# strukturag/libde265

Measured on AMD Instinct MI355X. Metric: decoded CTBs/s, higher is better.
Workload: dtype u16; 1 GPU; c5_8k10_8tiles; width=7680, height=4320, bit_depth=10, tiles=4x2, ctbs_per_picture=8160, stages=inter+residual+intra+deblock+sao, parallelism=pictures/1

## Files before the change

### libde265_amd/csrc/k_common.h

```cpp
#ifndef M355_K_COMMON_H
#define M355_K_COMMON_H

#include <hip/hip_runtime.h>
#include <stdint.h>

#include "de265_mi355x.h"
#include <k_asm.h>

struct DevRef {
  const void* plane[3];
  int stride[3];
  int valid;
  int pad;
};

struct DevIntraWork {
  uint32_t ctb;
  uint32_t ib_start, ib_count;
  uint16_t nb_same;
  uint16_t nb_earlier;
  uint8_t waves_code;
  uint8_t pad[3];
  uint32_t plan_base;
  uint32_t plan_count;
  uint32_t reserved;
};
#ifndef M355_INTRA_SHARE_MIN_LOG2
#define M355_INTRA_SHARE_MIN_LOG2 5
#endif
#define M355_IBX_HAS_RES 0x02000000u
#define M355_IBX_PCM     0x04000000u
#define M355_IBX_FILT    0x08000000u
#define M355_IBX_STRONG  0x10000000u
#define M355_IBX_BFILT   0x20000000u
#define M355_IBX_PUB_COL 0x40000000u
#define M355_IBX_PUB_ROW 0x80000000u
#define M355_INTRA_PLAN_CAP(cf) ((cf) == 0 ? 4608 : ((cf) == 1 ? 6912 : ((cf) == 2 ? 9216 : 13824)))
#define M355_INTRA_PLAN_BATCH(cf) ((cf) == 0 ? 2304 : ((cf) == 1 ? 2560 : ((cf) == 2 ? 3072 : 3584)))

struct DevPicParams {
  int32_t  width, height;
  int32_t  chroma_format_idc, bit_depth_luma, bit_depth_chroma, log2_ctb_size, log2_min_tb_size, log2_min_cb_size;
  int32_t  pic_cb_qp_offset, pic_cr_qp_offset;
  uint32_t flags;
  int32_t  num_tile_cols, num_tile_rows;
  uint16_t col_bd[M355_MAX_TILE_COLS + 1];
  uint16_t row_bd[M355_MAX_TILE_ROWS + 1];
};
static inline DevPicParams dev_pic_params(const m355_pic_params& q)
{
  DevPicParams d;
  d.width = q.width; d.height = q.height;
  d.chroma_format_idc = q.chroma_format_idc; d.bit_depth_luma = q.bit_depth_luma; d.bit_depth_chroma = q.bit_depth_chroma;
  d.log2_ctb_size = q.log2_ctb_size; d.log2_min_tb_size = q.log2_min_tb_size; d.log2_min_cb_size = q.log2_min_cb_size;
  d.pic_cb_qp_offset = q.pic_cb_qp_offset; d.pic_cr_qp_offset = q.pic_cr_qp_offset;
  d.flags = q.flags; d.num_tile_cols = q.num_tile_cols; d.num_tile_rows = q.num_tile_rows;
  for (int i = 0; i <= M355_MAX_TILE_COLS; i++) d.col_bd[i] = q.col_bd[i];
  for (int i = 0; i <= M355_MAX_TILE_ROWS; i++) d.row_bd[i] = q.row_bd[i];
  return d;
}

struct DevPic {
  DevPicParams pp;
  int sw, sh;
  int ctbW, ctbH, nCtb, w4, h4, wcb, hcb;
  int pw[3], ph[3];
  void* plane[3];
  int stride[3];
  void* out_plane[3];
  int out_stride[3];
  const DevRef* refs;
  const uint32_t* inter_tabs;
  const m355_slice* slices;
  const m355_ctb* ctbs;
  const m355_cu* cus;
  const m355_tu* tus;
  const m355_pb* pbs;
  const m355_wt* wts;
  const m355_rb* rb_bin[4];
  const m355_ib* ibs;
  const uint32_t* ib_aux;
  uint16_t* iplan;
  int intra_dense;
  const uint32_t* coeffs;
  const uint16_t* pcm;
  const uint8_t* scaling;
  int n_cus, n_tus, n_pbs, n_ibs;
  int rb_count[4];
  const uint32_t* ctb_ts;
  const uint32_t* ts2rs;
  const uint16_t* tile_id;
  uint32_t* cb_cu;
  uint8_t* cuf;
  uint8_t* edge_tu;
  uint8_t* edge_pb;
  uint32_t* pb_of;
  int16_t* resbuf;
  int16_t* res_tiles;
  uint32_t res_tile_base[4];
  int res_front;
  uint16_t* sao_nb;
  uint32_t* jobs;
  uint32_t* job_base;
  uint32_t* job_tot;
  uint32_t jobs_cap;
  int fill_pb_of_in_meta;
  unsigned long long* edge;
  uint32_t edge_col_ofs[3], edge_row_ofs[3];
  uint32_t* ticket;
  uint32_t* timeout;
  int device_validate;
  int n_wts;
  uint32_t n_coeffs, n_pcm, res_len, ref_valid;
  uint32_t epoch;
  const DevIntraWork* intra_work;
  int n_intra_work, n_intra_ticket;
  int intra_grid;
  int intra_keeper;
  int test_halo_late;
  const uint8_t* ctb_dep;
  const uint8_t* ctb_owner;
  int halo_cu_base, halo_pb_base;
  int n_pb_records;
};

struct HaloLayout {
  int n_vb, n_hb;
  int hw[3], hh[3];
  int xb[3][M355_MAX_TILE_COLS];
  int yb[3][M355_MAX_TILE_ROWS];
  int col_ofs[4], row_ofs[4];
  int n_units;
};

__host__ __device__ inline bool m355_pb_is_edge(const m355_pb& pb, int width, int height, int chroma_format_idc)
{
  const int h8 = (pb.h + 7) & ~7;
  for (int l = 0; l < 2; l++) {
    if (!(pb.flags & (M355_PBF_MC_L0 << l)) || (pb.flags & (M355_PBF_FILL_L0 << l))) continue;
    const int xl = pb.x + (pb.mv[l][0] >> 2), yl = pb.y + (pb.mv[l][1] >> 2);
    if (xl - 3 < 0 || xl + pb.w + 3 > width - 1) return true;
    if (yl - 3 < 0 || yl + h8 + 3 > height - 1) return true;
    if (chroma_format_idc == 1) {
      const int xc = (pb.x >> 1) + (pb.mv[l][0] >> 3), yc = (pb.y >> 1) + (pb.mv[l][1] >> 3);
      if (xc - 1 < 0 || xc + (pb.w >> 1) + 1 > (width >> 1) - 1) return true;
      if (yc - 1 < 0 || yc + (h8 >> 1) + 1 > (height >> 1) - 1) return true;
    }
  }
  return false;
}

__host__ __device__ inline void m355_intra_used_entries(int mode, int log2, int cidx, int chroma_format_idc, uint32_t pic_flags, uint32_t ib_flags, int* top_e, int* left_e)
{
  const int nT = 1 << log2;
  *top_e = 2 * nT; *left_e = 2 * nT;
  if (cidx == 0 && log2 == 5 && (pic_flags & M355_PF_STRONG_INTRA_SMOOTHING)) return;
  bool filt = false;
  if (!(pic_flags & M355_PF_INTRA_SMOOTHING_DISABLED) && (cidx == 0 || chroma_format_idc == 3) && mode != 1 && log2 != 2) {
    const int d26 = mode > 26 ? mode - 26 : 26 - mode, d10 = mode > 10 ? mode - 10 : 10 - mode, minDist = d26 < d10 ? d26 : d10;
    filt = log2 == 3 ? minDist > 7 : (log2 == 4 ? minDist > 1 : (log2 == 5 ? minDist > 0 : false));
  }
  const bool bf = cidx == 0 && log2 < 5 && (mode == 1 || !(ib_flags & M355_IBF_DISABLE_BOUNDARY_FILTER));
  const int mag[9] = {0, 2, 5, 9, 13, 17, 21, 26, 32};
  int te, le;
  if (mode == 0) { te = nT + 1; le = nT + 1; }
  else if (mode == 1) { te = nT; le = nT; }
  else if (mode > 10 && mode < 26) { te = nT; le = nT; }
  else if (mode == 26) { te = nT; le = bf ? nT : 0; }
  else if (mode == 10) { le = nT; te = bf ? nT : 0; }
  else if (mode > 26 && mode <= 34) { te = nT + 1 + ((nT * mag[mode - 26]) >> 5); le = 0; }
  else if (mode >= 2 && mode < 10) { le = nT + 1 + ((nT * mag[10 - mode]) >> 5); te = 0; }
  else return;
  if (filt) { if (te) te++; if (le) le++; }
  *top_e = te < 2 * nT ? te : 2 * nT; *left_e = le < 2 * nT ? le : 2 * nT;
}

struct TileCopyRect { uint32_t plane, xb, y, wb, h, pad; uint64_t ofs; };
static inline bool m355_inter_uses_jobs(const DevPic& p)
{
  const int bdmax = p.pp.bit_depth_luma > p.pp.bit_depth_chroma ? p.pp.bit_depth_luma : p.pp.bit_depth_chroma;
  return p.pp.chroma_format_idc <= 1 && bdmax <= 12 && p.pw[0] >= 16 && (p.pp.chroma_format_idc == 0 || p.pw[1] >= 8);
}

template <class PP> __host__ __device__ static inline bool m355_res32(const PP& pp) { return pp.bit_depth_luma >= 16 || pp.bit_depth_chroma >= 16; }

#define M355_TILE_COPY_RECTS 48
struct TileCopyArgs { char* plane[3]; size_t pitch[3]; TileCopyRect r[M355_TILE_COPY_RECTS]; };
void m355_launch_tiles_copy(const TileCopyArgs& a, int n, void* xbuf, bool to_slot, hipStream_t st);

struct ExportArgs {
  const uint8_t* src[3];
  uint8_t* dst[3];
  long long src_pitch[3], dst_pitch[3];
  uint32_t row_bytes[3], chunks[3], unit_end[3];
  int32_t shift[3];
  const uint32_t* timeout;
  uint32_t epoch;
};
void m355_launch_export(const ExportArgs& a, int src_bytes, int dst_bytes, bool semiplanar, hipStream_t st);

struct ExportScaledArgs {
  const uint8_t* src[3];
  uint8_t* dst[3];
  long long src_pitch[3], dst_pitch[3];
  uint32_t out_w[3], chunks[3], unit_end[3];
  int32_t rshift[3], lshift[3];
  const uint32_t* timeout;
  uint32_t epoch;
};
void m355_launch_export_scaled(const ExportScaledArgs& a, int src_bytes, int dst_bytes, bool semiplanar, int log2_scale, hipStream_t st);

struct ExportRgbArgs {
  const uint8_t* src[3];
  uint8_t* dst[3];
  long long src_pitch[2], dst_pitch[3];
  uint32_t x0, y0, width, height, cw, ch;
  uint32_t chunks, units;
  m355_rgb_coeffs k;
  const uint32_t* timeout;
  uint32_t epoch;
};
void m355_launch_export_rgb(const ExportRgbArgs& a, int src_bytes, int dst_bytes, bool planar, int chroma_format, hipStream_t st);

#define M355_RESIZE_TILE_W 256
#define M355_RESIZE_TILE_H 16
struct ExportResizedArgs {
  const uint8_t* src[3];
  uint8_t* dst[3];
  long long src_pitch[3], dst_pitch[3];
  uint32_t sn_x[3], sn_y[3], dn_x[3], dn_y[3], cosited[3];
  uint32_t tile_w[3], tiles_x[3], unit_end[3];
  int32_t tshift[3], oshift[3], lshift[3];
  const uint32_t* timeout;
  uint32_t epoch;
};
void m355_launch_export_resized(const ExportResizedArgs& a, int src_bytes, int dst_bytes, bool semiplanar, hipStream_t st);

struct ExportResizedRgbArgs {
  const uint8_t* src[3];
  uint8_t* dst[3];
  long long src_pitch[2], dst_pitch[3];
  uint32_t sn_x[2], sn_y[2], dn_x[2], dn_y[2];
  uint32_t tile_w, tiles_x, units;
  int32_t cf, planar, bdl, bdc;
  m355_rgb_coeffs k;
  const uint32_t* timeout;
  uint32_t epoch;
};
void m355_launch_export_resized_rgb(const ExportResizedRgbArgs& a, int src_bytes, int dst_bytes, hipStream_t st);

struct ExportTensorFrame {
  const uint8_t* src[3];
  long long src_pitch[2];
  const uint32_t* timeout;
  uint32_t epoch, pad;
};
struct ExportTensorArgs {
  uint8_t* dst;
  long long stride_n, stride_c, stride_h;
  uint32_t sn_x[2], sn_y[2], dn_x[2], dn_y[2];
  uint32_t tile_w, tiles_x, units, n;
  int32_t cf, nhwc, bf16, u16, bdl, bdc;
  float scale[3], bias[3];
  m355_rgb_coeffs k;
  ExportTensorFrame fr[M355_TENSOR_MAX_FRAMES];
};
void m355_launch_export_tensor(const ExportTensorArgs& a, int src_bytes, int elem_bytes, hipStream_t st);

template <class T> __device__ __forceinline__ T d_sel3(int c, T a0, T a1, T a2)
{
  M355_PIN_V(a0); M355_PIN_V(a1); M355_PIN_V(a2);
  return c == 0 ? a0 : (c == 1 ? a1 : a2);
}
#define M355_SEL3(arr, c) d_sel3((c), (arr)[0], (arr)[1], (arr)[2])

#define M355_GATE(p) do { if ((p).timeout[1] == (p).epoch) return; } while (0)

enum { E_TU_V = 1, E_TU_H = 2, E_PB_V = 4, E_PB_H = 8, E_NONZERO = 16 };

struct DevBatch { const DevPic* pics; uint32_t on; };
#define M355_BATCH_PIC_AT(b, k) if (!(((b).on >> (k)) & 1u)) return; const DevPic& p = (b).pics[(k)]
#define M355_BATCH_PIC(b) M355_BATCH_PIC_AT(b, blockIdx.z)
struct HostBatch { const DevPic* host; const DevPic* dev; int n; uint32_t on; };

void m355_launch_validate(const DevPic& p, hipStream_t st);
void m355_launch_meta(const DevPic& p, hipStream_t st);
void m355_launch_clear_gated(const DevPic& p, void* ptr, size_t bytes, hipStream_t st);
void m355_launch_meta_jobs(const DevPic& p, hipStream_t st);
void m355_launch_job_count(const DevPic& p, bool clear_planes, hipStream_t st);
void m355_launch_job_list(const DevPic& p, hipStream_t st);
void m355_launch_meta_planes(const DevPic& p, hipStream_t st, bool cleared, bool with_tu = true);
void m355_launch_meta_planes_jobs(const DevPic& p, hipStream_t st);
void m355_launch_tu_plan(const DevPic& p, hipStream_t st);
void m355_launch_inter(const DevPic& p, bool hbd, hipStream_t st);
#define M355_INTER_TAB_WORDS 300
void m355_inter_tables(bool bytes, int bd_luma, int bd_chroma, uint32_t* out);
void m355_launch_residual(const DevPic& p, bool hbd, bool big, hipStream_t st);
void m355_launch_residual_both(const DevPic& p, bool hbd, hipStream_t st);
void m355_launch_residual_add(const DevPic& p, bool hbd, hipStream_t st);
void m355_launch_residual_tu_plan(const DevPic& p, bool hbd, hipStream_t st);
void m355_launch_intra_plan(const DevPic& p, hipStream_t st);
void m355_launch_intra(const DevPic& p, bool hbd, hipStream_t st, bool ticket_zero = false);
void m355_launch_meta_planes_batch(const HostBatch& b, hipStream_t st);
void m355_launch_residual_batch(const HostBatch& b, bool hbd, bool big, hipStream_t st);
void m355_launch_intra_plan_batch(const HostBatch& b, hipStream_t st);
void m355_launch_deblock_batch(const HostBatch& b, bool hbd, hipStream_t st);
void m355_launch_sao_batch(const HostBatch& b, bool hbd, hipStream_t st);
void m355_launch_intra_batch(const DevPic& first, bool hbd, bool res32, const DevPic* dev_pics, int n, int max_work, uint32_t* ticket, int grid, hipStream_t st);
void m355_launch_deblock(const DevPic& p, bool hbd, hipStream_t st);
void m355_launch_deblock_pass(const DevPic& p, bool hbd, bool vertical, hipStream_t st);
void m355_launch_sao(const DevPic& p, bool hbd, hipStream_t st);
void m355_launch_halo_pack(const DevPic& p, const HaloLayout& h, bool hbd, int which, void* samples, uint32_t* meta, hipStream_t st);
void m355_launch_halo_add(uint32_t* buf, const uint32_t* scratch, uint32_t pitch_words, int n, uint32_t words, hipStream_t st);
void m355_launch_halo_unpack(const DevPic& p, const HaloLayout& h, bool hbd, int which, const void* samples, const uint32_t* meta, hipStream_t st);

__device__ __forceinline__ int d_clip3(int lo, int hi, int v) { return min(max(v, lo), hi); }
__device__ __forceinline__ int d_clip_bd(int v, int bd) { return d_clip3(0, (1 << bd) - 1, v); }
__device__ __forceinline__ int d_abs(int v) { return v < 0 ? -v : v; }
__device__ __forceinline__ int d_sign(int v) { return (v > 0) - (v < 0); }

__device__ __forceinline__ void wave_sync()
{
  __builtin_amdgcn_fence(__ATOMIC_RELEASE, "wavefront");
  __builtin_amdgcn_wave_barrier();
  __builtin_amdgcn_fence(__ATOMIC_ACQUIRE, "wavefront");
}

__device__ __forceinline__ int d_ctb_of(const DevPic& p, int xl, int yl)
{
  return (yl >> p.pp.log2_ctb_size) * p.ctbW + (xl >> p.pp.log2_ctb_size);
}
__device__ __forceinline__ const m355_slice& d_slice_at(const DevPic& p, int xl, int yl)
{
  return p.slices[p.ctbs[d_ctb_of(p, xl, yl)].slice_idx];
}
__device__ __forceinline__ uint32_t d_cu_index_at(const DevPic& p, int xl, int yl)
{
  return p.cb_cu[(yl >> p.pp.log2_min_cb_size) * p.wcb + (xl >> p.pp.log2_min_cb_size)];
}

#endif
```

### libde265_amd/csrc/k_intra.hip

```cpp
#include <stdlib.h>
#include <type_traits>
#include "k_common.h"
#include "k_meta_tu.h"

#include "k_intra_plan.h"
typedef unsigned long long m355_granule;

__device__ __forceinline__ m355_granule* d_edge_col(const DevPic& p, int c, int col, int y) { return p.edge + p.edge_col_ofs[c] + (size_t)col * (size_t)(p.ph[c] >> 1) + (size_t)(y >> 1); }
__device__ __forceinline__ m355_granule* d_edge_row(const DevPic& p, int c, int row, int x) { return p.edge + p.edge_row_ofs[c] + (size_t)row * (size_t)(p.pw[c] >> 1) + (size_t)(x >> 1); }

__device__ __forceinline__ uint32_t d_poll_halo(const m355_granule* top_row, const m355_granule* left_col, uint32_t* timeout, uint16_t* halo, int hi, uint32_t val, bool pending, int x0c, int y0c, uint32_t epoch)
{
  const int lane = threadIdx.x & 63;
  const bool is_top = hi < HALO_TOP_N;
  const int pos = is_top ? x0c - 1 + hi : y0c + hi - HALO_TOP_N;
  const m355_granule* gsrc = pending ? (is_top ? top_row : left_col) + (pos >> 1) : nullptr;
  unsigned spins = 0;
  for (;;) {
    if (pending) {
      const m355_granule gr = __hip_atomic_load(gsrc, __ATOMIC_RELAXED, __HIP_MEMORY_SCOPE_AGENT);
      if ((uint32_t)(gr >> 32) == epoch) { val = (uint32_t)((gr >> (16 * (pos & 1))) & 0xFFFFu); halo[hi] = (uint16_t)val; pending = false; }
    }
    if (!__any(pending)) break;
    __builtin_amdgcn_s_sleep(1);
    if ((++spins & 1023u) == 0 && (spins > SPIN_LIMIT || __hip_atomic_load(timeout, __ATOMIC_RELAXED, __HIP_MEMORY_SCOPE_AGENT) != 0u)) {
      if (lane == 0) atomicExch(timeout, 1u);
      break;
    }
  }
  return val;
}

template <int CF> __global__ void __launch_bounds__(256) k_intra_plan(DevPic p, int work_n) { k_intra_plan_body<CF>(p, work_n, (int)blockIdx.x, (int)blockIdx.y, (int)gridDim.y); }
template <int CF> __global__ void __launch_bounds__(256) k_intra_plan_batch(DevBatch b) { M355_BATCH_PIC(b); k_intra_plan_body<CF>(p, p.n_intra_work, (int)blockIdx.x, (int)blockIdx.y, (int)gridDim.y); }
template <int CF> __global__ void __launch_bounds__(256) k_tu_plan(DevPic p, int nb_tu, int work_n, int n_parts)
{
  const int b = (int)blockIdx.x;
  if (b < nb_tu) { k_meta_tu_body(p, b); return; }
  const int q = b - nb_tu;
  k_intra_plan_body<CF>(p, work_n, q / n_parts, q % n_parts, n_parts);
}

#ifdef __clang__
#define M355_WAVES_PER_EU(n) __attribute__((amdgpu_waves_per_eu(n)))
#else
#define M355_WAVES_PER_EU(n)
#endif
#ifndef M355_INTRA_SPARSE_WAVES_PER_EU
#define M355_INTRA_SPARSE_WAVES_PER_EU 6
#endif
template <class PIX, int CF, int NW, bool DENSE, bool BATCH, bool W16>
__global__ void __launch_bounds__(64 * NW) M355_WAVES_PER_EU((DENSE || CF >= 2) ? 4 : M355_INTRA_SPARSE_WAVES_PER_EU) k_intra(DevPic p0, int work_n, const DevPic* __restrict__ pics, int n_pics, uint32_t* batch_ticket)
{
  if (!BATCH) M355_GATE(p0);
  constexpr int CW_C = IntraGeo<CF>::CW_C;
  constexpr int BODY_L = IntraGeo<CF>::BODY_L, BODY_C = IntraGeo<CF>::BODY_C;
  constexpr int SAMP_L = IntraGeo<CF>::SAMP_L, SAMP_C = IntraGeo<CF>::SAMP_C;
  __shared__ __attribute__((aligned(16))) uint16_t s_body[SAMP_L + 2 * SAMP_C];
  constexpr int PLAN_LDS = DENSE ? M355_INTRA_PLAN_CAP(CF) : M355_INTRA_PLAN_BATCH(CF);
  constexpr bool PLAN_HERE = DENSE && NW == M355_INTRA_KEEPER_NW;
  __shared__ __attribute__((aligned(16))) uint16_t s_plan[PLAN_LDS];
  __shared__ uint16_t s_raw[NW][4 * 32 + 8];
  __shared__ uint16_t s_f[NW][4 * 32 + 8];
  __shared__ uint32_t s_ticket;
  __shared__ uint32_t s_need[3][MAXCTB];
  __shared__ uint32_t s_cover[3][MAXCTB / 4];
  __shared__ uint32_t s_hneed[3][8];
  __shared__ uint32_t s_hfinal[W16 ? 3 : 1][W16 ? (HALO_N + 31) / 32 : 1];
  __shared__ uint32_t s_kp_idx[(DENSE && NW == M355_INTRA_KEEPER_NW) ? 5 * 64 : 1];
  __shared__ uint16_t s_kp_h1[(DENSE && NW == M355_INTRA_KEEPER_NW) ? 5 * 64 : 1];

  const int wv = __builtin_amdgcn_readfirstlane((int)(threadIdx.x >> 6)), lane = threadIdx.x & 63;

  for (;;) {
  int item = (int)blockIdx.x, pk = 0;
  if (BATCH) {
    if (threadIdx.x == 0) s_ticket = atomicAdd(batch_ticket, 1u);
    __syncthreads();
    const uint32_t t = (uint32_t)__builtin_amdgcn_readfirstlane((int)s_ticket);
    if (t >= (uint32_t)work_n * (uint32_t)n_pics) return;
    pk = (int)(t % (uint32_t)n_pics); item = (int)(t / (uint32_t)n_pics);
  } else if (DENSE || item < p0.n_intra_ticket) {
    if (threadIdx.x == 0) s_ticket = atomicAdd(p0.ticket, 1u);
    __syncthreads();
    item = __builtin_amdgcn_readfirstlane((int)s_ticket);
  }
  item = __builtin_amdgcn_readfirstlane(item);
  const DevPic& p = *(BATCH ? pics + pk : &p0);
  if (BATCH) {
    if (item >= p.n_intra_work || p.timeout[1] == p.epoch) { __syncthreads(); continue; }
  } else if (item >= work_n) return;
  const DevIntraWork* wp = p.intra_work + item;
  const uint4 wd0 = *(const uint4*)wp;
  const uint4 wd1 = ((const uint4*)wp)[1];
  const int ctb = __builtin_amdgcn_readfirstlane((int)wd0.x);
  struct { uint32_t ib_start, ib_count; } ctbinfo = {(uint32_t)__builtin_amdgcn_readfirstlane((int)wd0.y), (uint32_t)__builtin_amdgcn_readfirstlane((int)wd0.z)};
  const uint32_t plan_base = (uint32_t)__builtin_amdgcn_readfirstlane((int)wd1.y), plan_count = (uint32_t)__builtin_amdgcn_readfirstlane((int)wd1.z);
  int GL, GC;
  {
    const int code = __builtin_amdgcn_readfirstlane((int)(wd1.x & 3u));
    constexpr int GLMAX = NW >= 12 ? 8 : (NW >= 6 ? 4 : 2), GCMAX = (NW - GLMAX) / 2 >= 4 ? 4 : ((NW - GLMAX) / 2 >= 2 ? 2 : 1);
    GL = min(GLMAX, code == 0 ? 1 : (code == 1 ? 2 : (code == 2 ? 4 : 8)));
    GC = code == 3 ? GCMAX : 1;
    if (DENSE) { GL = max(GL, 2); GC = GCMAX; }
  }
  const bool spare = wv >= GL + 2 * GC;
  if (spare && !DENSE) return;
  const int c = spare ? 3 : (wv < GL ? 0 : (wv < GL + GC ? 1 : 2));
  const int G = spare ? 1 : (c == 0 ? GL : GC), g = spare ? 0 : (c == 0 ? wv : (wv - GL - (c - 1) * GC));
  const int NWV = DENSE ? NW : GL + 2 * GC;
  const bool multi = GL + GC > 2;
  const int ctbX = ctb % p.ctbW, ctbY = ctb / p.ctbW;
  const int l2c = p.pp.log2_ctb_size;

  const int nc = p.pp.chroma_format_idc ? 3 : 1;
  const bool comp = c < nc;
  const int csw = (c && comp) ? (p.sw == 2) : 0, csh = (c && comp) ? (p.sh == 2) : 0;
  const int cw = (1 << l2c) >> csw, ch = (1 << l2c) >> csh;
  const int x0c = (ctbX << l2c) >> csw, y0c = (ctbY << l2c) >> csh;
  const int bd = (c && comp) ? p.pp.bit_depth_chroma : p.pp.bit_depth_luma;
  const bool res32 = W16 && m355_res32(p.pp);
  const int32_t* res32buf = (const int32_t*)p.resbuf;
  const int cs = comp ? c : 0;
  PIX* plane = (PIX*)p.plane[cs];
  const int stride = p.stride[cs], pw = p.pw[cs], ph = p.ph[cs];
  uint16_t* body = s_body + (cs == 0 ? 0 : SAMP_L + (cs - 1) * SAMP_C);
  const int HALO_BASE = cs == 0 ? BODY_L : BODY_C;
  uint16_t* halo = body + HALO_BASE;
  const int BODY_PITCH = cs == 0 ? BODY_PITCH_OF(MAXCTB) : BODY_PITCH_OF(CW_C);
  uint16_t* raw = s_raw[wv];
  uint16_t* pf = s_f[wv];
  const uint32_t epoch = p.epoch;
#define SYNC_CTB() do { if (multi) __syncthreads(); else wave_sync(); } while (0)

  constexpr bool EARLY = !DENSE;
  constexpr int HU = 4;
  static_assert(3 * MAXCTB + 1 <= 64 * HU, "a component's halo is staged in one pass");
  const int nhalo = (2 * cw + 1) + ch;
  uint4 ex_first = make_uint4(0, 0, 0, 0);
  uint32_t rf0 = 0, rf1 = 0xFFu, rf2 = 0;
  if (EARLY && lane < (int)min(ctbinfo.ib_count, 64u)) {
    ex_first = ((const uint4*)p.ib_aux)[ctbinfo.ib_start + lane];
    const uint32_t* r = (const uint32_t*)&p.ibs[ctbinfo.ib_start + lane];
    rf0 = r[0]; rf1 = r[1]; rf2 = r[2];
  }
  int hx[HU], hy[HU];
  bool hin[HU], htop[HU], hintra[HU];
  uint32_t hci[HU], hpm[HU];
  auto halo_where = [&]() {
#pragma unroll
    for (int u = 0; u < HU; u++) {
      const int h = lane + 64 * g + u * 64 * G;
      htop[u] = h < 2 * cw + 1;
      hx[u] = htop[u] ? x0c - 1 + h : x0c - 1; hy[u] = htop[u] ? y0c - 1 : y0c + (h - (2 * cw + 1));
      hin[u] = comp && h < nhalo && hx[u] >= 0 && hy[u] >= 0 && hx[u] < pw && hy[u] < ph;
      hci[u] = d_cu_index_at(p, hin[u] ? hx[u] << csw : 0, hin[u] ? hy[u] << csh : 0);
    }
  };
  auto halo_who = [&]() {
#pragma unroll
    for (int u = 0; u < HU; u++) hpm[u] = p.cus[hci[u] ? hci[u] - 1 : 0u].pred_mode;
  };
  auto halo_is_intra = [&]() {
#pragma unroll
    for (int u = 0; u < HU; u++) hintra[u] = hin[u] && hci[u] != 0 && hpm[u] == 0;
  };
  if (EARLY) halo_where();

  uint32_t plan_lo = 0;
  if (PLAN_HERE) {
    const uint32_t nbs = (uint32_t)__builtin_amdgcn_readfirstlane((int)(wd0.w & 0xFFFFu)), nbe = (uint32_t)__builtin_amdgcn_readfirstlane((int)(wd0.w >> 16));
    for (uint32_t k = (uint32_t)wv; k < ctbinfo.ib_count; k += (uint32_t)NW)
      d_intra_plan_block<CF>(p, ctbinfo.ib_start + k, ctbX, ctbY, nbs, nbe, s_raw[wv], s_plan);
  } else {
    const uint32_t n = min(plan_count, (uint32_t)PLAN_LDS);
    const uint4* src = (const uint4*)(p.iplan + plan_base);
    for (uint32_t o = (uint32_t)(wv * 64 + lane) * 8u; o < n; o += (uint32_t)NWV * 512u) *(uint4*)(s_plan + o) = src[o >> 3];
  }
  if (EARLY) halo_who();

  if (!res32) {
    int taken = 0;
    for (uint32_t kbase = 0; kbase < ctbinfo.ib_count; kbase += 64) {
      uint32_t rw0 = rf0, rw1 = rf1, rw2 = rf2;
      if (!(EARLY && kbase == 0)) {
        rw0 = 0; rw1 = 0xFFu; rw2 = 0;
        if (kbase + lane < ctbinfo.ib_count) {
          const uint32_t* r = (const uint32_t*)&p.ibs[ctbinfo.ib_start + kbase + lane];
          rw0 = r[0]; rw1 = r[1]; rw2 = r[2];
        }
      }
      unsigned long long mine = __ballot((int)(comp && (rw1 & 0xFFu) == (uint32_t)c));
      auto next_block = [&](int& b_ofs, int& b_log2, uint32_t& b_res) -> bool {
        while (mine) {
          const int src = __ffsll(mine) - 1;
          mine &= mine - 1;
          if ((taken++ & (G - 1)) != g) continue;
          const uint32_t w0 = __builtin_amdgcn_readlane(rw0, src), w1 = __builtin_amdgcn_readlane(rw1, src);
          const int flags = (int)(w1 >> 24);
          if (!(flags & M355_IBF_HAS_RESIDUAL) || (flags & M355_IBF_PCM)) continue;
          b_log2 = (int)((w1 >> 8) & 0xFFu); b_res = __builtin_amdgcn_readlane(rw2, src);
          b_ofs = ((int)(w0 >> 16) - y0c) * BODY_PITCH + BODY_X0 + (int)(w0 & 0xFFFFu) - x0c;
          return true;
        }
        return false;
      };
      auto load_block = [&](uint2* v, int b_log2, uint32_t b_res) {
#pragma unroll
        for (int u = 0; u < 4; u++) {
          const int o = lane * 4 + 256 * u;
          v[u] = make_uint2(0, 0);
          if (o < (1 << (2 * b_log2))) v[u] = *(const uint2*)(p.resbuf + b_res + o);
        }
      };
      auto store_block = [&](const uint2* v, int b_ofs, int b_log2) {
#pragma unroll
        for (int u = 0; u < 4; u++) {
          const int o = lane * 4 + 256 * u;
          if (o < (1 << (2 * b_log2))) *(uint2*)(body + b_ofs + (o >> b_log2) * BODY_PITCH + (o & ((1 << b_log2) - 1))) = v[u];
        }
      };
      for (;;) {
        int ofs_a = 0, log2_a = 2, ofs_b = 0, log2_b = 2;
        uint32_t res_a = 0, res_b = 0;
        if (!next_block(ofs_a, log2_a, res_a)) break;
        const bool two = next_block(ofs_b, log2_b, res_b);
        uint2 va[4], vb[4];
        load_block(va, log2_a, res_a);
        if (two) load_block(vb, log2_b, res_b);
        store_block(va, ofs_a, log2_a);
        if (two) store_block(vb, ofs_b, log2_b);
      }
    }
  }
  if (comp && g == 0) {
    for (int y = lane; y < ch; y += 64) s_need[cs][y] = 0;
    if (lane < 8) s_hneed[cs][lane] = 0;
    if (W16 && lane < (HALO_N + 31) / 32) s_hfinal[W16 ? cs : 0][lane] = 0;
    if (lane == 0) halo[HALO_N] = (uint16_t)(1u << (bd - 1));
    if (lane < MAXCTB / 4) s_cover[cs][lane] = 0;
    wave_sync();
    const int nvr = cw >> 3;
    for (uint32_t kbase = 0; kbase < ctbinfo.ib_count; kbase += 64) {
      uint32_t w0 = rf0, w1 = rf1;
      if (!(EARLY && kbase == 0)) {
        w1 = 0xFFu;
        if (kbase + lane < ctbinfo.ib_count) {
          const uint32_t* r = (const uint32_t*)&p.ibs[ctbinfo.ib_start + kbase + lane];
          w0 = r[0]; w1 = r[1];
        }
      }
      if ((w1 & 0xFFu) != (uint32_t)c) continue;
      const int nT = 1 << ((w1 >> 8) & 0xFFu);
      const int lx = (int)(w0 & 0xFFFFu) - x0c, ly = (int)(w0 >> 16) - y0c;
      {
        const uint32_t um = ((1u << (nT >> 2)) - 1u) << (lx >> 2);
        for (int uy = ly >> 2; uy < (ly + nT) >> 2; uy++) atomicOr(&s_cover[cs][uy], um);
      }
      if ((w1 >> 24) & M355_IBF_PCM) continue;
      if (ly >= 1) {
        const int v0 = max(lx - 1, 0) >> 3, v1 = min((lx + 2 * nT - 1) >> 3, nvr - 1);
        if (v1 >= v0) atomicOr(&s_need[cs][ly - 1], ((2u << v1) - 1u) & ~((1u << v0) - 1u));
      }
      if (lx >= 1) {
        const uint32_t bit = 1u << ((lx - 1) >> 3);
        const int y1 = min(ly + 2 * nT, ch);
        for (int y = max(ly, 0); y < y1; y++) atomicOr(&s_need[cs][y], bit);
      }
      auto need_range = [&](int h0, int h1) {
        for (int w = h0 >> 5; w <= (h1 >> 5); w++) {
          const int a = max(h0 - 32 * w, 0), b = min(h1 - 32 * w, 31);
          atomicOr(&s_hneed[cs][w], (b >= 31 ? ~0u : ((2u << b) - 1u)) & ~((1u << a) - 1u));
        }
      };
      if (ly == 0) need_range(lx, min(lx + 2 * nT, 2 * cw));
      if (lx == 0) need_range(2 * cw + 1 + max(ly - 1, 0), 2 * cw + 1 + min(ly + 2 * nT - 1, ch - 1));
    }
  }
  SYNC_CTB();
  if (comp) {
    if (!EARLY) { halo_where(); halo_who(); }
    halo_is_intra();
    m355_granule hgr[HU];
    uint32_t hpl[HU];
    const size_t g_row = p.edge_row_ofs[cs] + (size_t)max(ctbY - 1, 0) * (size_t)(pw >> 1), g_col = p.edge_col_ofs[cs] + (size_t)max(ctbX - 1, 0) * (size_t)(ph >> 1);
#pragma unroll
    for (int u = 0; u < HU; u++) {
      const int h = lane + 64 * g + u * 64 * G;
      const bool want = hin[u] && ((s_hneed[cs][min(h, nhalo - 1) >> 5] >> (h & 31)) & 1u);
      hintra[u] = hintra[u] && want;
      const size_t gi = htop[u] ? g_row + (size_t)(hx[u] >> 1) : g_col + (size_t)(hy[u] >> 1);
      hgr[u] = __hip_atomic_load(p.edge + (hintra[u] ? gi : (size_t)0), __ATOMIC_RELAXED, __HIP_MEMORY_SCOPE_AGENT);
      hpl[u] = plane[(want && !hintra[u]) ? (size_t)hy[u] * stride + hx[u] : (size_t)0];
      if (!want || hintra[u]) hpl[u] = 0;
    }
    {
      const int l2v = (l2c - csw) - 3;
      const int nvec = ch << l2v;
      constexpr int U = 4;
      auto stage_pass = [&](const int idx0) {
        uint4 v[U];
        bool take[U];
#pragma unroll
        for (int u = 0; u < U; u++) {
          const int idx = idx0 + u * 64 * G;
          const int y = idx >> l2v, xv = (idx & ((1 << l2v) - 1)) * 8;
          const int yc = min(y, ch - 1);
          take[u] = idx < nvec && ((s_need[cs][yc] >> (xv >> 3)) & 1u) && ((s_cover[cs][yc >> 2] >> (xv >> 2)) & 3u) != 3u && x0c + xv < pw && y0c + y < ph;
          v[u] = make_uint4(0, 0, 0, 0);
          if (take[u]) {
            const PIX* src = plane + (size_t)(y0c + y) * stride + x0c + xv;
            if (sizeof(PIX) == 2) v[u] = *(const uint4*)src;
            else { const uint2 b = *(const uint2*)src; v[u].x = b.x; v[u].y = b.y; }
          }
        }
#pragma unroll
        for (int u = 0; u < U; u++) {
          if (!take[u]) continue;
          const int idx = idx0 + u * 64 * G;
          const int y = idx >> l2v, xv = (idx & ((1 << l2v) - 1)) * 8;
          uint4 o = v[u];
          if (sizeof(PIX) == 1) {
            const uint32_t bx = v[u].x, by = v[u].y;
            o.x = (bx & 0xFFu) | ((bx & 0xFF00u) << 8); o.y = ((bx >> 16) & 0xFFu) | ((bx >> 8) & 0xFF0000u);
            o.z = (by & 0xFFu) | ((by & 0xFF00u) << 8); o.w = ((by >> 16) & 0xFFu) | ((by >> 8) & 0xFF0000u);
          }
          const uint32_t cov = (s_cover[cs][y >> 2] >> (xv >> 2)) & 3u;
          uint16_t* dst = body + y * BODY_PITCH + BODY_X0 + xv;
          if (cov == 0u) *(uint4*)dst = o;
          else if (cov == 2u) *(uint2*)dst = make_uint2(o.x, o.y);
          else *(uint2*)(dst + 4) = make_uint2(o.z, o.w);
        }
      };
      stage_pass(lane + 64 * g);
      for (int idx0 = lane + 64 * g + 64 * G * U; idx0 < nvec; idx0 += 64 * G * U) stage_pass(idx0);
    }
#pragma unroll
    for (int u = 0; u < HU; u++) {
      const int h = lane + 64 * g + u * 64 * G;
      if (h >= nhalo) continue;
      uint32_t val = hpl[u];
      if (hintra[u]) val = ((uint32_t)(hgr[u] >> 32) == epoch && !p.test_halo_late) ? (uint32_t)((hgr[u] >> (16 * ((htop[u] ? hx[u] : hy[u]) & 1))) & 0xFFFFu) : HALO_NOT_READY;
      if (htop[u]) halo[h] = (uint16_t)val; else halo[HALO_TOP_N + h - (2 * cw + 1)] = (uint16_t)val;
      if (W16 && !hintra[u] && val == HALO_NOT_READY) {
        const int hi = htop[u] ? h : HALO_TOP_N + h - (2 * cw + 1);
        atomicOr(&s_hfinal[W16 ? cs : 0][hi >> 5], 1u << (hi & 31));
      }
    }
  }
  __syncthreads();
  constexpr bool KEEPER = DENSE && NW == M355_INTRA_KEEPER_NW;
  constexpr int KSLOTS = CF == 3 ? 5 : 4;
  const bool keeper = KEEPER && wv == NW - 1;
  uint32_t kp_pend = 0, kp_fly = 0;
  m355_granule kp_gr[KSLOTS];
  if (keeper) {
    const int cwl = 1 << l2c;
#pragma unroll
    for (int k = 0; k < KSLOTS; k++) kp_gr[k] = 0;
#pragma unroll 1
    for (int k = 0; k < KSLOTS; k++) {
      int q = lane + 64 * k, cq = -1, cwq = 0;
      for (int cc = 0; cc < nc; cc++) {
        const int cw_ = cc ? cwl >> (p.sw == 2) : cwl, ch_ = cc ? cwl >> (p.sh == 2) : cwl, n_ = cw_ + 1 + (ch_ >> 1);
        if (cq < 0) { if (q < n_) { cq = cc; cwq = cw_; } else q -= n_; }
      }
      if (cq < 0) continue;
      const int cswq = cq ? (p.sw == 2) : 0, cshq = cq ? (p.sh == 2) : 0;
      const int x0q = (ctbX << l2c) >> cswq, y0q = (ctbY << l2c) >> cshq;
      const int hbase = (cq == 0 ? 0 : SAMP_L + (cq - 1) * SAMP_C) + (cq == 0 ? BODY_L : BODY_C);
      const bool top = q <= cwq;
      const int t = top ? q : q - (cwq + 1);
      const int h1 = top ? 2 * t : HALO_TOP_N + 2 * t + 1;
      const bool lo = !(top && t == 0);
      const bool miss = s_body[hbase + h1] == HALO_NOT_READY || (lo && s_body[hbase + h1 - 1] == HALO_NOT_READY);
      if (!miss) continue;
      const size_t eofs = top ? (cq == 0 ? p.edge_row_ofs[0] : (cq == 1 ? p.edge_row_ofs[1] : p.edge_row_ofs[2]))
                              : (cq == 0 ? p.edge_col_ofs[0] : (cq == 1 ? p.edge_col_ofs[1] : p.edge_col_ofs[2]));
      const int pwq = cq == 0 ? p.pw[0] : (cq == 1 ? p.pw[1] : p.pw[2]), phq = cq == 0 ? p.ph[0] : (cq == 1 ? p.ph[1] : p.ph[2]);
      s_kp_idx[k * 64 + lane] = (uint32_t)(top ? eofs + (size_t)(ctbY - 1) * (size_t)(pwq >> 1) + (size_t)((x0q - 2 + 2 * t) >> 1)
                                               : eofs + (size_t)(ctbX - 1) * (size_t)(phq >> 1) + (size_t)((y0q + 2 * t) >> 1));
      s_kp_h1[k * 64 + lane] = (uint16_t)((hbase + h1) | (lo ? 0x8000 : 0));
      kp_pend |= 1u << k;
    }
  }
  auto keeper_step = [&]() {
    if (!__any((int)(kp_pend != 0u))) return;
    uint32_t gi[KSLOTS], hh[KSLOTS];
#pragma unroll
    for (int k = 0; k < KSLOTS; k++) { gi[k] = s_kp_idx[k * 64 + lane]; hh[k] = s_kp_h1[k * 64 + lane]; }
#pragma unroll
    for (int k = 0; k < KSLOTS; k++) {
      if (!((kp_fly >> k) & 1u)) continue;
      const m355_granule gr = kp_gr[k];
      if ((uint32_t)(gr >> 32) != epoch) continue;
      s_body[hh[k] & 0x7FFFu] = (uint16_t)(gr >> 16);
      if (hh[k] & 0x8000u) s_body[(hh[k] & 0x7FFFu) - 1] = (uint16_t)gr;
      kp_pend &= ~(1u << k);
    }
    kp_fly = kp_pend;
#pragma unroll
    for (int k = 0; k < KSLOTS; k++)
      if ((kp_pend >> k) & 1u) kp_gr[k] = __hip_atomic_load(p.edge + gi[k], __ATOMIC_RELAXED, __HIP_MEMORY_SCOPE_AGENT);
  };
  const int thr_strong = 1 << (p.pp.bit_depth_luma - 5);
  const int pix_max = (1 << bd) - 1;
  const int lofs_b4 = ((lane & 15) >> 2) * BODY_PITCH + (lane & 3), lofs_b8 = (lane >> 3) * BODY_PITCH + (lane & 7);
  int taken = 0;
  if (KEEPER && keeper) {
    for (uint32_t kbase = 0; kbase < ctbinfo.ib_count; kbase += 64) {
      const int nvalid = min(64, (int)(ctbinfo.ib_count - kbase));
      const int lv = lane < nvalid ? (int)((p.ib_aux[4 * (size_t)(ctbinfo.ib_start + kbase + lane) + 3] >> 16) & 0x3FFFu) : -1;
      const int lv_first = __builtin_amdgcn_readlane(lv, 0), lv_last = __builtin_amdgcn_readlane(lv, nvalid - 1);
      for (int L = lv_first; L <= lv_last; L++) {
        keeper_step();
        d_drain_lds(); __builtin_amdgcn_s_barrier();
      }
    }
  } else
  for (uint32_t kbase = 0; kbase < ctbinfo.ib_count; kbase += 64) {
    uint4 ex = make_uint4(0, 0, 0, 0);
    int lv = -1;
    const int nvalid = min(64, (int)(ctbinfo.ib_count - kbase));
    if (lane < nvalid) {
      ex = (EARLY && kbase == 0) ? ex_first : ((const uint4*)p.ib_aux)[ctbinfo.ib_start + kbase + lane];
      lv = (int)((ex.w >> 16) & 0x3FFFu);
    }
    if (!DENSE) {
      const uint32_t lo = (uint32_t)__builtin_amdgcn_readlane((int)ex.w, 0) & 0xFFFFu;
      const uint32_t last = (uint32_t)__builtin_amdgcn_readlane((int)ex.w, nvalid - 1) & 0xFFFFu;
      if (last + 130u > plan_lo + (uint32_t)PLAN_LDS && plan_count > (uint32_t)PLAN_LDS) {
        __syncthreads();
        const uint32_t lo8 = lo & ~7u;
        const uint32_t n = min(plan_count - lo8, (uint32_t)PLAN_LDS);
        const uint4* src = (const uint4*)(p.iplan + plan_base + lo8);
        for (uint32_t o = (uint32_t)(wv * 64 + lane) * 8u; o < n; o += (uint32_t)NWV * 512u) *(uint4*)(s_plan + o) = src[o >> 3];
        plan_lo = lo8;
        __syncthreads();
      }
    }
    const int lv_first = __builtin_amdgcn_readlane(lv, 0), lv_last = __builtin_amdgcn_readlane(lv, nvalid - 1);
    unsigned long long mine;
    {
      const unsigned long long same = __ballot((int)(comp && lane < nvalid && ((ex.x >> 17) & 3u) == (uint32_t)c));
      const unsigned long long big = same & __ballot((int)(((ex.x >> 14) & 7u) >= (uint32_t)M355_INTRA_SHARE_MIN_LOG2 && !(ex.x & M355_IBX_PCM)));
      const unsigned long long few = same & ~big;
      const int rank = taken + __popcll(few & ((1ull << lane) - 1ull));
      mine = (few & __ballot((int)((rank & (G - 1)) == g))) | big;
      taken += __popcll(few);
    }
    int nsrc = -1, nlevel = -1;
    uint32_t e0 = 0, e1 = 0, e3 = 0, ncode = 0;
    int d_bofs = 0, d_angle = 0, d_inv = 0, d_cls = 0, d_log2 = 0, d_small = 0;
    int d_baddr = 0;
    auto fetch_next = [&]() {
      nsrc = mine ? __ffsll(mine) - 1 : -1;
      mine &= mine - 1;
      if (nsrc < 0) return;
      e0 = (uint32_t)__builtin_amdgcn_readlane((int)ex.x, nsrc); e1 = (uint32_t)__builtin_amdgcn_readlane((int)ex.y, nsrc);
      const uint32_t e2 = (uint32_t)__builtin_amdgcn_readlane((int)ex.z, nsrc);
      e3 = (uint32_t)__builtin_amdgcn_readlane((int)ex.w, nsrc);
      nlevel = (int)((e3 >> 16) & 0x3FFFu);
      d_log2 = (int)((e0 >> 14) & 7u);
      const int lx = (int)(e0 & 127u), ly = (int)((e0 >> 7) & 127u);
      d_bofs = ly * BODY_PITCH + lx + BODY_X0;
      d_cls = (int)((e2 >> 8) & 7u); d_angle = (int)(int8_t)(e2 & 0xFFu); d_inv = (int)(int16_t)(e2 >> 16);
      d_small = (d_log2 <= 3 && !(e0 & M355_IBX_PCM)) ? 1 : 0;
      if (d_small) {
        ncode = s_plan[((e3 & 0xFFFFu) - plan_lo) + (uint32_t)min(lane, 4 << d_log2)];
        d_baddr = d_bofs + (d_log2 == 2 ? lofs_b4 : lofs_b8);
      }
      M355_PIN_S(d_small); M355_PIN_S(d_bofs); M355_PIN_S(d_cls); M355_PIN_S(d_angle); M355_PIN_S(d_inv); M355_PIN_S(d_log2); M355_PIN_S(nlevel);
    };
    fetch_next();
    bool pend = false;
#define PROF_T(k) do { } while (0)
    for (int L = lv_first; L <= lv_last; L++) {
    PROF_T(0);
    if (pend) { fetch_next(); pend = false; }
    while (nsrc >= 0 && nlevel == L) {
      const uint32_t code0 = ncode;
      uint32_t bv0 = 0;
      int rs0 = 0;
      if (__builtin_expect(d_small, 1)) { bv0 = body[code0]; rs0 = (int)(int16_t)body[d_baddr]; }
      if (res32 && d_small && (e0 & M355_IBX_HAS_RES)) rs0 = lane < (1 << (2 * d_log2)) ? res32buf[e1 + lane] : 0;
      const int log2 = d_log2, nT = 1 << log2, cls = d_cls, angle = d_angle, inv = d_inv;
      const int mode = (int)((e0 >> 19) & 63u);
      const bool vert = mode >= 18;
      const bool has_res = (e0 & M355_IBX_HAS_RES) != 0, bfilt = (e0 & M355_IBX_BFILT) != 0;
      const bool pub_col = (e0 & M355_IBX_PUB_COL) != 0, pub_row = (e0 & M355_IBX_PUB_ROW) != 0;
      const int lx = (int)(e0 & 127u), ly = (int)((e0 >> 7) & 127u);

      auto small_block = [&](auto l2_) {
        constexpr int LOG2 = decltype(l2_)::value, NT = 1 << LOG2, Z = 2 * NT, NENT = 4 * NT + 1;
        const int x = lane & (NT - 1), y = lane >> LOG2;
        const bool inb = lane < NT * NT;
        uint32_t bv = bv0;
        int rs = 0;
        rs = rs0 & (has_res ? -1 : 0);
        if (__builtin_expect(__any((int)(bv == HALO_NOT_READY)), 0)) {
          bool pending = bv == HALO_NOT_READY && code0 >= (uint32_t)HALO_BASE && code0 < (uint32_t)(HALO_BASE + HALO_N);
          if (W16 && pending) pending = !((s_hfinal[W16 ? cs : 0][(code0 - HALO_BASE) >> 5] >> ((code0 - HALO_BASE) & 31)) & 1u);
          if (__any((int)pending))
            bv = d_poll_halo(d_edge_row(p, cs, ctbY - 1, 0), d_edge_col(p, cs, ctbX - 1, 0), p.timeout, halo, (int)code0 - HALO_BASE, bv, pending, x0c, y0c, epoch);
        }
        PROF_T(1);
        {
          const uint32_t nb = (uint32_t)__builtin_amdgcn_update_dpp(0, (int)bv, 0x138, 0xF, 0xF, false) + (uint32_t)__builtin_amdgcn_update_dpp(0, (int)bv, 0x130, 0xF, 0xF, false);
          const uint32_t fbv = (nb + 2u * bv + 2u) >> 2;
          if ((e0 & M355_IBX_FILT) && lane > 0 && lane < NENT - 1) bv = fbv;
        }
#define BRL(i) ((int)__builtin_amdgcn_readlane((int)bv, (i) + Z))
#define BRP(i) ((int)__builtin_amdgcn_ds_bpermute(((i) + Z) << 2, (int)bv))
        int v;
        if (__builtin_expect(cls >= 3, 1)) {
          const int a_ = vert ? y : x, b_ = vert ? x : y;
          const int tt = __mul24(a_ + 1, angle), iIdx = tt >> 5, iFact = tt & 31;
          const int x1 = b_ + iIdx + 1, x2 = x1 + 1;
          const int p1 = (__mul24(x1, inv) + 128) >> 8, p2 = (__mul24(x2, inv) + 128) >> 8;
          int i1 = x1 >= 0 ? x1 : -p1, i2 = x2 >= 0 ? x2 : -p2;
          if (!vert) { i1 = -i1; i2 = -i2; }
          const int r1 = BRP(i1), r2 = BRP(i2);
          v = (32 * r1 + __mul24(iFact, r2 - r1) + 16) >> 5;
        } else if (cls == 0) {
          const int l = BRP(-1 - y), t = BRP(1 + x), tr = BRL(1 + NT), bl = BRL(-1 - NT);
          v = (__mul24(NT - 1 - x, l) + __mul24(x + 1, tr) + __mul24(NT - 1 - y, t) + __mul24(y + 1, bl) + NT) >> (LOG2 + 1);
        } else if (cls == 1) {
          int s_ = (lane >= Z - NT && lane <= Z + NT && lane != Z) ? (int)bv : 0;
          s_ += __builtin_amdgcn_update_dpp(0, s_, 0xB1, 0xF, 0xF, false);
          s_ += __builtin_amdgcn_update_dpp(0, s_, 0x4E, 0xF, 0xF, false);
          s_ += __builtin_amdgcn_update_dpp(0, s_, 0x141, 0xF, 0xF, false);
          s_ += __builtin_amdgcn_update_dpp(0, s_, 0x140, 0xF, 0xF, false);
          int sum = __builtin_amdgcn_readlane(s_, 0) + __builtin_amdgcn_readlane(s_, 16);
          const int dc = (sum + NT) >> (LOG2 + 1);
          v = dc;
          if (bfilt) {
            const int eb = BRP(y == 0 ? x + 1 : -y - 1), e2c = BRL(-1) + BRL(1);
            if (x == 0 || y == 0) v = (eb + 3 * dc + 2) >> 2;
            if (lane == 0) v = (e2c + 2 * dc + 2) >> 2;
          }
        } else {
          const int l = BRP(-1 - y), t = BRP(1 + x), corner = BRL(0), first = vert ? BRL(1) : BRL(-1);
          v = vert ? t : l;
          if (bfilt && (vert ? x == 0 : y == 0)) v = d_clip3(0, pix_max, first + (((vert ? l : t) - corner) >> 1));
        }
#undef BRL
#undef BRP
        v = d_clip3(0, pix_max, v + rs);
        if (inb) body[d_baddr] = (uint16_t)v;
        if (__builtin_expect((e0 & (M355_IBX_PUB_COL | M355_IBX_PUB_ROW)) != 0, 0)) {
        if (pub_col) {
          const uint32_t v2 = (uint32_t)__builtin_amdgcn_ds_bpermute((lane + NT) << 2, v);
          if (inb && x == NT - 1 && !(y & 1))
            __hip_atomic_store(d_edge_col(p, cs, ctbX, y0c + ly + y), ((m355_granule)epoch << 32) | (v2 << 16) | (uint32_t)v, __ATOMIC_RELAXED, __HIP_MEMORY_SCOPE_AGENT);
        }
        if (pub_row) {
          const uint32_t v2 = (uint32_t)__builtin_amdgcn_ds_bpermute((lane + 1) << 2, v);
          if (inb && y == NT - 1 && !(x & 1))
            __hip_atomic_store(d_edge_row(p, cs, ctbY, x0c + lx + x), ((m355_granule)epoch << 32) | (v2 << 16) | (uint32_t)v, __ATOMIC_RELAXED, __HIP_MEMORY_SCOPE_AGENT);
        }
        }
      };

      if (__builtin_expect(d_small, 1)) {
        if (log2 == 2) small_block(std::integral_constant<int, 2>()); else small_block(std::integral_constant<int, 3>());
      } else {
      const int nPass = (nT * nT) >> 6;
      const bool shared = log2 >= M355_INTRA_SHARE_MIN_LOG2;
      const int it_lo = shared ? (nPass * g) / G : 0, it_hi = shared ? (nPass * (g + 1)) / G : nPass;
      if (!(e0 & M355_IBX_PCM)) {
        if (it_lo < it_hi) {
        const int nEnt = 4 * nT + 1, Z = 2 * nT;
        const uint16_t* pl = s_plan + ((e3 & 0xFFFFu) - plan_lo);
        uint32_t cd[3] = {0, 0, 0}, val[3] = {0, 0, 0};
#pragma unroll
        for (int q = 0; q < 3; q++) {
          if (64 * q >= nEnt) continue;
          const int e = lane + 64 * q;
          if (e < nEnt) cd[q] = (uint32_t)pl[e];
        }
#pragma unroll
        for (int q = 0; q < 3; q++) {
          if (64 * q >= nEnt) continue;
          if (lane + 64 * q < nEnt) val[q] = body[cd[q]];
        }
        if (__any((int)(val[0] == HALO_NOT_READY || val[1] == HALO_NOT_READY || val[2] == HALO_NOT_READY))) {
#pragma unroll
          for (int q = 0; q < 3; q++) {
            if (64 * q >= nEnt) continue;
            bool pending = lane + 64 * q < nEnt && val[q] == HALO_NOT_READY && cd[q] >= (uint32_t)HALO_BASE && cd[q] < (uint32_t)(HALO_BASE + HALO_N);
            if (W16 && pending) pending = !((s_hfinal[W16 ? cs : 0][(cd[q] - HALO_BASE) >> 5] >> ((cd[q] - HALO_BASE) & 31)) & 1u);
            if (__any((int)pending))
              val[q] = d_poll_halo(d_edge_row(p, cs, ctbY - 1, 0), d_edge_col(p, cs, ctbX - 1, 0), p.timeout, halo, (int)cd[q] - HALO_BASE, val[q], pending, x0c, y0c, epoch);
          }
        }
#pragma unroll
        for (int q = 0; q < 3; q++) {
          if (64 * q >= nEnt) continue;
          if (lane + 64 * q < nEnt) raw[lane + 64 * q] = (uint16_t)val[q];
        }
        wave_sync();
        PROF_T(1);
        uint16_t* P = raw;
        if (e0 & M355_IBX_FILT) {
          const bool bi = (e0 & M355_IBX_STRONG) && d_abs((int)raw[Z] + raw[Z + 64] - 2 * raw[Z + 32]) < thr_strong && d_abs((int)raw[Z] + raw[Z - 64] - 2 * raw[Z - 32]) < thr_strong;
#pragma unroll
          for (int q = 0; q < 3; q++) {
            if (64 * q >= nEnt) continue;
            const int e = lane + 64 * q;
            if (e < nEnt) {
              const int i = e - Z;
              int v;
              if (i == -Z || i == Z) v = raw[e];
              else if (bi) {
                if (i == 0) v = raw[Z];
                else if (i < 0) v = raw[Z] + (((-i) * ((int)raw[Z - 64] - raw[Z]) + 32) >> 6);
                else v = raw[Z] + ((i * ((int)raw[Z + 64] - raw[Z]) + 32) >> 6);
              } else v = (raw[e + 1] + 2 * raw[e] + raw[e - 1] + 2) >> 2;
              pf[e] = (uint16_t)v;
            }
          }
          wave_sync();
          P = pf;
        }
#define BRD(i) ((int)P[(i) + Z])
        int dcVal = 0;
        if (mode == 1) {
          int s_ = 0;
          if (lane < nT) s_ = BRD(lane + 1) + BRD(-lane - 1);
          s_ += __builtin_amdgcn_update_dpp(0, s_, 0xB1, 0xF, 0xF, false);
          s_ += __builtin_amdgcn_update_dpp(0, s_, 0x4E, 0xF, 0xF, false);
          s_ += __builtin_amdgcn_update_dpp(0, s_, 0x141, 0xF, 0xF, false);
          s_ += __builtin_amdgcn_update_dpp(0, s_, 0x140, 0xF, 0xF, false);
          dcVal = (__builtin_amdgcn_readlane(s_, 0) + __builtin_amdgcn_readlane(s_, 16) + nT) >> (log2 + 1);
        }
        {
          const int xb = lane & (nT - 1), yb = lane >> log2, ystep = 64 >> log2, nIt = (nT * nT) >> 6;
          const int res_on = has_res ? -1 : 0;
          auto big_loop = [&](auto cls_) {
            constexpr int CLS = decltype(cls_)::value;
            const int x = xb;
            const int t_x = (CLS == 0 || CLS == 2) ? BRD(1 + x) : 0;
            const int u_tr = CLS == 0 ? BRD(1 + nT) : 0, u_bl = CLS == 0 ? BRD(-1 - nT) : 0;
            const int u_c = CLS == 2 ? BRD(0) : 0, u_f = CLS == 2 ? (vert ? BRD(1) : BRD(-1)) : 0;
            const int u_e2 = CLS == 1 ? BRD(-1) + BRD(1) : 0;
            (void)nIt;
            for (int it0 = it_lo; it0 < it_hi; it0 += 4) {
              int ta[4], tb[4], fa[4], rs[4];
#pragma unroll
              for (int u = 0; u < 4; u++) {
                const int y = yb + min(it0 + u, it_hi - 1) * ystep;
                fa[u] = 0; tb[u] = 0;
                if (CLS == 0 || CLS == 2) ta[u] = BRD(-1 - y);
                else if (CLS == 1) ta[u] = BRD(y == 0 ? x + 1 : -y - 1);
                else {
                  const int a_ = vert ? y : x, b_ = vert ? x : y;
                  const int tt = __mul24(a_ + 1, angle), iIdx = tt >> 5;
                  fa[u] = tt & 31;
                  const int x1 = b_ + iIdx + 1, x2 = x1 + 1;
                  int i1, i2;
                  if (CLS == 3) { i1 = vert ? x1 : -x1; i2 = vert ? x2 : -x2; }
                  else {
                    const int p1 = (__mul24(x1, inv) + 128) >> 8, p2 = (__mul24(x2, inv) + 128) >> 8;
                    i1 = x1 >= 0 ? x1 : -p1; i2 = x2 >= 0 ? x2 : -p2;
                    if (!vert) { i1 = -i1; i2 = -i2; }
                  }
                  ta[u] = BRD(i1); tb[u] = BRD(fa[u] ? i2 : i1);
                }
                rs[u] = (int)(int16_t)body[d_bofs + y * BODY_PITCH + x] & res_on;
                if (res32) rs[u] = has_res ? res32buf[e1 + y * nT + x] : 0;
              }
#pragma unroll
              for (int u = 0; u < 4; u++) {
                const int y = yb + min(it0 + u, it_hi - 1) * ystep;
                int v;
                if (CLS == 0) v = (__mul24(nT - 1 - x, ta[u]) + __mul24(x + 1, u_tr) + __mul24(nT - 1 - y, t_x) + __mul24(y + 1, u_bl) + nT) >> (log2 + 1);
                else if (CLS == 1) {
                  v = dcVal;
                  if (bfilt) {
                    if (x == 0 || y == 0) v = (ta[u] + 3 * dcVal + 2) >> 2;
                    if (x == 0 && y == 0) v = (u_e2 + 2 * dcVal + 2) >> 2;
                  }
                } else if (CLS == 2) {
                  v = vert ? t_x : ta[u];
                  if (bfilt && (vert ? x == 0 : y == 0)) v = d_clip3(0, pix_max, u_f + (((vert ? ta[u] : t_x) - u_c) >> 1));
                } else v = (32 * ta[u] + __mul24(fa[u], tb[u] - ta[u]) + 16) >> 5;
                v = d_clip3(0, pix_max, v + rs[u]);
                body[d_bofs + y * BODY_PITCH + x] = (uint16_t)v;
              }
            }
          };
          if (cls == 0) big_loop(std::integral_constant<int, 0>());
          else if (cls == 1) big_loop(std::integral_constant<int, 1>());
          else if (cls == 2) big_loop(std::integral_constant<int, 2>());
          else if (cls == 3) big_loop(std::integral_constant<int, 3>());
          else big_loop(std::integral_constant<int, 4>());
        }
#undef BRD
        }
      } else {
        for (int o = lane; o < nT * nT; o += 64) {
          const int y = o >> log2, x = o & (nT - 1);
          body[(ly + y) * BODY_PITCH + lx + x + BODY_X0] = p.pcm[e1 + o];
        }
      }
      const int pr_lo = (e0 & M355_IBX_PCM) ? 0 : it_lo * (64 >> log2), pr_hi = (e0 & M355_IBX_PCM) ? nT : it_hi * (64 >> log2);
      if (pub_col || (pub_row && pr_hi == nT)) {
        wave_sync();
        if (pub_col && lane < (nT >> 1) && 2 * lane >= pr_lo && 2 * lane < pr_hi) {
          const int y = ly + 2 * lane;
          const uint32_t s0 = body[y * BODY_PITCH + lx + nT - 1 + BODY_X0], s1 = body[(y + 1) * BODY_PITCH + lx + nT - 1 + BODY_X0];
          __hip_atomic_store(d_edge_col(p, cs, ctbX, y0c + y), ((m355_granule)epoch << 32) | (s1 << 16) | s0, __ATOMIC_RELAXED, __HIP_MEMORY_SCOPE_AGENT);
        }
        if (pub_row && pr_hi == nT && lane >= 32 && lane < 32 + (nT >> 1)) {
          const int x = lx + 2 * (lane - 32);
          const uint32_t s0 = body[(ly + nT - 1) * BODY_PITCH + x + BODY_X0], s1 = body[(ly + nT - 1) * BODY_PITCH + x + 1 + BODY_X0];
          __hip_atomic_store(d_edge_row(p, cs, ctbY, x0c + x), ((m355_granule)epoch << 32) | (s1 << 16) | s0, __ATOMIC_RELAXED, __HIP_MEMORY_SCOPE_AGENT);
        }
      }
      }
      PROF_T(2);
      const int peek = mine ? __builtin_amdgcn_readlane(lv, __ffsll(mine) - 1) : -1;
      if (peek != L) { pend = true; break; }
      fetch_next();
    }
    PROF_T(3);
    SYNC_CTB();
    PROF_T(4);
    }
  }
  if (comp) {
    const int l2u = (l2c - csw) - 2;
    const int npieces = ch << l2u;
    for (int idx = lane + 64 * g; idx < npieces; idx += 64 * G) {
      const int y = idx >> l2u, u = idx & ((1 << l2u) - 1);
      if (!((s_cover[cs][y >> 2] >> u) & 1u)) continue;
      const uint2 v = *(const uint2*)(body + y * BODY_PITCH + BODY_X0 + 4 * u);
      PIX* dst = plane + (size_t)(y0c + y) * stride + x0c + 4 * u;
      if (sizeof(PIX) == 2) *(uint2*)dst = v;
      else *(uint32_t*)dst = (v.x & 0xFFu) | ((v.x >> 8) & 0xFF00u) | ((v.y & 0xFFu) << 16) | ((v.y & 0xFF0000u) << 8);
    }
  }
  if (!DENSE) return;
  __syncthreads();
  }
#undef SYNC_CTB
}

#ifndef M355_INTRA_DENSE_NW
#define M355_INTRA_DENSE_NW 12
#endif
#ifndef M355_INTRA_SPARSE_NW
#define M355_INTRA_SPARSE_NW 4
#endif

template <class PIX, int CF, bool W16>
static void launch_intra_cf(const DevPic& p, bool ticket_zero, hipStream_t st)
{
  if (!ticket_zero) hipMemsetAsync(p.ticket, 0, 4, st);
  const dim3 dense_grid(p.intra_grid > 0 && p.intra_grid < p.n_intra_work ? p.intra_grid : p.n_intra_work);
  if (p.intra_dense && p.intra_keeper) hipLaunchKernelGGL(HIP_KERNEL_NAME(k_intra<PIX, CF, M355_INTRA_KEEPER_NW, true, false, W16>), dense_grid, dim3(64 * M355_INTRA_KEEPER_NW), 0, st, p, p.n_intra_work, (const DevPic*)nullptr, 1, (uint32_t*)nullptr);
  else if (p.intra_dense) hipLaunchKernelGGL(HIP_KERNEL_NAME(k_intra<PIX, CF, M355_INTRA_DENSE_NW, true, false, W16>), dense_grid, dim3(64 * M355_INTRA_DENSE_NW), 0, st, p, p.n_intra_work, (const DevPic*)nullptr, 1, (uint32_t*)nullptr);
  else hipLaunchKernelGGL(HIP_KERNEL_NAME(k_intra<PIX, CF, M355_INTRA_SPARSE_NW, false, false, W16>), dim3(p.n_intra_work), dim3(64 * M355_INTRA_SPARSE_NW), 0, st, p, p.n_intra_work, (const DevPic*)nullptr, 1, (uint32_t*)nullptr);
}

void m355_launch_intra(const DevPic& p, bool hbd, hipStream_t st, bool ticket_zero)
{
  if (!p.n_intra_work) return;
  if (hbd && m355_res32(p.pp)) {
    switch (p.pp.chroma_format_idc) {
      case 0: launch_intra_cf<uint16_t, 0, true>(p, ticket_zero, st); break;
      case 1: launch_intra_cf<uint16_t, 1, true>(p, ticket_zero, st); break;
      case 2: launch_intra_cf<uint16_t, 2, true>(p, ticket_zero, st); break;
      default: launch_intra_cf<uint16_t, 3, true>(p, ticket_zero, st); break;
    }
    return;
  }
  switch (p.pp.chroma_format_idc) {
    case 0: if (hbd) launch_intra_cf<uint16_t, 0, false>(p, ticket_zero, st); else launch_intra_cf<uint8_t, 0, false>(p, ticket_zero, st); break;
    case 1: if (hbd) launch_intra_cf<uint16_t, 1, false>(p, ticket_zero, st); else launch_intra_cf<uint8_t, 1, false>(p, ticket_zero, st); break;
    case 2: if (hbd) launch_intra_cf<uint16_t, 2, false>(p, ticket_zero, st); else launch_intra_cf<uint8_t, 2, false>(p, ticket_zero, st); break;
    default: if (hbd) launch_intra_cf<uint16_t, 3, false>(p, ticket_zero, st); else launch_intra_cf<uint8_t, 3, false>(p, ticket_zero, st); break;
  }
}

template <class PIX, int CF, bool W16 = false>
static void launch_intra_batch_cf(const DevPic& first, const DevPic* dev_pics, int n, int max_work, uint32_t* ticket, int grid, hipStream_t st)
{
  hipLaunchKernelGGL(HIP_KERNEL_NAME(k_intra<PIX, CF, M355_INTRA_DENSE_NW, true, true, W16>), dim3(grid), dim3(64 * M355_INTRA_DENSE_NW), 0, st, first, max_work, dev_pics, n, ticket);
}
void m355_launch_intra_batch(const DevPic& first, bool hbd, bool res32, const DevPic* dev_pics, int n, int max_work, uint32_t* ticket, int grid, hipStream_t st)
{
  if (max_work <= 0 || n <= 0) return;
  if (hbd && res32) {
    switch (first.pp.chroma_format_idc) {
      case 0: launch_intra_batch_cf<uint16_t, 0, true>(first, dev_pics, n, max_work, ticket, grid, st); break;
      case 1: launch_intra_batch_cf<uint16_t, 1, true>(first, dev_pics, n, max_work, ticket, grid, st); break;
      case 2: launch_intra_batch_cf<uint16_t, 2, true>(first, dev_pics, n, max_work, ticket, grid, st); break;
      default: launch_intra_batch_cf<uint16_t, 3, true>(first, dev_pics, n, max_work, ticket, grid, st); break;
    }
    return;
  }
  switch (first.pp.chroma_format_idc) {
    case 0: if (hbd) launch_intra_batch_cf<uint16_t, 0>(first, dev_pics, n, max_work, ticket, grid, st); else launch_intra_batch_cf<uint8_t, 0>(first, dev_pics, n, max_work, ticket, grid, st); break;
    case 1: if (hbd) launch_intra_batch_cf<uint16_t, 1>(first, dev_pics, n, max_work, ticket, grid, st); else launch_intra_batch_cf<uint8_t, 1>(first, dev_pics, n, max_work, ticket, grid, st); break;
    case 2: if (hbd) launch_intra_batch_cf<uint16_t, 2>(first, dev_pics, n, max_work, ticket, grid, st); else launch_intra_batch_cf<uint8_t, 2>(first, dev_pics, n, max_work, ticket, grid, st); break;
    default: if (hbd) launch_intra_batch_cf<uint16_t, 3>(first, dev_pics, n, max_work, ticket, grid, st); else launch_intra_batch_cf<uint8_t, 3>(first, dev_pics, n, max_work, ticket, grid, st); break;
  }
}

void m355_launch_intra_plan_batch(const HostBatch& b, hipStream_t st)
{
  int work = 0, cf = 1;
  for (int k = 0; k < b.n; k++) if ((b.on >> k) & 1u) { work = std::max(work, b.host[k].n_intra_work); cf = b.host[k].pp.chroma_format_idc; }
  if (!work) return;
  const DevBatch d{b.dev, b.on};
  const dim3 grid(work, PLAN_SPLIT, b.n);
  switch (cf) {
    case 0: hipLaunchKernelGGL(HIP_KERNEL_NAME(k_intra_plan_batch<0>), grid, dim3(256), 0, st, d); break;
    case 1: hipLaunchKernelGGL(HIP_KERNEL_NAME(k_intra_plan_batch<1>), grid, dim3(256), 0, st, d); break;
    case 2: hipLaunchKernelGGL(HIP_KERNEL_NAME(k_intra_plan_batch<2>), grid, dim3(256), 0, st, d); break;
    default: hipLaunchKernelGGL(HIP_KERNEL_NAME(k_intra_plan_batch<3>), grid, dim3(256), 0, st, d); break;
  }
}

void m355_launch_tu_plan(const DevPic& p, hipStream_t st)
{
  const int n_plan = (p.intra_dense && p.intra_keeper) ? 0 : p.n_intra_work, split = p.intra_dense ? PLAN_SPLIT : 1;
  const int nb_tu = (p.n_tus + 255) / 256, nb = nb_tu + n_plan * split;
  if (!nb) return;
  switch (p.pp.chroma_format_idc) {
    case 0: hipLaunchKernelGGL(HIP_KERNEL_NAME(k_tu_plan<0>), dim3(nb), dim3(256), 0, st, p, nb_tu, n_plan, split); break;
    case 1: hipLaunchKernelGGL(HIP_KERNEL_NAME(k_tu_plan<1>), dim3(nb), dim3(256), 0, st, p, nb_tu, n_plan, split); break;
    case 2: hipLaunchKernelGGL(HIP_KERNEL_NAME(k_tu_plan<2>), dim3(nb), dim3(256), 0, st, p, nb_tu, n_plan, split); break;
    default: hipLaunchKernelGGL(HIP_KERNEL_NAME(k_tu_plan<3>), dim3(nb), dim3(256), 0, st, p, nb_tu, n_plan, split); break;
  }
}

void m355_launch_intra_plan(const DevPic& p, hipStream_t st)
{
  if (!p.n_intra_work) return;
  if (p.intra_dense && p.intra_keeper) return;
  const int split = p.intra_dense ? PLAN_SPLIT : 1;
  switch (p.pp.chroma_format_idc) {
    case 0: hipLaunchKernelGGL(HIP_KERNEL_NAME(k_intra_plan<0>), dim3(p.n_intra_work, split), dim3(256), 0, st, p, p.n_intra_work); break;
    case 1: hipLaunchKernelGGL(HIP_KERNEL_NAME(k_intra_plan<1>), dim3(p.n_intra_work, split), dim3(256), 0, st, p, p.n_intra_work); break;
    case 2: hipLaunchKernelGGL(HIP_KERNEL_NAME(k_intra_plan<2>), dim3(p.n_intra_work, split), dim3(256), 0, st, p, p.n_intra_work); break;
    default: hipLaunchKernelGGL(HIP_KERNEL_NAME(k_intra_plan<3>), dim3(p.n_intra_work, split), dim3(256), 0, st, p, p.n_intra_work); break;
  }
}
```

### libde265_amd/csrc/runtime_decode.hip

```cpp
#include "runtime_internal.h"

extern "C" {

bool chain_residuals_forced();

int prepare(m355_ctx* c, Resident& r, DevPic& d_out, bool& want_sao_out, hipStream_t st) {
  hipSetDevice(c->device);
  const m355_picture& pic = r.hdr;
  const m355_pic_params& pp = pic.pp;
  Frame* dst = get_frame(c, pic.dst_frame);
  if (!dst) return fail(M355_ERR_INVALID, "dst_frame %d is not a live frame", pic.dst_frame);
  if (dst->w != pp.width || dst->h != pp.height || dst->cf != pp.chroma_format_idc || dst->bdl != pp.bit_depth_luma || dst->bdc != pp.bit_depth_chroma)
    return fail(M355_ERR_INVALID, "dst frame geometry does not match the picture parameters");
  DevPic d = r.dp;
  d.ref_valid = 0;
  DevRef refs[M355_MAX_REF_FRAMES];
  memset(refs, 0, sizeof(refs));
  for (int i = 0; i < M355_MAX_REF_FRAMES; i++) {
    if (pic.ref_frames[i] < 0) continue;
    Frame* f = get_frame(c, pic.ref_frames[i]);
    if (!f) return fail(M355_ERR_INVALID, "ref_frames[%d]=%d is not a live frame", i, pic.ref_frames[i]);
    if (f->w != dst->w || f->h != dst->h || f->cf != dst->cf || f->bdl != dst->bdl || f->bdc != dst->bdc)
      return fail(M355_ERR_INVALID, "reference frame %d geometry differs (motion.cc:377-398 would conceal; record FILL instead)", i);
    if (f == dst) return fail(M355_ERR_INVALID, "a picture cannot reference itself");
    for (int cc = 0; cc < 3; cc++) { refs[i].plane[cc] = f->plane[cc]; refs[i].stride[cc] = f->stride[cc]; }
    refs[i].valid = 1;
    d.ref_valid |= 1u << i;
  }
  if (!r.refs_dev) {
    HIPCHK(hipMalloc(&r.refs_dev, sizeof(refs)));
    HIPCHK(hipHostMalloc(&r.refs_host, sizeof(refs), hipHostMallocDefault));
    r.refs_valid = false;
  }
  if (!r.refs_valid || memcmp(r.refs_host, refs, sizeof(refs)) != 0) {
    if (!r.fresh) HIPCHK(sync_all(c));
    memcpy(r.refs_host, refs, sizeof(refs));
    HIPCHK(hipMemcpyAsync(r.refs_dev, r.refs_host, sizeof(refs), hipMemcpyHostToDevice, st));
    r.refs_valid = true;
  }
  d.refs = r.refs_dev;
  {
    const uint32_t key = (uint32_t)(dst->bpp[0] == 1) | ((uint32_t)pp.bit_depth_luma << 8) | ((uint32_t)pp.bit_depth_chroma << 16);
    const uint32_t* tab = nullptr;
    for (auto& e : c->inter_tabs) if (e.first == key) tab = e.second;
    if (!tab) {
      uint32_t host[M355_INTER_TAB_WORDS];
      m355_inter_tables(dst->bpp[0] == 1, std::min((int)pp.bit_depth_luma, 16), std::min((int)pp.bit_depth_chroma, 16), host);
      uint32_t* dev = nullptr;
      HIPCHK(hipMalloc(&dev, sizeof(host)));
      HIPCHK(hipMemcpy(dev, host, sizeof(host), hipMemcpyHostToDevice));
      c->inter_tabs.emplace_back(key, dev);
      tab = dev;
    }
    d.inter_tabs = tab;
  }
  Lane& L = lane(c);
  int rc;
  {
    const size_t u4 = (size_t)d.w4 * d.h4, ncb = (size_t)d.wcb * d.hcb;
    const size_t need = ((2 * u4 + 63) & ~(size_t)63) + ncb * 4 + 64;
    if ((rc = grow(&L.edge_tu, &L.cap_u4, need, st, false))) return rc;
    if ((rc = grow(&L.pb_of, &L.cap_cb, u4, st, true))) return rc;
  }
  {
    size_t n = 0;
    for (int cc = 0; cc < 3; cc++) {
      d.edge_col_ofs[cc] = (uint32_t)n; n += (size_t)d.ctbW * (size_t)(dst->ph[cc] >> 1);
      d.edge_row_ofs[cc] = (uint32_t)n; n += (size_t)d.ctbH * (size_t)(dst->pw[cc] >> 1);
    }
    if ((rc = grow(&L.edge, &L.cap_edge, n + 1, st, true))) return rc;
  }
  if ((rc = grow(&L.cuf, &L.cap_cuf, (size_t)pic.n_cus + (size_t)r.halo.n_units + 1, st, false))) return rc;
  const size_t res_intra = (((size_t)pic.res_len + 64) & ~(size_t)63) * (m355_res32(pp) ? 2 : 1);
  size_t res_tiles = 0;
  for (int s = 0; s < 4; s++) { d.res_tile_base[s] = (uint32_t)res_tiles; res_tiles += (size_t)pic.rb_count[s] << (2 * (s + 2)); }
  const bool tiles = (c->depth >= sched::chain_residual_tiles_min_depth || chain_residuals_forced()) && (long long)pic.pp.width * pic.pp.height <= sched::one_stream_max_samples;
  const size_t res_need = res_intra + (tiles ? res_tiles : 0) + 1;
  if ((rc = grow(&L.resbuf, &L.cap_res, res_need, st, false))) return rc;
  d.res_tiles = tiles ? L.resbuf + res_intra : nullptr;
  d.res_front = 0;
  if ((rc = grow(&L.sao_nb, &L.cap_sao, (size_t)d.nCtb * 3, st, false))) return rc;
  {
    const size_t area = (size_t)pp.width * pp.height;
    const size_t cap = pic.n_pbs > 0 ? std::min(area / 16, area / 32 + 8 * (size_t)pic.n_pbs) + 256 : 1;
    const size_t n_chunks = ((size_t)(pic.n_pbs > 0 ? pic.n_pbs : 0) + 255) / 256;
    if ((rc = grow(&L.jobs, &L.cap_jobs, cap, st, false))) return rc;
    if ((rc = grow(&L.job_base, &L.cap_jobbase, n_chunks * 4 + 8, st, true))) return rc;
    d.jobs_cap = (uint32_t)cap; d.job_base = L.job_base; d.job_tot = L.job_base + n_chunks * 4;
  }
  if ((rc = grow(&L.iplan, &L.cap_iplan, (size_t)r.n_iplan + 8, st, false))) return rc;

  const bool want_sao = (c->stages & M355_STAGE_SAO) && (pp.flags & M355_PF_SAO_ENABLED);
  Frame* target = dst;
  if (want_sao) {
    if (!L.work.used || L.work.w != dst->w || L.work.h != dst->h || L.work.cf != dst->cf || L.work.bdl != dst->bdl || L.work.bdc != dst->bdc) {
      HIPCHK(sync_all(c));
      if (L.work.used) frame_free(L.work);
      frame_geometry(L.work, dst->w, dst->h, dst->cf, dst->bdl, dst->bdc);
      if ((rc = frame_alloc(L.work, st))) return rc;
    }
    target = &L.work;
  }
  for (int cc = 0; cc < 3; cc++) {
    d.pw[cc] = dst->pw[cc]; d.ph[cc] = dst->ph[cc];
    d.plane[cc] = target->plane[cc]; d.stride[cc] = target->stride[cc];
    d.out_plane[cc] = dst->plane[cc]; d.out_stride[cc] = dst->stride[cc];
  }
  d.edge_tu = L.edge_tu; d.edge_pb = L.edge_tu + (size_t)d.w4 * d.h4;
  d.cb_cu = (uint32_t*)(L.edge_tu + (((size_t)2 * d.w4 * d.h4 + 63) & ~(size_t)63));
  d.cuf = L.cuf; d.pb_of = L.pb_of;
  d.fill_pb_of_in_meta = ((c->stages & M355_STAGE_INTER) && m355_inter_uses_jobs(d)) ? 0 : 1;
  d.jobs = L.jobs; d.sao_nb = L.sao_nb; d.iplan = L.iplan;
  d.resbuf = L.resbuf; d.edge = L.edge; d.ticket = L.ticket; d.timeout = L.timeout;
  {
    static const int grid_env = getenv("M355_INTRA_GRID") ? atoi(getenv("M355_INTRA_GRID")) : 0;
    static int slots = 0;
    if (!slots) { hipDeviceProp_t prop; slots = (hipGetDeviceProperties(&prop, c->device) == hipSuccess && prop.multiProcessorCount > 0) ? 2 * prop.multiProcessorCount : 512; }
    d.intra_grid = grid_env > 0 ? grid_env : std::max(64, slots / std::max(1, c->depth));
    d.intra_keeper = c->depth <= sched::intra_keeper_max_depth;
    if (!d.intra_keeper && r.dp.intra_dense) {
      bool idle = true;
      for (int i = 0; i < c->depth && idle; i++) if (&c->lanes[i] != &L && ev_query(c, c->lanes[i].last) != hipSuccess) idle = false;
      d.intra_keeper = idle;
    }
    static const bool no_keeper = getenv("M355_TEST_NO_KEEPER") != nullptr;
    if (no_keeper) d.intra_keeper = 0;
    static const int halo_late = getenv("M355_TEST_HALO_LATE") ? atoi(getenv("M355_TEST_HALO_LATE")) : 0;
    d.test_halo_late = halo_late;
  }
  d.epoch = ++c->epoch;
  if (d.epoch == 0) d.epoch = ++c->epoch;
  d_out = d; want_sao_out = want_sao;
  return M355_OK;
}

void clear_target(m355_ctx* c, const DevPic& d, Frame* tgt, bool gated, hipStream_t st) {
  for (int cc = 0; cc < 3; cc++) {
    if (!tgt->pw[cc]) continue;
    const size_t bytes = (size_t)tgt->stride[cc] * tgt->ph[cc] * tgt->bpp[cc];
    if (gated) m355_launch_clear_gated(d, tgt->plane[cc], bytes, st);
    else hipMemsetAsync(tgt->plane[cc], 0, bytes, st);
  }
}

bool chain_residuals_forced() { static const bool on = getenv("M355_TEST_CHAIN_RESIDUALS") != nullptr; return on; }

hipStream_t launch_prediction(m355_ctx* c, const Resident& r, const DevPic& d, bool hbd, hipStream_t st, hipEvent_t* ev, bool with_intra, hipStream_t chain, Frame* hazard_dst) {
  Lane& L = lane(c);
  const bool single = d.intra_dense || (long long)d.pp.width * d.pp.height <= sched::one_stream_max_samples;
  hipStream_t s2 = single ? st : L.stream2;
  static const int clear_min = getenv("M355_CLEAR_IN_COUNT_MIN") ? atoi(getenv("M355_CLEAR_IN_COUNT_MIN")) : sched::clear_in_count_min_pbs;
  const bool clear_in_count = d.n_pbs >= std::max(1, clear_min);
  bool tu_plan_with_residuals = false;
  const bool res_front = (chain || chain_residuals_forced()) && d.res_tiles && (c->stages & M355_STAGE_RESIDUAL) && d.pp.bit_depth_luma <= 15 && d.pp.bit_depth_chroma <= 15 &&
                         d.rb_count[0] + d.rb_count[1] + d.rb_count[2] + d.rb_count[3] > 0;
  if (clear_in_count) m355_launch_job_count(d, true, st);
  if (!single) { hipEventRecord(L.ev_fork, st); hipStreamWaitEvent(s2, L.ev_fork, 0); }
  if (single && clear_in_count && (c->stages & M355_STAGE_INTRA)) {
    m355_launch_meta_planes_jobs(d, st);
    if (c->depth <= sched::tu_plan_in_residuals_max_depth && (c->stages & M355_STAGE_RESIDUAL) && !res_front) tu_plan_with_residuals = true; else m355_launch_tu_plan(d, st);
  } else {
    if (c->stages & M355_STAGE_INTRA) {
      m355_launch_meta_planes(d, s2, clear_in_count, false);
      m355_launch_tu_plan(d, s2);
    } else m355_launch_meta_planes(d, s2, clear_in_count);
    if (clear_in_count) m355_launch_job_list(d, st); else m355_launch_meta_jobs(d, st);
  }
  auto launch_residuals = [&](const DevPic& dd) {
    hipStream_t sr = !single ? s2 : st;
    if (sr != st) { hipEventRecord(L.ev_fork2, st); hipStreamWaitEvent(s2, L.ev_fork2, 0); }
    if (tu_plan_with_residuals) m355_launch_residual_tu_plan(dd, hbd, st);
    else if (sr == st) m355_launch_residual_both(dd, hbd, st);
    else {
      m355_launch_residual(dd, hbd, false, sr);
      m355_launch_residual(dd, hbd, true, st);
    }
  };
  if (res_front) { DevPic dq = d; dq.res_front = 1; launch_residuals(dq); }
  if (ev) hipEventRecord(ev[1], st);
  if (chain && chain != st) {
    EvRef front;
    if (ev_mark(c, st, &front) == M355_OK) {
      st = chain; ev_wait(c, st, front);
      if (ev) hipEventRecord(ev[1], st);
    }
  }
  if (hazard_dst) dst_hazards(c, hazard_dst, true, st);
  if (c->depth >= 2)
    for (int i = 0; i < M355_MAX_REF_FRAMES; i++) {
      Frame* f = r.hdr.ref_frames[i] >= 0 ? get_frame(c, r.hdr.ref_frames[i]) : nullptr;
      if (f) ev_wait(c, st, f->wr);
    }
  if (c->stages & M355_STAGE_INTER) m355_launch_inter(d, hbd, st);
  if (ev) hipEventRecord(ev[2], st);
  if ((c->stages & M355_STAGE_RESIDUAL) && !res_front) launch_residuals(d);
  else if (res_front) m355_launch_residual_add(d, hbd, st);
  if (!single) { hipEventRecord(L.ev_join, s2); hipStreamWaitEvent(st, L.ev_join, 0); }
  if (ev) hipEventRecord(ev[3], st);
  if (with_intra && (c->stages & M355_STAGE_INTRA)) m355_launch_intra(d, hbd, st, clear_in_count);
  if (ev) hipEventRecord(ev[4], st);
  return st;
}

void dst_hazards(m355_ctx* c, Frame* dstf, bool piped, hipStream_t st) {
  readers_wait(c, st, dstf);
  if (!piped) return;
  ev_wait(c, st, dstf->wr);
  for (int k = 0; k < M355_MAX_LANES; k++) ev_wait(c, st, dstf->rd[k]);
}

int mark_done(m355_ctx* c, Resident& r, Frame* dstf, hipStream_t st, const DevPic* d) {
  const int rc = ev_mark(c, st, &r.done);
  if (rc) return rc;
  r.fresh = false;
  dstf->wr_stream = st; dstf->wr = r.done;
  dstf->wr_gate = d ? d->timeout : nullptr; dstf->wr_epoch = d ? d->epoch : 0;
  lane(c).last = r.done; lane(c).last_stream = st;
  return M355_OK;
}

struct DecodeState {
  DevPic d; bool want_sao = false; hipEvent_t* ev = nullptr;
  hipStream_t st = nullptr;
};

enum { PRE_ALL = 0, PRE_NO_INTRA = 1, PRE_HAZARDS = 2 };
static int decode_pre(m355_ctx* c, Resident& r, bool rotate, DecodeState& S, int mode, hipStream_t on_stream = nullptr)
{
  const bool with_intra = mode == PRE_ALL;
  if (r.sharded) return fail(M355_ERR_INVALID, "a sharded picture is decoded by phases (m355_decode_phase)");
  hipStream_t chain = nullptr;
  if (rotate && c->depth >= 2) {
    unsigned long long newest = 0;
    for (int i = 0; i < M355_MAX_REF_FRAMES; i++) {
      Frame* f = r.hdr.ref_frames[i] >= 0 ? get_frame(c, r.hdr.ref_frames[i]) : nullptr;
      static const bool always = getenv("M355_TEST_CHAIN_LANES") != nullptr;
      if (!f || f->wr.ticket <= newest || (!always && ev_query(c, f->wr) == hipSuccess)) continue;
      newest = f->wr.ticket; chain = f->wr.stream;
    }
    int lane = (c->active + 1) % c->depth;
    if (chain) {
      const bool split = c->depth >= sched::chain_split_min_depth;
      for (int k = 0; k < c->depth; k++) {
        const int l = (c->active + 1 + k) % c->depth;
        if ((c->lanes[l].stream != chain) == split) { lane = l; break; }
      }
    }
    select_lane(c, lane);
  }
  Lane& L = lane(c);
  hipStream_t st = on_stream ? on_stream : L.stream;
  if (!on_stream && with_intra && r.dp.intra_dense && c->active >= sched::intra_class_first_lane && lane_priorities_mode() == 2 && lane_class_priority(c->active) != 0) {
    if (!L.stream_hi) HIPCHK(hipStreamCreateWithPriority(&L.stream_hi, hipStreamNonBlocking, lane_class_priority(c->active)));
    st = L.stream_hi;
  }
  ev_wait(c, st, L.last);
  DevPic& d = S.d;
  int rc = prepare(c, r, d, S.want_sao, st);
  if (rc) return rc;
  const bool want_sao = S.want_sao;
  const m355_pic_params& pp = r.hdr.pp;
  const bool hbd = pp.bit_depth_luma > 8;
  const bool piped = c->depth >= 2;
  Frame* dstf = get_frame(c, r.hdr.dst_frame);
  if (piped) {
    ev_wait(c, st, r.up);
  }
  hipEvent_t* ev = nullptr;
  if (with_intra && c->timing_on) {
    if (c->ev_used >= 4096) c->ev_used = 0;
    while ((int)c->evs.size() < (c->ev_used + 1) * 7) { hipEvent_t e; HIPCHK(hipEventCreate(&e)); c->evs.push_back(e); }
    ev = &c->evs[c->ev_used * 7];
    c->ev_used++;
    hipEventRecord(ev[0], st);
  }
  S.ev = ev;
  if (r.device_validate) m355_launch_validate(d, st);
  const bool hazards_late = !want_sao && piped && mode != PRE_HAZARDS && !(pp.flags & M355_PF_CLEAR_DST);
  if (!want_sao && !hazards_late) dst_hazards(c, dstf, piped, st);
  if (pp.flags & M355_PF_CLEAR_DST) clear_target(c, d, want_sao ? &L.work : dstf, r.device_validate && !want_sao, st);
  if (!with_intra) d.intra_keeper = 0;
  if (mode != PRE_HAZARDS) st = launch_prediction(c, r, d, hbd, st, ev, with_intra, with_intra && chain != st ? chain : nullptr, hazards_late ? dstf : nullptr);
  S.st = st;
  return M355_OK;
}

static int decode_post(m355_ctx* c, Resident& r, DecodeState& S, bool filters = true)
{
  const DevPic& d = S.d;
  const bool want_sao = S.want_sao;
  hipEvent_t* ev = S.ev;
  const m355_pic_params& pp = r.hdr.pp;
  const bool hbd = pp.bit_depth_luma > 8;
  const bool piped = c->depth >= 2;
  Frame* dstf = get_frame(c, r.hdr.dst_frame);
  const hipStream_t st = S.st;
  const bool deblock = filters && (c->stages & M355_STAGE_DEBLOCK) && (pp.flags & M355_PF_DEBLOCK_ENABLED);
  if (deblock) m355_launch_deblock(d, hbd, st);
  if (ev) hipEventRecord(ev[5], st);
  if (filters && want_sao) { dst_hazards(c, dstf, piped, st); m355_launch_sao(d, hbd, st); }
  if (ev) hipEventRecord(ev[6], st);
  {
    const int rcm = mark_done(c, r, dstf, st, &d);
    if (rcm) return rcm;
  }
  const EvRef done = r.done;
  for (int i = 0; i < M355_MAX_REF_FRAMES; i++) {
    Frame* f = r.hdr.ref_frames[i] >= 0 ? get_frame(c, r.hdr.ref_frames[i]) : nullptr;
    if (f) f->rd[c->active] = done;
  }
  {
    m355_ctx::Status& s = c->status[++c->serial % M355_STATUS_RING];
    if (s.serial && s.validated && !s.reported) {
      ev_sync(c, s.done);
      if (c->status_words[4 * (s.serial % M355_STATUS_RING) + 1] == s.epoch) { if (!c->lost_count++) c->lost_first = s.serial; }
    }
    s.serial = c->serial; s.epoch = d.epoch; s.validated = r.device_validate; s.reported = false;
    s.done = done;
    if (r.device_validate) {
      if (!c->status_words) HIPCHK(hipHostMalloc(&c->status_words, 16 * M355_STATUS_RING, hipHostMallocDefault));
      hipMemcpyAsync(c->status_words + 4 * (c->serial % M355_STATUS_RING), lane(c).timeout, 16, hipMemcpyDeviceToHost, st);
      const int rcm = ev_mark(c, st, &s.done);
      if (rcm) return rcm;
    }
  }
  hipError_t e = hipGetLastError();
  if (e != hipSuccess) return fail(M355_ERR_HIP, "kernel launch failed: %s", hipGetErrorString(e));
  {
    static const bool dbg = getenv("M355_DEBUG_TIMEOUT") && atoi(getenv("M355_DEBUG_TIMEOUT"));
    if (dbg) {
      hipStreamSynchronize(st);
      uint32_t t = 0;
      hipMemcpy(&t, lane(c).timeout, 4, hipMemcpyDeviceToHost);
      if (t) fprintf(stderr, "m355: decode %llu (epoch %u, %d pbs, %d ibs, %d cus, lane %d): intra wait gave up\n", c->serial, d.epoch, d.n_pbs, d.n_ibs, d.n_cus, c->active);
    }
  }
  return M355_OK;
}

int decode(m355_ctx* c, Resident& r, bool rotate) {
  DecodeState S;
  const int rc = decode_pre(c, r, rotate, S, PRE_ALL);
  return rc ? rc : decode_post(c, r, S);
}

int status_of(m355_ctx* c, m355_ctx::Status& s) {
  if (!s.validated) return M355_OK;
  const uint32_t* w = c->status_words + 4 * (s.serial % M355_STATUS_RING);
  if (w[1] != s.epoch) return M355_OK;
  const unsigned long long key = (unsigned long long)w[2] | ((unsigned long long)w[3] << 32);
  uint32_t bad = (uint32_t)key;
  if ((uint32_t)(key >> 32) != ~s.epoch) bad = 0;
  static const char* const names[8] = {"?", "cu", "tu", "pb", "weight", "rb", "ib", "?"};
  s.reported = true;
  return fail(M355_ERR_INVALID, "picture %llu: %s %u rejected by the device-side list validation (the picture was not decoded)", s.serial, names[(bad >> 28) & 7], bad & 0x0FFFFFFFu);
}

unsigned long long m355_last_serial(m355_ctx* c) { return c->serial; }

int m355_decode_status(m355_ctx* c, unsigned long long serial)
{
  if (serial == 0 || serial > c->serial) return fail(M355_ERR_INVALID, "no decode with serial %llu", serial);
  m355_ctx::Status& s = c->status[serial % M355_STATUS_RING];
  if (s.serial != serial) return fail(M355_ERR_STALE, "decode %llu is older than the last %d decodes: its status is no longer kept (m355_wait reports rejections)", serial, M355_STATUS_RING);
  hipSetDevice(c->device);
  const hipError_t q = ev_query(c, s.done);
  if (q == hipErrorNotReady) return M355_ERR_BUSY;
  if (q != hipSuccess) return fail(M355_ERR_HIP, "hipEventQuery failed: %s", hipGetErrorString(q));
  return status_of(c, s);
}

int m355_decode_batch(m355_ctx* c, const int* handles, int n)
{
  if (n < 1 || !handles) return fail(M355_ERR_INVALID, "m355_decode_batch: no pictures");
  if (n > std::max(1, c->depth)) return fail(M355_ERR_INVALID, "m355_decode_batch: %d pictures on %d lanes (m355_set_pipeline_depth)", n, c->depth);
  for (int k = 0; k < n; k++) {
    const int h = handles[k];
    if (h < 0 || h >= (int)c->resident.size() || !c->resident[h].used) return fail(M355_ERR_INVALID, "bad picture handle");
    for (int j = 0; j < k; j++) if (handles[j] == h) return fail(M355_ERR_INVALID, "m355_decode_batch: picture %d twice in one batch", h);
    const Resident& r = c->resident[h];
    const m355_pic_params &a = r.hdr.pp, &b = c->resident[handles[0]].hdr.pp;
    if (r.sharded) return fail(M355_ERR_INVALID, "a sharded picture is decoded by phases (m355_decode_phase)");
    if (!r.dp.intra_dense || r.dp.n_pbs > 0) return fail(M355_ERR_INVALID, "m355_decode_batch: picture %d is not an intra picture", h);
    if (a.chroma_format_idc != b.chroma_format_idc || (a.bit_depth_luma > 8) != (b.bit_depth_luma > 8))
      return fail(M355_ERR_INVALID, "m355_decode_batch: the pictures differ in chroma format or sample type");
    for (int j = 0; j < k; j++)
      if (c->resident[handles[j]].hdr.dst_frame == r.hdr.dst_frame) return fail(M355_ERR_INVALID, "m355_decode_batch: two pictures into frame %d", r.hdr.dst_frame);
  }
  hipSetDevice(c->device);
  if (n == 1 || !(c->stages & M355_STAGE_INTRA)) {
    for (int k = 0; k < n; k++) { int rc = decode(c, c->resident[handles[k]]); if (rc) return rc; }
    return M355_OK;
  }
  DecodeState S[M355_MAX_LANES];
  int lane[M355_MAX_LANES];
  int rc_late = M355_OK, n_ok = 0;
  static const int streams_env = getenv("M355_BATCH_STREAMS") ? std::min(4, std::max(0, atoi(getenv("M355_BATCH_STREAMS")))) : -1;
  const int n_streams = streams_env >= 0 ? streams_env : std::min(4, std::max(1, c->depth / n));
  hipStream_t bs = nullptr;
  if (n_streams > 0) {
    const int j = (int)(c->batch_count++ % (unsigned)n_streams);
    if (!c->batch_stream[j]) HIPCHK(hipStreamCreateWithFlags(&c->batch_stream[j], hipStreamNonBlocking));
    bs = c->batch_stream[j];
  }
  for (int k = 0; k < n; k++) {
    Resident& r = c->resident[handles[k]];
    const int rc = decode_pre(c, r, true, S[k], bs ? PRE_HAZARDS : PRE_NO_INTRA, bs);
    if (rc) { rc_late = rc; break; }
    lane[k] = c->active;
    if (!bs) {
      if (!c->batch_ev_pre[k] && hipEventCreateWithFlags(&c->batch_ev_pre[k], hipEventDisableTiming) != hipSuccess) return fail(M355_ERR_HIP, "hipEventCreate failed");
      hipEventRecord(c->batch_ev_pre[k], S[k].st);
    }
    n_ok++;
  }
  if (!n_ok) return rc_late;
  m355_ctx::BatchSlot& b = c->batch[c->batch_next];
  c->batch_next = (c->batch_next + 1) % M355_BATCH_RING;
  if (!b.dev) {
    HIPCHK(hipHostMalloc((void**)&b.host, sizeof(DevPic) * M355_MAX_LANES, hipHostMallocDefault));
    HIPCHK(hipMalloc((void**)&b.dev, sizeof(DevPic) * M355_MAX_LANES + 64));
    b.ticket = (uint32_t*)((uint8_t*)b.dev + sizeof(DevPic) * M355_MAX_LANES);
    HIPCHK(hipEventCreateWithFlags(&b.ev, hipEventDisableTiming));
  }
  if (b.pending) { hipEventSynchronize(b.ev); b.pending = false; }
  const hipStream_t st0 = S[0].st;
  int max_work = 0; long total = 0;
  bool res32 = false;
  for (int k = 0; k < n_ok; k++) {
    b.host[k] = S[k].d;
    max_work = std::max(max_work, S[k].d.n_intra_work); total += S[k].d.n_intra_work;
    res32 = res32 || m355_res32(S[k].d.pp);
    if (k && !bs) hipStreamWaitEvent(st0, c->batch_ev_pre[k], 0);
  }
  hipMemcpyAsync(b.dev, b.host, sizeof(DevPic) * n_ok, hipMemcpyHostToDevice, st0);
  hipMemsetAsync(b.ticket, 0, 4, st0);
  const bool hbd = c->resident[handles[0]].hdr.pp.bit_depth_luma > 8;
  const HostBatch hb{b.host, b.dev, n_ok, n_ok >= 32 ? 0xFFFFFFFFu : (1u << n_ok) - 1u};
  if (bs) {
    m355_launch_meta_planes_batch(hb, st0);
    if (c->stages & M355_STAGE_INTRA) m355_launch_intra_plan_batch(hb, st0);
    if (c->stages & M355_STAGE_RESIDUAL) { m355_launch_residual_batch(hb, hbd, false, st0); m355_launch_residual_batch(hb, hbd, true, st0); }
  }
  {
    static const int grid_env = getenv("M355_INTRA_GRID") ? atoi(getenv("M355_INTRA_GRID")) : 0;
    static int slots = 0;
    if (!slots) { hipDeviceProp_t prop; slots = (hipGetDeviceProperties(&prop, c->device) == hipSuccess && prop.multiProcessorCount > 0) ? 2 * prop.multiProcessorCount : 512; }
    int widest = 0;
    for (int k = 0; k < n_ok; k++) widest += std::min(S[k].d.ctbH, (S[k].d.ctbW + 1) / 2) + 1;
    const int grid = (int)std::min<long>(std::max<long>(total, 1), grid_env > 0 ? grid_env : std::min(slots, n_streams <= 1 ? slots : std::max(widest, slots / (2 * n_streams))));
    m355_launch_intra_batch(S[0].d, hbd, res32, b.dev, n_ok, max_work, b.ticket, grid, st0);
  }
  hipEventRecord(b.ev, st0); b.pending = true;
  if (bs) {
    uint32_t dbk = 0, sao = 0;
    for (int k = 0; k < n_ok; k++) {
      if ((c->stages & M355_STAGE_DEBLOCK) && (c->resident[handles[k]].hdr.pp.flags & M355_PF_DEBLOCK_ENABLED)) dbk |= 1u << k;
      if (S[k].want_sao) sao |= 1u << k;
    }
    if (dbk) m355_launch_deblock_batch(HostBatch{b.host, b.dev, n_ok, dbk}, hbd, st0);
    if (sao) {
      for (int k = 0; k < n_ok; k++) if ((sao >> k) & 1u) dst_hazards(c, get_frame(c, c->resident[handles[k]].hdr.dst_frame), c->depth >= 2, bs);
      m355_launch_sao_batch(HostBatch{b.host, b.dev, n_ok, sao}, hbd, st0);
    }
    hipEventRecord(b.ev, st0);
  }
  for (int k = 0; k < n_ok; k++) {
    select_lane(c, lane[k]);
    if (!bs && k) hipStreamWaitEvent(S[k].st, b.ev, 0);
    const int rc = decode_post(c, c->resident[handles[k]], S[k], !bs);
    if (rc && !rc_late) rc_late = rc;
  }
  return rc_late;
}
}
```

### libde265_amd/csrc/runtime_internal.h

```cpp
#ifndef M355_RUNTIME_INTERNAL_H
#define M355_RUNTIME_INTERNAL_H
#include <dlfcn.h>
#include <stdarg.h>
#include <stdio.h>
#include <stdlib.h>
#include <string.h>

#include <algorithm>
#include <array>
#include <atomic>
#include <chrono>
#include <condition_variable>
#include <functional>
#include <mutex>
#include <thread>
#include <string>
#include <utility>
#include <vector>

#include <pthread.h>
#include "k_common.h"
#include "k_hash.h"
#include "k_measure.h"


extern thread_local std::string g_err;
int fail(int code, const char* fmt, ...);
#define HIPCHK(call) do { hipError_t e_ = (call); if (e_ != hipSuccess) return fail(M355_ERR_HIP, "%s failed: %s", #call, hipGetErrorString(e_)); } while (0)

#define M355_STATUS_RING 64
#define M355_BATCH_RING 16
#define M355_MAX_LANES 32
#define M355_TRANSIENT_MAX 12

namespace sched {
constexpr long long one_stream_max_samples = 16ll << 20;
constexpr int clear_in_count_min_pbs = 64 * 256;
constexpr int tu_plan_in_residuals_max_depth = 1;
constexpr int intra_keeper_max_depth = 1;
constexpr int chain_split_min_depth = 3;
constexpr int chain_residual_tiles_min_depth = 3;
constexpr int intra_class_first_lane = 3;
}

struct EvRef { unsigned long long ticket = 0; hipStream_t stream = nullptr; };
#define M355_EV_RING 256

enum ReaderKind { RD_DOWNLOAD, RD_EXPORT, RD_HASH, RD_MEASURE, RD_KINDS };
struct Frame {
  bool used = false;
  int w = 0, h = 0, cf = 0, bdl = 0, bdc = 0;
  int pw[3] = {0, 0, 0}, ph[3] = {0, 0, 0}, stride[3] = {0, 0, 0}, bpp[3] = {1, 1, 1};
  void* plane[3] = {nullptr, nullptr, nullptr};
  EvRef wr, rd[M355_MAX_LANES];
  hipStream_t wr_stream = nullptr;
  const uint32_t* wr_gate = nullptr; uint32_t wr_epoch = 0;
  EvRef reader[RD_KINDS];
};

static void frame_geometry(Frame& f, int w, int h, int cf, int bdl, int bdc)
{
  f.w = w; f.h = h; f.cf = cf; f.bdl = bdl; f.bdc = bdc;
  const int sw = (cf == 1 || cf == 2) ? 2 : 1, sh = (cf == 1) ? 2 : 1;
  for (int c = 0; c < 3; c++) {
    f.bpp[c] = ((c ? bdc : bdl) <= 8) ? 1 : 2;
    if (c && cf == 0) { f.pw[c] = f.ph[c] = f.stride[c] = 0; continue; }
    f.pw[c] = c ? w / sw : w;
    f.ph[c] = c ? h / sh : h;
    const int pitch_bytes = (f.pw[c] * f.bpp[c] + 127) & ~127;
    f.stride[c] = pitch_bytes / f.bpp[c];
  }
}
static int frame_alloc(Frame& f, hipStream_t st)
{
  for (int c = 0; c < 3; c++) {
    if (!f.pw[c]) continue;
    const size_t bytes = (size_t)f.stride[c] * f.ph[c] * f.bpp[c] + 256;
    HIPCHK(hipMalloc(&f.plane[c], bytes));
    HIPCHK(hipMemsetAsync(f.plane[c], 0, bytes, st));
  }
  f.used = true;
  return M355_OK;
}
static void frame_free(Frame& f)
{
  for (int c = 0; c < 3; c++) { if (f.plane[c]) hipFree(f.plane[c]); f.plane[c] = nullptr; }
  f.wr = EvRef();
  for (int k = 0; k < M355_MAX_LANES; k++) f.rd[k] = EvRef();
  for (EvRef& m : f.reader) m = EvRef();
  f.wr_stream = nullptr; f.wr_gate = nullptr; f.wr_epoch = 0;
  f.used = false;
}

struct Resident {
  bool used = false;
  m355_picture hdr;
  char* dev = nullptr;
  char* host = nullptr;
  size_t cap = 0, bytes = 0;
  DevPic dp;
  DevRef* refs_dev = nullptr;
  DevRef* refs_host = nullptr;
  bool refs_valid = false;
  int n_intra_work = 0;
  uint32_t n_iplan = 0;
  bool sharded = false;
  int shard_rank = 0, shard_n = 1;
  HaloLayout halo;
  DevPic live;
  bool live_sao = false, live_valid = false;
  void* xprev = nullptr;
  int lane = 0;
  void* xb[4] = {nullptr, nullptr, nullptr, nullptr};
  size_t xb_bytes[4] = {0, 0, 0, 0};
  void* xscratch = nullptr;
  std::vector<hipEvent_t> x3_read;
  unsigned long long xb_epoch = 0;
  std::vector<int> peers;
  EvRef up;
  EvRef done;
  bool fresh = false;
  bool arena = false;
  m355_arena_caps caps;
  int arena_halo_units = 0;
  bool reserved = false;
  bool device_validate = false;
  size_t xscratch_pitch = 0;
  std::vector<uint8_t> sched_u8;
  std::vector<uint32_t> sched_u32;
  std::vector<uint32_t> sched_order, sched_cand, sched_bucket, sched_u32b;
};

struct Lane {
  hipStream_t stream = nullptr, stream2 = nullptr;
  hipEvent_t ev_fork = nullptr, ev_fork2 = nullptr, ev_join = nullptr;
  hipStream_t stream_hi = nullptr, last_stream = nullptr;
  EvRef last;
  Frame work;
  uint32_t *pb_of = nullptr, *ticket = nullptr, *timeout = nullptr;
  unsigned long long* edge = nullptr;
  uint8_t *edge_tu = nullptr, *cuf = nullptr;
  int16_t* resbuf = nullptr;
  uint32_t* jobs = nullptr;
  uint16_t* sao_nb = nullptr;
  uint16_t* iplan = nullptr;
  uint32_t* job_base = nullptr;
  size_t cap_cb = 0, cap_u4 = 0, cap_edge = 0, cap_cuf = 0, cap_res = 0, cap_jobs = 0, cap_sao = 0, cap_iplan = 0, cap_jobbase = 0;
};

struct m355_ctx {
  int device = 0;
  Lane lanes[M355_MAX_LANES];
  int depth = 1, active = 0;
  std::vector<std::pair<uint32_t, uint32_t*>> inter_tabs;
  struct EvSlot { hipEvent_t ev = nullptr; unsigned long long ticket = 0; };
  EvSlot evring[M355_EV_RING];
  unsigned long long ev_ticket = 0;
  std::vector<Frame> frames;
  std::vector<Resident> resident;
  Resident transient[M355_TRANSIENT_MAX];
  int next_transient = 0;
  int transient_ring() const { return 3; }
  uint32_t epoch = 0;
  struct Status { unsigned long long serial = 0; uint32_t epoch = 0; bool validated = false, reported = false; EvRef done; };
  Status status[M355_STATUS_RING];
  uint32_t* status_words = nullptr;
  unsigned long long serial = 0;
  unsigned long long lost_first = 0; int lost_count = 0;
  int stages = M355_STAGE_ALL;
  int shard_rank = 0, shard_n = 0;
  m355_comm comm = {nullptr, nullptr, nullptr};
  void* rccl = nullptr;
  void* ipc = nullptr;
  int xchg_h = -1, xchg_k = -1;
  std::vector<hipEvent_t> evs;
  int ev_used = 0;
  bool timing_on = false;
  uint32_t* hash_acc = nullptr;
  struct HashSlot {
    unsigned long long ticket = 0; int type = 0, np = 0;
    int row_bytes[3] = {0, 0, 0}, rows[3] = {0, 0, 0};
    EvRef mark; int frame = -1;
    uint8_t* planes = nullptr; size_t planes_cap = 0;
  };
  HashSlot hash_slot[M355_HASH_REQUESTS];
  unsigned long long hash_ticket = 0;
  uint32_t *hash_rec = nullptr, *hash_res = nullptr;
  std::vector<std::pair<uint8_t*, size_t>> hash_pool;
  struct MeasSlot {
    unsigned long long ticket = 0;
    int np = 0, pw[3] = {0, 0, 0}, ph[3] = {0, 0, 0}, row0[3] = {0, 0, 0};
    EvRef mark; int frame[2] = {-1, -1};
    unsigned long long* rows = nullptr; size_t rows_cap = 0;
  };
  MeasSlot meas_slot[M355_MEASURE_REQUESTS];
  unsigned long long meas_ticket = 0;
  unsigned long long *meas_rec = nullptr, *meas_res = nullptr;
  std::vector<std::pair<unsigned long long*, size_t>> meas_pool;
  void* stage = nullptr; size_t stage_bytes = 0;
  struct BatchSlot { DevPic* host = nullptr; DevPic* dev = nullptr; uint32_t* ticket = nullptr; hipEvent_t ev = nullptr; bool pending = false; };
  BatchSlot batch[M355_BATCH_RING];
  int batch_next = 0;
  hipStream_t batch_stream[4] = {nullptr, nullptr, nullptr, nullptr};
  unsigned batch_count = 0;
  hipEvent_t batch_ev_pre[M355_MAX_LANES] = {};
  struct ScanCache { int ctbW = 0, ctbH = 0, ntc = 0, ntr = 0; decltype(m355_pic_params::col_bd) col_bd; decltype(m355_pic_params::row_bd) row_bd;
                     std::vector<uint32_t> ctb_ts, ts2rs; std::vector<uint16_t> tile_id; } scan;
};
static inline Lane& lane(m355_ctx* c) { return c->lanes[c->active]; }
static inline void select_lane(m355_ctx* c, int index) { c->active = index; }

struct TileRect { int x0, y0, x1, y1; };
struct Seg { const void* src; size_t bytes; size_t ofs; };
struct Lay {
  Seg seg[32];
  int ns;
  size_t total;
  int i_sl, i_ct, i_cu, i_tu, i_pb, i_wt, i_rb[4], i_ibin, i_ib, i_il, i_co, i_pc, i_sc, i_ts, i_rs, i_ti, i_iw, i_dp, i_ow;
};
struct Id128 { char b[128]; };
struct Rccl {
  void* so = nullptr;
  void* comm = nullptr;
  int (*GetUniqueId)(void*) = nullptr;
  int (*CommInitRank)(void**, int,  Id128, int) = nullptr;
  int (*CommDestroy)(void*) = nullptr;
  int (*GroupStart)() = nullptr;
  int (*GroupEnd)() = nullptr;
  int (*Send)(const void*, size_t, int, int, void*, void*) = nullptr;
  int (*Recv)(void*, size_t, int, int, void*, void*) = nullptr;
  int (*AllGather)(const void*, void*, size_t, int, void*, void*) = nullptr;
};
extern Rccl g_rccl;
int ipc_before_repack(m355_ctx* c, int h, hipStream_t st);
int ipc_end_picture(m355_ctx* c, int rc_own);
int ipc_before_free(m355_ctx* c, int h);
extern "C" int m355_shard_ipc_close(m355_ctx* c);
template <class T> static int grow(T** p, size_t* cap, size_t need, hipStream_t st, bool zero)
{
  if (need <= *cap) return M355_OK;
  HIPCHK(hipStreamSynchronize(st));
  if (*p) hipFree(*p);
  *p = nullptr;
  const size_t n = need + need / 4 + 64;
  HIPCHK(hipMalloc(p, n * sizeof(T)));
  if (zero) HIPCHK(hipMemsetAsync(*p, 0, n * sizeof(T), st));
  *cap = n;
  return M355_OK;
}

extern "C" {
void clear_target(m355_ctx* c, const DevPic& d, Frame* tgt, bool gated, hipStream_t st);
int copy_tiles(m355_ctx* c, const m355_pic_params& pp, Frame* f, int k0, int k1, int skip, int nranks, char* xbuf, size_t slot, bool to_slot);
int decode(m355_ctx* c, Resident& r, bool rotate = true);
void dst_hazards(m355_ctx* c, Frame* dstf, bool piped, hipStream_t st);
int ev_mark(m355_ctx* c, hipStream_t st, EvRef* out);
hipError_t ev_query(m355_ctx* c, const EvRef& r);
hipError_t ev_sync(m355_ctx* c, const EvRef& r);
void ev_wait(m355_ctx* c, hipStream_t st, const EvRef& r);
Frame* get_frame(m355_ctx* c, int h);
hipStream_t reader_begin(m355_ctx* c, Frame* f, int kind, const uint32_t** gate = nullptr, uint32_t* epoch = nullptr);
int reader_end(m355_ctx* c, Frame* f, int kind, hipStream_t st);
void readers_wait(m355_ctx* c, hipStream_t st, const Frame* f);
void halo_layout(const m355_pic_params& pp, HaloLayout& h);
int lane_class_priority(int index);
int lane_priorities_mode();
hipStream_t launch_prediction(m355_ctx* c, const Resident& r, const DevPic& d, bool hbd, hipStream_t st, hipEvent_t* ev, bool with_intra = true, hipStream_t chain = nullptr, Frame* hazard_dst = nullptr);
void make_layout(const m355_arena_caps& k, int nCtb, int halo_units, bool sharded, bool with_ib_input, Lay& L);
int mark_done(m355_ctx* c, Resident& r, Frame* dstf, hipStream_t st, const DevPic* d = nullptr);
int prepare(m355_ctx* c, Resident& r, DevPic& d_out, bool& want_sao_out, hipStream_t st);
size_t slot_bytes(const m355_pic_params& pp, int nranks);
int status_of(m355_ctx* c, m355_ctx::Status& s);
hipError_t sync_all(m355_ctx* c);
int upload(m355_ctx* c, Resident& r, const m355_picture* pic);
}

#endif
```

### libde265_amd/csrc/runtime_upload.hip

```cpp
#include "runtime_internal.h"
#include "record_checks.h"

extern "C" {

extern "C++" {
static int host_threads()
{
  static int n = 0;
  if (!n) {
    const unsigned hc = std::thread::hardware_concurrency();
    n = hc >= 128 ? 32 : (hc >= 32 ? 16 : (hc >= 16 ? 8 : (hc >= 4 ? 4 : 1)));
    if (const char* e = getenv("M355_HOST_THREADS")) { const int v = atoi(e); if (v >= 1 && v <= 64) n = v; }
  }
  return n;
}
struct HostPool {
  std::vector<std::thread> th;
  std::mutex mu;
  std::condition_variable cv_go, cv_done;
  const std::function<void(int)>* job = nullptr;
  int n_parts = 0, next = 0, pending = 0;
  unsigned long long gen = 0;
  std::atomic<unsigned long long> gen_hint{0};
  std::atomic<int> pending_hint{0};
  bool stop = false;
  explicit HostPool(int workers)
  {
    for (int i = 0; i < workers; i++) th.emplace_back([this]() { work(); });
  }
  ~HostPool()
  {
    { std::lock_guard<std::mutex> g(mu); stop = true; }
    cv_go.notify_all();
    for (auto& t : th) t.join();
  }
  static void cpu_relax()
  {
#if defined(__x86_64__) || defined(__i386__)
    __builtin_ia32_pause();
#endif
  }
  void work()
  {
    unsigned long long seen = 0;
    bool warm = false;
    std::unique_lock<std::mutex> lk(mu);
    for (;;) {
      if (warm && !stop && !(gen != seen && next < n_parts)) {
        lk.unlock();
        for (int spin = 0; spin < 4000 && gen_hint.load(std::memory_order_acquire) == seen; spin++) cpu_relax();
        lk.lock();
      }
      warm = false;
      cv_go.wait(lk, [&]() { return stop || (gen != seen && next < n_parts); });
      if (stop) return;
      while (next < n_parts) {
        const int part = next++;
        const std::function<void(int)>* f = job;
        lk.unlock();
        (*f)(part);
        lk.lock();
        warm = true;
        pending_hint.store(--pending, std::memory_order_release);
        if (pending == 0) cv_done.notify_all();
      }
      seen = gen;
    }
  }
  void run(int parts, const std::function<void(int)>& f)
  {
    std::unique_lock<std::mutex> lk(mu);
    job = &f; n_parts = parts; next = 0; pending = parts; gen++;
    pending_hint.store(parts, std::memory_order_relaxed);
    gen_hint.store(gen, std::memory_order_release);
    cv_go.notify_all();
    while (next < n_parts) {
      const int part = next++;
      lk.unlock();
      f(part);
      lk.lock();
      pending_hint.store(--pending, std::memory_order_release);
    }
    if (pending) {
      lk.unlock();
      for (int spin = 0; spin < 4000 && pending_hint.load(std::memory_order_acquire) != 0; spin++) cpu_relax();
      lk.lock();
    }
    cv_done.wait(lk, [&]() { return pending == 0; });
    job = nullptr; n_parts = 0;
  }
};
static HostPool* g_pool = nullptr;
static HostPool& host_pool()
{
  static std::once_flag once;
  std::call_once(once, []() { pthread_atfork(nullptr, nullptr, []() { g_pool = nullptr; }); });
  if (!g_pool) g_pool = new HostPool(host_threads() - 1);
  return *g_pool;
}
static std::mutex g_pool_mu;
template <class F> static void parallel_ranges(size_t n, size_t min_per_thread, F f)
{
  int T = host_threads();
  if (n < 2 * min_per_thread) T = 1;
  else if (n / min_per_thread < (size_t)T) T = (int)(n / min_per_thread);
  if (T <= 1) { f((size_t)0, n); return; }
  const std::function<void(int)> part = [&](int t) { f(n * (size_t)t / T, n * ((size_t)t + 1) / T); };
  std::unique_lock<std::mutex> g(g_pool_mu, std::try_to_lock);
  if (!g.owns_lock()) { f((size_t)0, n); return; }
  host_pool().run(T, part);
}
static void parallel_memcpy(void* dst, const void* src, size_t bytes)
{
  parallel_ranges(bytes, (size_t)1 << 20, [=](size_t b, size_t e) { memcpy((char*)dst + b, (const char*)src + b, e - b); });
}
}

static int validate(const m355_picture* pic, const m355_rb* const* rb_bin_in, bool records_on_device, int* ctbW_out, int* ctbH_out)
{
  const m355_pic_params& pp = pic->pp;
  if (pp.width <= 0 || pp.height <= 0 || pp.chroma_format_idc > 3) return fail(M355_ERR_INVALID, "bad picture size / chroma format");
  if (pp.log2_ctb_size < 4 || pp.log2_ctb_size > 6 || pp.log2_min_tb_size < 2 || pp.log2_min_tb_size > pp.log2_ctb_size ||
      pp.log2_min_cb_size < 3 || pp.log2_min_cb_size > pp.log2_ctb_size)
    return fail(M355_ERR_INVALID, "bad block-size parameters");
  if (pp.bit_depth_luma < 8 || pp.bit_depth_luma > 16 || pp.bit_depth_chroma < 8 || pp.bit_depth_chroma > 16) return fail(M355_ERR_INVALID, "bad bit depth");
  if ((pp.width & ((1 << pp.log2_min_cb_size) - 1)) || (pp.height & ((1 << pp.log2_min_cb_size) - 1)))
    return fail(M355_ERR_INVALID, "picture size %dx%d is not a multiple of the minimum coding block size %d", pp.width, pp.height, 1 << pp.log2_min_cb_size);
  if (pp.width > 65535 - 64 || pp.height > 65535 - 64) return fail(M355_ERR_INVALID, "picture larger than the 16-bit block coordinates allow");
  if (pic->n_pbs >= (1 << 25)) return fail(M355_ERR_INVALID, "too many prediction blocks (job words hold 25 index bits)");
  const int cs = 1 << pp.log2_ctb_size;
  const int ctbW = (pp.width + cs - 1) / cs, ctbH = (pp.height + cs - 1) / cs;
  if (pic->n_ctbs != ctbW * ctbH) return fail(M355_ERR_INVALID, "n_ctbs %d != %dx%d", pic->n_ctbs, ctbW, ctbH);
  if (pp.num_tile_cols < 1 || pp.num_tile_cols > M355_MAX_TILE_COLS || pp.num_tile_rows < 1 || pp.num_tile_rows > M355_MAX_TILE_ROWS)
    return fail(M355_ERR_INVALID, "bad tile counts");
  if (pp.col_bd[0] != 0 || pp.row_bd[0] != 0 || pp.col_bd[pp.num_tile_cols] != ctbW || pp.row_bd[pp.num_tile_rows] != ctbH)
    return fail(M355_ERR_INVALID, "tile boundaries do not cover the picture");
  for (int i = 0; i < pp.num_tile_cols; i++) if (pp.col_bd[i + 1] <= pp.col_bd[i]) return fail(M355_ERR_INVALID, "tile columns not increasing");
  for (int i = 0; i < pp.num_tile_rows; i++) if (pp.row_bd[i + 1] <= pp.row_bd[i]) return fail(M355_ERR_INVALID, "tile rows not increasing");
  if (pic->n_slices < 1) return fail(M355_ERR_INVALID, "no slices");
  if ((pp.flags & M355_PF_SCALING_LIST) && !pic->scaling_factors) return fail(M355_ERR_INVALID, "scaling list enabled but no factors");
  if (pic->n_cus < 0 || pic->n_tus < 0 || pic->n_pbs < 0 || pic->n_wts < 0 || pic->n_ibs < 0) return fail(M355_ERR_INVALID, "negative list length");
  const int sw = (pp.chroma_format_idc == 1 || pp.chroma_format_idc == 2) ? 2 : 1, sh = pp.chroma_format_idc == 1 ? 2 : 1;
  uint32_t ibsum = 0;
  for (int i = 0; i < pic->n_ctbs; i++) {
    const m355_ctb& c = pic->ctbs[i];
    if (c.slice_idx >= pic->n_slices) return fail(M355_ERR_INVALID, "ctb %d: slice index out of range", i);
    if ((uint64_t)c.ib_start + c.ib_count > (uint64_t)pic->n_ibs) return fail(M355_ERR_INVALID, "ctb %d: intra block range out of bounds", i);
    ibsum += c.ib_count;
  }
  if ((int)ibsum != pic->n_ibs) return fail(M355_ERR_INVALID, "intra blocks not all owned by a CTB");
  size_t nrb = 0, bin_end[4];
  for (int s = 0; s < 4; s++) { if (pic->rb_count[s] < 0) return fail(M355_ERR_INVALID, "negative rb_count"); nrb += (size_t)pic->rb_count[s]; bin_end[s] = nrb; }
  auto chk_ctb = [&](size_t i) -> const char* {
    const m355_ctb& c = pic->ctbs[i];
    const int cx = (int)i % ctbW, cy = (int)i / ctbW;
    for (uint32_t k = 0; k < c.ib_count; k++) {
      const m355_ib& ib = pic->ibs[c.ib_start + k];
      if (ib.cidx > 2 || ib.log2_size < 2 || ib.log2_size > 5) return "an intra block is malformed";
      const int csw = ib.cidx ? (sw == 2) : 0, csh = ib.cidx ? (sh == 2) : 0, n = 1 << ib.log2_size;
      const int x0 = (cx << pp.log2_ctb_size) >> csw, y0 = (cy << pp.log2_ctb_size) >> csh;
      if (ib.x < x0 || ib.y < y0 || ib.x + n > x0 + (cs >> csw) || ib.y + n > y0 + (cs >> csh)) return "an intra block lies outside the CTB";
    }
    return nullptr;
  };
  M355RecLimits lim = {pp.width, pp.height, sw, sh, pp.chroma_format_idc, pp.log2_min_cb_size, pp.log2_ctb_size, pic->n_wts,
                       pp.flags, pic->n_coeffs, pic->res_len, pic->n_pcm, 0};
  for (int i = 0; i < M355_MAX_REF_FRAMES; i++) if (pic->ref_frames[i] >= 0) lim.ref_mask |= 1u << i;
  const m355_rb* rb_bin[4];
  for (int b = 0; b < 4; b++) rb_bin[b] = rb_bin_in ? rb_bin_in[b] : pic->rbs + (b ? bin_end[b - 1] : 0);
  auto chk_rb = [&](size_t k) {
    const int s = k < bin_end[0] ? 0 : (k < bin_end[1] ? 1 : (k < bin_end[2] ? 2 : 3));
    return m355_check_rb(rb_bin[s][k - (s ? bin_end[s - 1] : 0)], s, lim);
  };
  const char* const names[7] = {"ctb", "cu", "tu", "pb", "weight", "rb", "ib"};
  const size_t rec = records_on_device ? 0 : 1;
  const size_t cnts[7] = {(size_t)pic->n_ctbs, rec * pic->n_cus, rec * pic->n_tus, rec * pic->n_pbs, rec * pic->n_wts, rec * nrb, rec * pic->n_ibs};
  size_t ofs[8];
  ofs[0] = 0;
  for (int q = 0; q < 7; q++) ofs[q + 1] = ofs[q] + cnts[q];
  std::atomic<size_t> first(ofs[7]);
  std::atomic<const char*> first_msg(nullptr);
  std::mutex mu;
  parallel_ranges(ofs[7], records_on_device ? 512 : 8192, [&](size_t b, size_t e) {
    for (int q = 0; q < 7; q++) {
      const size_t lo = std::max(b, ofs[q]), hi = std::min(e, ofs[q + 1]);
      if (lo >= hi || lo >= first.load(std::memory_order_relaxed)) continue;
      size_t bad = hi;
      const char* m = nullptr;
      const size_t base = ofs[q];
#define SWEEP(check, text) for (size_t g = lo; g < hi; g++) { const size_t i = g - base; if (auto r = (check)) { bad = g; m = (text); break; } }
      switch (q) {
        case 0: SWEEP(chk_ctb(i), r) break;
        case 1: SWEEP(m355_check_cu(pic->cus[i], lim), m355_rc_text[r]) break;
        case 2: SWEEP(m355_check_tu(pic->tus[i], lim), m355_rc_text[r]) break;
        case 3: SWEEP(m355_check_pb(pic->pbs[i], lim), m355_rc_text[r]) break;
        case 4: SWEEP(m355_check_wt(pic->wts[i], lim), m355_rc_text[r]) break;
        case 5: SWEEP(chk_rb(i), m355_rc_text[r]) break;
        default: SWEEP(m355_check_ib(pic->ibs[i], lim), m355_rc_text[r]) break;
      }
#undef SWEEP
      if (bad < hi) { std::lock_guard<std::mutex> gd(mu); if (bad < first.load()) { first.store(bad); first_msg.store(m); } return; }
    }
  });
  if (first.load() < ofs[7]) {
    int q = 0;
    while (first.load() >= ofs[q + 1]) q++;
    return fail(M355_ERR_INVALID, "%s %zu: %s", names[q], first.load() - ofs[q], first_msg.load());
  }
  *ctbW_out = ctbW; *ctbH_out = ctbH;
  return M355_OK;
}


static void intra_dependencies(int ctbW, int ctbH, const uint16_t* tile_id, const uint8_t* touch, const uint8_t* need, uint8_t* dep)
{
  const int nCtb = ctbW * ctbH;
  memset(dep, 0, (size_t)nCtb);
  for (int c = 0; c < nCtb; c++) {
    if (!need[c]) continue;
    const int cx = c % ctbW, cy = c / ctbW;
    const int dx[4] = {-1, -1, 0, 1}, dy[4] = {0, -1, -1, -1};
    const uint8_t tbit[4] = {1, 4, 2, 2};
    for (int n = 0; n < 4; n++) {
      const int nx = cx + dx[n], ny = cy + dy[n];
      if (nx < 0 || ny < 0 || nx >= ctbW) continue;
      const int nb = ny * ctbW + nx;
      if (tile_id[nb] != tile_id[c]) continue;
      if (((need[c] >> n) & 1) && (touch[nb] & tbit[n])) {
        dep[c] |= (uint8_t)(1 << n);
        dep[nb] |= 16;
      }
    }
  }
}

static int intra_schedule(const m355_picture* pic, int ctbW, int ctbH, m355_ib* out, uint32_t* aux, uint32_t* plan_count, uint8_t* log2_waves, uint8_t* touch, uint8_t* need, int* dense)
{
  const m355_pic_params& pp = pic->pp;
  const int sw = (pp.chroma_format_idc == 1 || pp.chroma_format_idc == 2) ? 2 : 1, sh = pp.chroma_format_idc == 1 ? 2 : 1;
  std::atomic<long long> n_blocks(0), n_intra_ctbs(0), n_levels(0);
  std::atomic<int> overlap(-1);
  const bool one_sided = !(pp.flags & M355_PF_CONSTRAINED_INTRA_PRED);
  const bool timed = one_sided && (size_t)pic->n_ibs >= 8 * (size_t)pic->n_ctbs;
  static const bool level_stats = getenv("M355_INTRA_LEVEL_STATS") != nullptr;
  double span[4] = {0, 0, 0, 0};
  std::mutex span_mu;
  std::vector<int32_t> edge_t;
  std::vector<uint16_t> tcol, trow;
  if (timed) {
    edge_t.assign((size_t)pic->n_ctbs * 96, -1);
    tcol.resize((size_t)ctbW); trow.resize((size_t)ctbH);
    for (int i = 0; i < pp.num_tile_cols; i++) for (int x = pp.col_bd[i]; x < pp.col_bd[i + 1] && x < ctbW; x++) tcol[(size_t)x] = (uint16_t)i;
    for (int i = 0; i < pp.num_tile_rows; i++) for (int y = pp.row_bd[i]; y < pp.row_bd[i + 1] && y < ctbH; y++) trow[(size_t)y] = (uint16_t)i;
  }
  constexpr int T_HANDOFF = 6, T_16 = 2, T_32 = 2;
  struct Scratch {
    std::vector<std::pair<uint32_t, uint32_t>> key, sorted;
    std::vector<int32_t> tstart, tvals;
    std::vector<uint32_t> histv;
    long long my_blocks = 0, my_ctbs = 0, my_levels = 0;
    double my_span[4] = {0, 0, 0, 0};
  };
  auto schedule_ctb = [&](size_t c, Scratch& S) {
    auto& key = S.key; auto& sorted = S.sorted;
    long long& my_blocks = S.my_blocks; long long& my_ctbs = S.my_ctbs; long long& my_levels = S.my_levels; double* const my_span = S.my_span;
    {
      const m355_ctb& ctb = pic->ctbs[c];
      log2_waves[c] = 0; plan_count[c] = 0; touch[c] = 0; need[c] = 0;
      if (!ctb.ib_count) return;
      my_ctbs++; my_blocks += ctb.ib_count;
      const int cx = (int)c % ctbW, cy = (int)c / ctbW;
      int8_t grid[3][16][16];
      int32_t tgrid[3][16][16];
      memset(grid, 0xFF, sizeof(grid));
      if (timed) { memset(tgrid, 0xFF, sizeof(tgrid)); S.tstart.assign(ctb.ib_count, 0); }
      key.clear();
      bool clash = false;
      for (uint32_t k = 0; k < ctb.ib_count; k++) {
        const m355_ib& ib = pic->ibs[ctb.ib_start + k];
        const int csw = ib.cidx ? (sw == 2) : 0, csh = ib.cidx ? (sh == 2) : 0;
        const int ux = (ib.x - ((cx << pp.log2_ctb_size) >> csw)) >> 2, uy = (ib.y - ((cy << pp.log2_ctb_size) >> csh)) >> 2;
        const int n4 = (1 << ib.log2_size) >> 2;
        int level = 0;
        {
          const int cw = (1 << pp.log2_ctb_size) >> csw, ch = (1 << pp.log2_ctb_size) >> csh, n = 1 << ib.log2_size;
          const int lx = ib.x - ((cx << pp.log2_ctb_size) >> csw), ly = ib.y - ((cy << pp.log2_ctb_size) >> csh);
          uint8_t t = 0, n_ = 0;
          if (lx + n == cw) t |= 1;
          if (ly + n == ch) t |= 2;
          if (lx + n == cw && ly + n == ch) t |= 4;
          if (!(ib.flags & M355_IBF_PCM)) {
            if (lx == 0) n_ |= 1;
            if (lx == 0 && ly == 0) n_ |= 2;
            if (ly == 0) n_ |= 4;
            if (ly == 0 && lx + 2 * n > cw) n_ |= 8;
          }
          touch[c] |= t; need[c] |= n_;
        }
        if (ux < 0 || uy < 0 || ux >= 16 || uy >= 16) { key.push_back(std::make_pair((uint32_t)ib.cidx, k)); continue; }
        if (!(ib.flags & M355_IBF_PCM)) {
          const int nT = 1 << ib.log2_size;
          int top_e = 2 * nT, left_e = 2 * nT;
          if (one_sided && !(ib.cidx == 0 && ib.log2_size == 5 && (pp.flags & M355_PF_STRONG_INTRA_SMOOTHING))) {
            const int m = ib.mode;
            bool filt = false;
            if (!(pp.flags & M355_PF_INTRA_SMOOTHING_DISABLED) && (ib.cidx == 0 || pp.chroma_format_idc == 3) && m != 1 && ib.log2_size != 2) {
              const int minDist = std::min(abs(m - 26), abs(m - 10));
              filt = ib.log2_size == 3 ? minDist > 7 : (ib.log2_size == 4 ? minDist > 1 : (ib.log2_size == 5 ? minDist > 0 : false));
            }
            const bool bf = ib.cidx == 0 && ib.log2_size < 5 && (m == 1 || !(ib.flags & M355_IBF_DISABLE_BOUNDARY_FILTER));
            static const int8_t mag[9] = {0, 2, 5, 9, 13, 17, 21, 26, 32};
            int te = 2 * nT, le = 2 * nT;
            if (m == 0) { te = nT + 1; le = 2 * nT; }
            else if (m == 1) { te = nT; le = nT; }
            else if (m > 10 && m < 26) { te = nT; le = nT; }
            else if (m == 26) { te = nT; le = (bf || uy == 0) ? nT : 0; }
            else if (m == 10) { le = nT; te = (bf || ux == 0) ? nT : 0; }
            else if (m > 26 && m <= 34) { te = std::min(2 * nT, nT + ((nT * mag[m - 26]) >> 5) + 2); le = uy > 0 ? 0 : 2 * nT; }
            else if (m >= 2 && m <= 9) { le = 2 * nT; te = ux > 0 ? 0 : 2 * nT; }
            if (filt) { if (te) te = std::min(2 * nT, te + 1); if (le) le = 2 * nT; }
            top_e = te; left_e = le;
          }
          const int top_u = (top_e + 3) >> 2, left_u = (left_e + 3) >> 2;
          if (!timed) for (int t = -1; t < 2 * n4; t++) {
            if (t < left_u && ux - 1 >= 0 && uy + t >= 0 && uy + t < 16) level = std::max(level, grid[ib.cidx][uy + t][ux - 1] + 1);
            if (t < top_u && uy - 1 >= 0 && ux + t >= 0 && ux + t < 16) level = std::max(level, grid[ib.cidx][uy - 1][ux + t] + 1);
          }
          if (timed) {
            int ute, ule;
            m355_intra_used_entries(ib.mode, ib.log2_size, ib.cidx, pp.chroma_format_idc, pp.flags, ib.flags, &ute, &ule);
            const int utop = (ute + 3) >> 2, uleft = (ule + 3) >> 2;
            const int cu = ((1 << pp.log2_ctb_size) >> csw) >> 2, cv = ((1 << pp.log2_ctb_size) >> csh) >> 2;
            int32_t ts = 0;
            auto nb_edge = [&](int dx, int dy, int slot) -> int32_t {
              const int nx = cx + dx, ny = cy + dy;
              if (nx < 0 || ny < 0 || nx >= ctbW || tcol[(size_t)nx] != tcol[(size_t)cx] || trow[(size_t)ny] != trow[(size_t)cy]) return -1;
              return edge_t[((size_t)ny * ctbW + nx) * 96 + (size_t)ib.cidx * 32 + slot];
            };
            for (int t = -1; t < 2 * n4; t++) {
              const int ly_ = uy + t, lx_ = ux + t;
              if (ux - 1 >= 0) { if (t < left_u && ly_ >= 0 && ly_ < 16) ts = std::max(ts, tgrid[ib.cidx][ly_][ux - 1]); }
              else if ((t < uleft || t == -1) && ly_ < cv) {
                const int32_t e = ly_ >= 0 ? nb_edge(-1, 0, ly_) : nb_edge(-1, -1, 16 + cu - 1);
                if (e >= 0) ts = std::max(ts, e + T_HANDOFF);
              }
              if (uy - 1 >= 0) { if (t < top_u && lx_ >= 0 && lx_ < 16) ts = std::max(ts, tgrid[ib.cidx][uy - 1][lx_]); }
              else if (t < utop || t == -1) {
                const int32_t e = lx_ < 0 ? nb_edge(-1, -1, 16 + cu - 1) : (lx_ < cu ? nb_edge(0, -1, 16 + lx_) : (lx_ - cu < cu ? nb_edge(1, -1, 16 + lx_ - cu) : -1));
                if (e >= 0) ts = std::max(ts, e + T_HANDOFF);
              }
            }
            S.tstart[k] = ts;
          }
        }
        if (timed) {
          const int32_t td = S.tstart[k] + (ib.log2_size >= 5 ? T_32 : (ib.log2_size == 4 ? T_16 : 1));
          for (int y = uy; y < uy + n4 && y < 16; y++) for (int x = ux; x < ux + n4 && x < 16; x++) tgrid[ib.cidx][y][x] = td;
        }
        level = std::min(level, 126);
        for (int y = uy; y < uy + n4 && y < 16; y++)
          for (int x = ux; x < ux + n4 && x < 16; x++) { if (grid[ib.cidx][y][x] >= 0) clash = true; grid[ib.cidx][y][x] = (int8_t)level; }
        key.push_back(std::make_pair(((uint32_t)level << 2) | ib.cidx, k));
      }
      if (clash) { int e = -1; overlap.compare_exchange_strong(e, (int)c); }
      if (timed) {
        int32_t tmin = INT32_MAX, tmax = 0;
        for (uint32_t k = 0; k < ctb.ib_count; k++) { tmin = std::min(tmin, S.tstart[k]); tmax = std::max(tmax, S.tstart[k]); }
        const size_t span_t = (size_t)(tmax - tmin) + 1;
        if (span_t <= 8192) {
          S.tvals.assign(span_t + 1, 0);
          for (uint32_t k = 0; k < ctb.ib_count; k++) S.tvals[(size_t)(S.tstart[k] - tmin)] = 1;
          int32_t r = 0;
          for (size_t i = 0; i < span_t; i++) { const int32_t u = S.tvals[i]; S.tvals[i] = r; r += u; }
          for (auto& e : key) e.first = ((uint32_t)S.tvals[(size_t)(S.tstart[e.second] - tmin)] << 2) | (e.first & 3u);
        } else {
          S.tvals.assign(S.tstart.begin(), S.tstart.end());
          std::sort(S.tvals.begin(), S.tvals.end());
          S.tvals.erase(std::unique(S.tvals.begin(), S.tvals.end()), S.tvals.end());
          for (auto& e : key) e.first = ((uint32_t)(std::lower_bound(S.tvals.begin(), S.tvals.end(), S.tstart[e.second]) - S.tvals.begin()) << 2) | (e.first & 3u);
        }
        int32_t* const et = &edge_t[c * 96];
        for (int q = 0; q < 3; q++) {
          const int csw = q ? (sw == 2) : 0, csh = q ? (sh == 2) : 0;
          const int cu = ((1 << pp.log2_ctb_size) >> csw) >> 2, cv = ((1 << pp.log2_ctb_size) >> csh) >> 2;
          for (int i = 0; i < 16; i++) { et[q * 32 + i] = i < cv ? tgrid[q][i][cu - 1] : -1; et[q * 32 + 16 + i] = i < cu ? tgrid[q][cv - 1][i] : -1; }
        }
      }
      {
        uint32_t kmax = 0;
        for (const auto& e : key) kmax = std::max(kmax, e.first);
        if (S.histv.size() < (size_t)kmax + 2) S.histv.resize((size_t)kmax + 2);
        uint32_t* const hist = S.histv.data();
        for (uint32_t i = 0; i <= kmax + 1; i++) hist[i] = 0;
        for (const auto& e : key) hist[e.first + 1]++;
        for (uint32_t i = 1; i <= kmax; i++) hist[i] += hist[i - 1];
        sorted.resize(key.size());
        for (const auto& e : key) sorted[hist[e.first]++] = e;
        key.swap(sorted);
      }
      uint32_t widest = 1, run = 0, rel = 0;
      for (uint32_t k = 0; k < ctb.ib_count; k++) {
        const m355_ib& ib = pic->ibs[ctb.ib_start + key[k].second];
        out[ctb.ib_start + k] = ib;
        const int csw_ = ib.cidx ? (sw == 2) : 0, csh_ = ib.cidx ? (sh == 2) : 0;
        const int cwc = (1 << pp.log2_ctb_size) >> csw_, chc = (1 << pp.log2_ctb_size) >> csh_, nT_ = 1 << ib.log2_size;
        const int lx_ = ib.x - ((cx << pp.log2_ctb_size) >> csw_), ly_ = ib.y - ((cy << pp.log2_ctb_size) >> csh_);
        uint32_t e0 = (uint32_t)(lx_ & 127) | ((uint32_t)(ly_ & 127) << 7) | ((uint32_t)(ib.log2_size & 7) << 14) | ((uint32_t)(ib.cidx & 3) << 17) | ((uint32_t)(ib.mode & 63) << 19);
        if (ib.flags & M355_IBF_HAS_RESIDUAL) e0 |= M355_IBX_HAS_RES;
        if (ib.flags & M355_IBF_PCM) e0 |= M355_IBX_PCM;
        if (ib.cidx == 0 && ib.log2_size < 5 && (ib.mode == 1 || !(ib.flags & M355_IBF_DISABLE_BOUNDARY_FILTER))) e0 |= M355_IBX_BFILT;
        if (lx_ + nT_ == cwc && cx + 1 < ctbW) e0 |= M355_IBX_PUB_COL;
        if (ly_ + nT_ == chc && cy + 1 < ctbH) e0 |= M355_IBX_PUB_ROW;
        if (!(ib.flags & M355_IBF_PCM) && !(pp.flags & M355_PF_INTRA_SMOOTHING_DISABLED) && (ib.cidx == 0 || pp.chroma_format_idc == 3) && ib.mode != 1 && ib.log2_size != 2) {
          const int minDist = std::min(abs((int)ib.mode - 26), abs((int)ib.mode - 10));
          const bool filt = ib.log2_size == 3 ? minDist > 7 : (ib.log2_size == 4 ? minDist > 1 : (ib.log2_size == 5 ? minDist > 0 : false));
          if (filt) e0 |= M355_IBX_FILT | (((pp.flags & M355_PF_STRONG_INTRA_SMOOTHING) && ib.cidx == 0 && ib.log2_size == 5) ? M355_IBX_STRONG : 0u);
        }
        int angle = 0, inv = 0;
        if (ib.mode >= 2 && ib.mode <= 34) {
          static const int8_t mag[9] = {0, 2, 5, 9, 13, 17, 21, 26, 32};
          static const int16_t invm[9] = {0, 4096, 1638, 910, 630, 482, 390, 315, 256};
          const int d = ib.mode >= 18 ? abs((int)ib.mode - 26) : abs((int)ib.mode - 10);
          const bool neg = ib.mode >= 18 ? ib.mode < 26 : ib.mode > 10;
          angle = neg ? -mag[d] : mag[d];
          inv = angle < 0 ? -invm[d] : 0;
        }
        uint32_t* ex = aux + 4 * (size_t)(ctb.ib_start + k);
        const uint32_t cls = ib.mode == 0 ? 0u : (ib.mode == 1 ? 1u : (angle == 0 ? 2u : (angle > 0 ? 3u : 4u)));
        ex[0] = e0; ex[1] = ib.res_ofs; ex[2] = ((uint32_t)(uint16_t)(int16_t)inv << 16) | (cls << 8) | (uint32_t)(uint8_t)(int8_t)angle;
        ex[3] = (rel & 0xFFFFu) | (((key[k].first >> 2) & 0x3FFFu) << 16);
        if (!(ib.flags & M355_IBF_PCM) && ib.log2_size >= 2 && ib.log2_size <= 5) rel += (4u << ib.log2_size) + 1u;
        run = (k && key[k].first == key[k - 1].first) ? run + 1 : 1;
        if ((key[k].first & 3) == 0) widest = std::max(widest, run);
        if (ib.log2_size >= M355_INTRA_SHARE_MIN_LOG2 && !(ib.flags & M355_IBF_PCM)) widest = std::max(widest, 8u);
      }
      plan_count[c] = rel;
      log2_waves[c] = widest >= 5 ? 3 : (widest >= 3 ? 2 : (widest == 2 ? 1 : 0));
      if (level_stats) {
        static const int GW[4][3] = {{8, 2, 2}, {8, 4, 4}, {12, 0, 0}, {16, 16, 16}};
        double ms[4] = {0, 0, 0, 0};
        uint32_t k0 = 0;
        while (k0 < ctb.ib_count) {
          uint32_t k1 = k0;
          while (k1 < ctb.ib_count && (key[k1].first >> 2) == (key[k0].first >> 2)) k1++;
          for (int pol = 0; pol < 4; pol++) {
            double load[3][16]; memset(load, 0, sizeof(load));
            int cnt[3] = {0, 0, 0};
            for (uint32_t k = k0; k < k1; k++) {
              const m355_ib& ib = pic->ibs[ctb.ib_start + key[k].second];
              const double cost = ib.log2_size >= 5 ? 4.5 : (ib.log2_size == 4 ? 2.0 : 1.0);
              const int comp = GW[pol][1] ? ib.cidx : 0;
              load[comp][cnt[comp]++ % GW[pol][comp]] += cost;
            }
            double m = 0;
            for (int a = 0; a < 3; a++) for (int b = 0; b < 16; b++) m = std::max(m, load[a][b]);
            ms[pol] += m;
          }
          k0 = k1;
        }
        for (int pol = 0; pol < 4; pol++) my_span[pol] += ms[pol];
      }
      if (ctb.ib_count) my_levels += (key[ctb.ib_count - 1].first >> 2) + 1;
    }
  };
  auto fold_stats = [&](const Scratch& S) {
    n_blocks += S.my_blocks; n_intra_ctbs += S.my_ctbs; n_levels += S.my_levels;
    if (level_stats) { std::lock_guard<std::mutex> lk(span_mu); for (int q = 0; q < 4; q++) span[q] += S.my_span[q]; }
  };
  if (!timed) {
    parallel_ranges((size_t)pic->n_ctbs, (size_t)pic->n_ibs >= 8 * (size_t)pic->n_ctbs ? 16 : 256, [&](size_t cb, size_t ce) {
      Scratch S;
      for (size_t c = cb; c < ce; c++) schedule_ctb(c, S);
      fold_stats(S);
    });
  } else {
    const size_t n = (size_t)pic->n_ctbs;
    std::vector<uint32_t> order(n);
    {
      std::vector<uint32_t> cnt((size_t)ctbW + 2 * (size_t)ctbH + 2, 0);
      for (size_t c = 0; c < n; c++) cnt[(c % ctbW) + 2 * (c / ctbW) + 1]++;
      for (size_t i = 1; i < cnt.size(); i++) cnt[i] += cnt[i - 1];
      for (size_t c = 0; c < n; c++) order[cnt[(c % ctbW) + 2 * (c / ctbW)]++] = (uint32_t)c;
    }
    std::unique_ptr<std::atomic<uint8_t>[]> done(new std::atomic<uint8_t>[n]);
    for (size_t c = 0; c < n; c++) done[c].store(0, std::memory_order_relaxed);
    std::atomic<size_t> next(0);
    const size_t parts = std::min<size_t>((size_t)std::max(1, host_threads()), std::max<size_t>(1, (size_t)std::min(ctbW, ctbH)));
    parallel_ranges(parts, 1, [&](size_t, size_t) {
      Scratch S;
      for (;;) {
        const size_t i = next.fetch_add(1, std::memory_order_relaxed);
        if (i >= n) break;
        const size_t c = order[i];
        const int cx = (int)(c % ctbW), cy = (int)(c / ctbW);
        const size_t dep[2] = {cx > 0 ? c - 1 : n, cy > 0 ? (cx + 1 < ctbW ? c - ctbW + 1 : c - ctbW) : n};
        for (int d = 0; d < 2; d++)
          if (dep[d] < n) while (!done[dep[d]].load(std::memory_order_acquire)) std::this_thread::yield();
        schedule_ctb(c, S);
        done[c].store(1, std::memory_order_release);
      }
      fold_stats(S);
    });
  }
  {
    const bool stats = level_stats;
    if (stats) fprintf(stderr, "intra_schedule: level makespans in block units, waves 8+2+2: %.0f, 8+4+4: %.0f, 12 shared: %.0f, 16 shared: %.0f\n", span[0], span[1], span[2], span[3]);
    if (stats) fprintf(stderr, "intra_schedule: %lld blocks in %lld CTBs, %lld levels (one-sided %d)\n", n_blocks.load(), n_intra_ctbs.load(), n_levels.load(), (int)one_sided);
  }
  *dense = (n_intra_ctbs.load() && n_blocks.load() >= 8 * (long)ctbW * ctbH) ? 1 : 0;
  return overlap.load();
}

static size_t al(size_t v) { return (v + 255) & ~(size_t)255; }
void halo_layout(const m355_pic_params& pp, HaloLayout& h) {
  memset(&h, 0, sizeof(h));
  const int cf = pp.chroma_format_idc;
  const int sw = (cf == 1 || cf == 2) ? 2 : 1, sh = cf == 1 ? 2 : 1;
  const int cs = 1 << pp.log2_ctb_size;
  h.n_vb = pp.num_tile_cols - 1; h.n_hb = pp.num_tile_rows - 1;
  int col = 0, row = 0;
  for (int c = 0; c < 3; c++) {
    h.col_ofs[c] = col; h.row_ofs[c] = row;
    if (c && cf == 0) continue;
    const int pw = c ? pp.width / sw : pp.width, ph = c ? pp.height / sh : pp.height;
    h.hw[c] = c ? 4 / sw : 4; h.hh[c] = c ? 4 / sh : 4;
    for (int b = 0; b < h.n_vb; b++) h.xb[c][b] = (pp.col_bd[b + 1] * cs) / (c ? sw : 1);
    for (int b = 0; b < h.n_hb; b++) h.yb[c][b] = (pp.row_bd[b + 1] * cs) / (c ? sh : 1);
    col += h.n_vb * ph * 2 * h.hw[c];
    row += h.n_hb * 2 * h.hh[c] * pw;
  }
  h.col_ofs[3] = col; h.row_ofs[3] = row;
  const int w4 = (pp.width + 3) / 4, h4 = (pp.height + 3) / 4;
  h.n_units = 2 * h.n_vb * h4 + 2 * h.n_hb * w4;
}

static void caps_of(const m355_picture* pic, m355_arena_caps& k)
{
  memset(&k, 0, sizeof(k));
  k.n_slices = pic->n_slices; k.n_ctbs = pic->n_ctbs; k.n_cus = pic->n_cus; k.n_tus = pic->n_tus; k.n_pbs = pic->n_pbs; k.n_wts = pic->n_wts;
  for (int b = 0; b < 4; b++) k.n_rbs[b] = pic->rb_count[b];
  k.n_ibs = pic->n_ibs; k.n_coeffs = pic->n_coeffs; k.n_pcm = pic->n_pcm; k.scaling = pic->scaling_factors != nullptr;
}
void make_layout(const m355_arena_caps& k, int nCtb, int halo_units, bool sharded, bool with_ib_input, Lay& L) {
  L.ns = 0; L.total = 0;
  auto add = [&](size_t bytes) { L.seg[L.ns].src = nullptr; L.seg[L.ns].bytes = 0; L.seg[L.ns].ofs = L.total; L.total += al(bytes ? bytes : 1); return L.ns++; };
  L.i_sl = add(sizeof(m355_slice) * (size_t)k.n_slices);
  L.i_ct = add(sizeof(m355_ctb) * (size_t)k.n_ctbs);
  L.i_cu = add(sizeof(m355_cu) * ((size_t)k.n_cus + (size_t)halo_units));
  L.i_tu = add(sizeof(m355_tu) * (size_t)k.n_tus);
  L.i_pb = add(sizeof(m355_pb) * ((size_t)k.n_pbs + (size_t)halo_units));
  L.i_wt = add(sizeof(m355_wt) * (size_t)k.n_wts);
  for (int b = 0; b < 4; b++) L.i_rb[b] = add(sizeof(m355_rb) * (size_t)k.n_rbs[b]);
  L.i_ibin = add(with_ib_input ? sizeof(m355_ib) * (size_t)k.n_ibs : 0);
  L.i_ib = add(sizeof(m355_ib) * (size_t)k.n_ibs);
  L.i_il = add(16 * (size_t)k.n_ibs);
  L.i_co = add(4 * (size_t)k.n_coeffs);
  L.i_pc = add(2 * (size_t)k.n_pcm);
  L.i_sc = add(k.scaling ? 6 * (16 + 64 + 256 + 1024) : 0);
  L.i_ts = add(4 * (size_t)nCtb);
  L.i_rs = add(4 * (size_t)nCtb);
  L.i_ti = add(2 * (size_t)nCtb);
  L.i_iw = add(sizeof(DevIntraWork) * (size_t)nCtb);
  L.i_dp = add((size_t)nCtb);
  L.i_ow = add(sharded ? (size_t)nCtb : 0);
}

int upload(m355_ctx* c, Resident& r, const m355_picture* pic) {
  static const bool prof = getenv("M355_PROFILE_UPLOAD") != nullptr;
  auto now = []() { return std::chrono::steady_clock::now(); };
  auto ms = [](std::chrono::steady_clock::time_point a, std::chrono::steady_clock::time_point b) { return std::chrono::duration<double, std::milli>(b - a).count(); };
  const auto t_start = now();
  const m355_pic_params& pp = pic->pp;
  const bool in_place = r.arena && r.host && pic->n_ctbs > 0 && (const char*)pic->ctbs >= r.host && (const char*)pic->ctbs < r.host + r.cap;
  int ctbW, ctbH;
  r.device_validate = in_place && c->shard_n < 1;
  int rc = validate(pic, in_place ? (const m355_rb* const*)r.caps.rb_bin : nullptr, r.device_validate, &ctbW, &ctbH);
  if (rc) return rc;
  const auto t_valid = now();
  const int nCtb = ctbW * ctbH;
  const bool sharded = c->shard_n >= 1;
  HaloLayout halo;
  memset(&halo, 0, sizeof(halo));
  if (sharded) halo_layout(pp, halo);
  m355_arena_caps cp;
  caps_of(pic, cp);
  if (in_place) {
    const m355_arena_caps& k = r.caps;
    if (halo.n_units != r.arena_halo_units) return fail(M355_ERR_INVALID, "in-place submit: the arena was laid out for another tile structure (m355_picture_arena_begin's pp)");
    if (cp.n_slices > k.n_slices || cp.n_ctbs > k.n_ctbs || cp.n_cus > k.n_cus || cp.n_tus > k.n_tus || cp.n_pbs > k.n_pbs || cp.n_wts > k.n_wts ||
        cp.n_rbs[0] > k.n_rbs[0] || cp.n_rbs[1] > k.n_rbs[1] || cp.n_rbs[2] > k.n_rbs[2] || cp.n_rbs[3] > k.n_rbs[3] || cp.n_ibs > k.n_ibs ||
        cp.n_coeffs > k.n_coeffs || cp.n_pcm > k.n_pcm || (cp.scaling && !k.scaling))
      return fail(M355_ERR_INVALID, "lists exceed the capacities given to m355_arena_begin");
    cp = k;
  }
  Lay L;
  make_layout(cp, nCtb, halo.n_units, sharded, in_place, L);
  Seg* seg = L.seg;
  const int ns = L.ns;
  const size_t total = L.total;
  const int i_sl = L.i_sl, i_ct = L.i_ct, i_cu = L.i_cu, i_tu = L.i_tu, i_pb = L.i_pb, i_wt = L.i_wt, i_ib = L.i_ib, i_il = L.i_il, i_co = L.i_co, i_pc = L.i_pc,
            i_sc = L.i_sc, i_ts = L.i_ts, i_rs = L.i_rs, i_ti = L.i_ti, i_iw = L.i_iw, i_dp = L.i_dp, i_ow = L.i_ow;
  {
    size_t rb_o = 0;
    const void* srcs[32]; size_t used[32];
    for (int i = 0; i < ns; i++) { srcs[i] = nullptr; used[i] = 0; }
    srcs[i_sl] = pic->slices; used[i_sl] = sizeof(m355_slice) * (size_t)pic->n_slices;
    srcs[i_ct] = pic->ctbs; used[i_ct] = sizeof(m355_ctb) * (size_t)pic->n_ctbs;
    srcs[i_cu] = pic->cus; used[i_cu] = sizeof(m355_cu) * (size_t)pic->n_cus;
    srcs[i_tu] = pic->tus; used[i_tu] = sizeof(m355_tu) * (size_t)pic->n_tus;
    srcs[i_pb] = pic->pbs; used[i_pb] = sizeof(m355_pb) * (size_t)pic->n_pbs;
    srcs[i_wt] = pic->wts; used[i_wt] = sizeof(m355_wt) * (size_t)pic->n_wts;
    for (int b = 0; b < 4; b++) { srcs[L.i_rb[b]] = pic->rbs + rb_o; used[L.i_rb[b]] = sizeof(m355_rb) * (size_t)pic->rb_count[b]; rb_o += (size_t)pic->rb_count[b]; }
    used[i_ib] = sizeof(m355_ib) * (size_t)pic->n_ibs; used[i_il] = 16 * (size_t)pic->n_ibs;
    srcs[i_co] = pic->coeffs; used[i_co] = 4 * (size_t)pic->n_coeffs;
    srcs[i_pc] = pic->pcm; used[i_pc] = 2 * (size_t)pic->n_pcm;
    srcs[i_sc] = pic->scaling_factors; used[i_sc] = pic->scaling_factors ? 6 * (16 + 64 + 256 + 1024) : 0;
    used[i_ts] = used[i_rs] = 4 * (size_t)nCtb; used[i_iw] = sizeof(DevIntraWork) * (size_t)nCtb;    used[i_ti] = 2 * (size_t)nCtb; used[i_dp] = (size_t)nCtb;
    used[i_ow] = sharded ? (size_t)nCtb : 0;
    for (int i = 0; i < ns; i++) { seg[i].src = srcs[i]; seg[i].bytes = used[i]; }
    if (in_place) {
      const void* want[] = {pic->slices, pic->ctbs, pic->cus, pic->tus, pic->pbs, pic->wts, pic->coeffs, pic->pcm};
      const int idx[] = {i_sl, i_ct, i_cu, i_tu, i_pb, i_wt, i_co, i_pc};
      for (int k = 0; k < 8; k++)
        if (seg[idx[k]].bytes && want[k] != (const void*)(r.host + seg[idx[k]].ofs)) return fail(M355_ERR_INVALID, "in-place submit: a list is not where m355_arena_begin put it");
      if (pic->n_ibs && pic->ibs != (const m355_ib*)(r.host + seg[L.i_ibin].ofs)) return fail(M355_ERR_INVALID, "in-place submit: ibs[] is not where m355_arena_begin put it");
      if (pic->rbs != (const m355_rb*)(r.host + seg[L.i_rb[0]].ofs)) return fail(M355_ERR_INVALID, "in-place submit: rbs must point at the first size bin's region");
      if (pic->scaling_factors && pic->scaling_factors != (const uint8_t*)(r.host + seg[i_sc].ofs)) return fail(M355_ERR_INVALID, "in-place submit: scaling_factors is not where m355_arena_begin put it");
      for (int i = 0; i < ns; i++) seg[i].src = nullptr;
    }
  }

  hipSetDevice(c->device);
  if (total > r.cap) {
    if (r.dev || r.host) HIPCHK(sync_all(c));
    if (r.dev) hipFree(r.dev);
    if (r.host) hipHostFree(r.host);
    r.dev = r.host = nullptr;
    r.cap = total + total / 4;
    HIPCHK(hipMalloc(&r.dev, r.cap));
    HIPCHK(hipHostMalloc(&r.host, r.cap, hipHostMallocDefault));
  } else if (r.done.ticket) {
    HIPCHK(ev_sync(c, r.done));
    r.done = EvRef();
  }
  const auto t_wait = now();
  for (int i = 0; i < ns; i++)
    if (seg[i].src && seg[i].bytes) parallel_memcpy(r.host + seg[i].ofs, seg[i].src, seg[i].bytes);
  const auto t_copy = now();
  r.sched_u8.resize((size_t)nCtb * 3); r.sched_u32.resize((size_t)nCtb);
  uint8_t* const log2_waves = r.sched_u8.data(); uint8_t* const ctb_touch = log2_waves + nCtb; uint8_t* const ctb_need = ctb_touch + nCtb;
  uint32_t* const plan_count = r.sched_u32.data();
  int intra_dense = 0;
  {
    const int bad = intra_schedule(pic, ctbW, ctbH, (m355_ib*)(r.host + seg[i_ib].ofs), (uint32_t*)(r.host + seg[i_il].ofs), plan_count, log2_waves, ctb_touch, ctb_need, &intra_dense);
    if (bad >= 0) return fail(M355_ERR_INVALID, "ctb %d: intra blocks overlap", bad);
    const uint32_t cap = (uint32_t)M355_INTRA_PLAN_CAP(pp.chroma_format_idc);
    for (int i = 0; i < nCtb; i++) if (plan_count[(size_t)i] > cap) return fail(M355_ERR_INVALID, "ctb %d: more intra blocks than a CTB holds", i);
  }
  const auto t_sched = now();
  uint32_t* ctb_ts = (uint32_t*)(r.host + seg[i_ts].ofs);
  uint32_t* ts2rs = (uint32_t*)(r.host + seg[i_rs].ofs);
  uint16_t* tile_id = (uint16_t*)(r.host + seg[i_ti].ofs);
  DevIntraWork* iw = (DevIntraWork*)(r.host + seg[i_iw].ofs);
  {
    m355_ctx::ScanCache& sc = c->scan;
    const bool same = sc.ctbW == ctbW && sc.ctbH == ctbH && sc.ntc == pp.num_tile_cols && sc.ntr == pp.num_tile_rows &&
                      !memcmp(sc.col_bd, pp.col_bd, sizeof(pp.col_bd)) && !memcmp(sc.row_bd, pp.row_bd, sizeof(pp.row_bd));
    if (!same) {
      sc.ctbW = ctbW; sc.ctbH = ctbH; sc.ntc = pp.num_tile_cols; sc.ntr = pp.num_tile_rows;
      memcpy(sc.col_bd, pp.col_bd, sizeof(pp.col_bd)); memcpy(sc.row_bd, pp.row_bd, sizeof(pp.row_bd));
      sc.ctb_ts.assign((size_t)nCtb, 0); sc.ts2rs.assign((size_t)nCtb, 0); sc.tile_id.assign((size_t)nCtb, 0);
      uint32_t ts = 0; int tidx = 0;
      for (int ty = 0; ty < pp.num_tile_rows; ty++)
        for (int tx = 0; tx < pp.num_tile_cols; tx++) {
          for (int y = pp.row_bd[ty]; y < pp.row_bd[ty + 1]; y++)
            for (int x = pp.col_bd[tx]; x < pp.col_bd[tx + 1]; x++) {
              sc.ctb_ts[y * ctbW + x] = ts; sc.ts2rs[ts] = (uint32_t)(y * ctbW + x); sc.tile_id[y * ctbW + x] = (uint16_t)tidx; ts++;
            }
          tidx++;
        }
    }
    memcpy(ctb_ts, sc.ctb_ts.data(), 4 * (size_t)nCtb); memcpy(ts2rs, sc.ts2rs.data(), 4 * (size_t)nCtb); memcpy(tile_id, sc.tile_id.data(), 2 * (size_t)nCtb);
  }
  intra_dependencies(ctbW, ctbH, tile_id, ctb_touch, ctb_need, (uint8_t*)(r.host + seg[i_dp].ofs));
  for (int i = 0; i < nCtb; i++) ((uint8_t*)(r.host + seg[i_dp].ofs))[i] |= (uint8_t)(log2_waves[i] << 5);
  const auto t_deps = now();
  int nw = 0, n_free = 0, n_ticket = 0;
  uint32_t n_iplan = 0;
  {
    const uint8_t* dep = (const uint8_t*)(r.host + seg[i_dp].ofs);
    std::vector<uint32_t>& order = r.sched_order;
    std::vector<uint32_t>& cand = r.sched_cand;
    cand.clear();
    uint32_t max_cnt = 0;
    size_t n_dep = 0;
    for (int t = 0; t < nCtb; t++) {
      const uint32_t rs = ts2rs[t], cnt = pic->ctbs[rs].ib_count;
      if (!cnt) continue;
      const bool free_ctb = !(dep[rs] & 15);
      cand.push_back(rs); cand.push_back(cnt | (free_ctb ? 0x80000000u : 0u));
      if (free_ctb) max_cnt = std::max(max_cnt, cnt); else n_dep++;
    }
    const size_t n_cand = cand.size() / 2;
    order.resize(n_cand);
    std::vector<uint32_t>& bucket = r.sched_bucket;
    if (!intra_dense) {
      std::vector<uint32_t>& rem = r.sched_u32b;
      rem.assign((size_t)nCtb, 0);
      const uint32_t* const aux = (const uint32_t*)(r.host + seg[i_il].ofs);
      constexpr uint32_t REM_CAP = 4095, T_HANDOFF_LEVELS = 6;
      for (size_t i = n_cand; i-- > 0;) {
        const uint32_t rs = cand[2 * i];
        if (!(dep[rs] & 31)) continue;
        const m355_ctb& cb = pic->ctbs[rs];
        const uint32_t levels = ((aux[4 * (size_t)(cb.ib_start + cb.ib_count - 1) + 3] >> 16) & 0x3FFFu) + 1u;
        const uint32_t mine = std::min(REM_CAP, rem[rs] + levels + T_HANDOFF_LEVELS);
        rem[rs] = mine;
        const int cx = (int)rs % ctbW, cy = (int)rs / ctbW;
        const int dx[4] = {-1, -1, 0, 1}, dy[4] = {0, -1, -1, -1};
        for (int n = 0; n < 4; n++)
          if ((dep[rs] >> n) & 1) { uint32_t& pr = rem[(size_t)(cy + dy[n]) * ctbW + (cx + dx[n])]; pr = std::max(pr, mine); }
      }
      bucket.assign((size_t)REM_CAP + 2 + (size_t)max_cnt + 2, 0);
      size_t n_chain = 0;
      auto slot_of = [&](size_t i) -> size_t {
        const uint32_t rs = cand[2 * i];
        return (dep[rs] & 31) ? (size_t)(REM_CAP - rem[rs]) : (size_t)REM_CAP + 1 + (size_t)(max_cnt - (cand[2 * i + 1] & 0x7FFFFFFFu));
      };
      for (size_t i = 0; i < n_cand; i++) { bucket[slot_of(i) + 1]++; if (dep[cand[2 * i]] & 31) n_chain++; }
      for (size_t i = 1; i < bucket.size(); i++) bucket[i] += bucket[i - 1];
      for (size_t i = 0; i < n_cand; i++) order[bucket[slot_of(i)]++] = cand[2 * i];
      n_ticket = (int)n_chain;
    } else {
    n_free = (int)(n_cand - n_dep);
    n_ticket = (int)n_cand;
    {
      bucket.assign((size_t)max_cnt + 2, 0);
      for (size_t i = 0; i < n_cand; i++) if (cand[2 * i + 1] >> 31) bucket[(size_t)(max_cnt - (cand[2 * i + 1] & 0x7FFFFFFFu)) + 1]++;
      for (size_t i = 1; i < bucket.size(); i++) bucket[i] += bucket[i - 1];
      for (size_t i = 0; i < n_cand; i++) if (cand[2 * i + 1] >> 31) order[bucket[max_cnt - (cand[2 * i + 1] & 0x7FFFFFFFu)]++] = cand[2 * i];
    }
    if (n_dep) {
      std::vector<int> tx0((size_t)pp.num_tile_cols * pp.num_tile_rows), ty0(tx0.size());
      for (int ty = 0, t = 0; ty < pp.num_tile_rows; ty++)
        for (int tx = 0; tx < pp.num_tile_cols; tx++, t++) { tx0[t] = pp.col_bd[tx]; ty0[t] = pp.row_bd[ty]; }
      auto wkey = [&](uint32_t rs) { const int cx = (int)rs % ctbW, cy = (int)rs / ctbW, ti = tile_id[rs]; return (uint32_t)((cx - tx0[ti]) + 2 * (cy - ty0[ti])); };
      bucket.assign((size_t)ctbW + 2 * (size_t)ctbH + 2, 0);
      for (size_t i = 0; i < n_cand; i++) if (!(cand[2 * i + 1] >> 31)) bucket[(size_t)wkey(cand[2 * i]) + 1]++;
      for (size_t i = 1; i < bucket.size(); i++) bucket[i] += bucket[i - 1];
      for (size_t i = 0; i < n_cand; i++) if (!(cand[2 * i + 1] >> 31)) order[(size_t)n_free + bucket[wkey(cand[2 * i])]++] = cand[2 * i];
    }
    }
    nw = (int)order.size();
    std::vector<uint32_t>& pbase = r.sched_u32b;
    pbase.resize((size_t)nw + 1);
    for (int k = 0; k < nw; k++) { pbase[(size_t)k] = n_iplan; n_iplan += (plan_count[order[(size_t)k]] + 7u) & ~7u; }
    parallel_ranges((size_t)nw, 512, [&](size_t kb, size_t ke) {
      for (size_t k = kb; k < ke; k++) {
        const uint32_t rs = order[k];
        DevIntraWork w;
        memset(&w, 0, sizeof(w));
        w.ctb = rs; w.ib_start = pic->ctbs[rs].ib_start; w.ib_count = pic->ctbs[rs].ib_count;
        w.waves_code = (uint8_t)(log2_waves[rs] & 3);
        w.plan_base = pbase[k]; w.plan_count = plan_count[rs];
        const int cx = (int)rs % ctbW, cy = (int)rs / ctbW;
        const uint32_t my_sa = pic->slices[pic->ctbs[rs].slice_idx].slice_addr_rs;
        for (int q = 0; q < 9; q++) {
          const int nx = cx + q % 3 - 1, ny = cy + q / 3 - 1;
          if (nx < 0 || ny < 0 || nx >= ctbW || ny >= ctbH) continue;
          const int n = ny * ctbW + nx;
          if (pic->slices[pic->ctbs[n].slice_idx].slice_addr_rs == my_sa && tile_id[n] == tile_id[rs]) w.nb_same |= (uint16_t)(1u << q);
          if (ctb_ts[n] < ctb_ts[rs]) w.nb_earlier |= (uint16_t)(1u << q);
        }
        iw[k] = w;
      }
    });
  }
  seg[i_iw].bytes = sizeof(DevIntraWork) * (size_t)(nw ? nw : 1);
  r.n_intra_work = nw; r.n_iplan = n_iplan;
  if (sharded) {
    uint8_t* ow = (uint8_t*)(r.host + seg[i_ow].ofs);
    const int n_tiles = pp.num_tile_cols * pp.num_tile_rows;
    for (int i = 0; i < nCtb; i++) ow[i] = m355_shard_owner_of_tile(tile_id[i], n_tiles, c->shard_n) == c->shard_rank;
    for (int i = 0; i < pic->n_cus; i++)
      if (!ow[(pic->cus[i].y >> pp.log2_ctb_size) * ctbW + (pic->cus[i].x >> pp.log2_ctb_size)])
        return fail(M355_ERR_INVALID, "sharded picture: cu %d lies in a tile of another rank", i);
    for (int i = 0; i < nCtb; i++)
      if (!ow[i] && pic->ctbs[i].ib_count) return fail(M355_ERR_INVALID, "sharded picture: ctb %d of another rank has intra blocks", i);
  }
  r.sharded = sharded; r.shard_rank = c->shard_rank; r.shard_n = c->shard_n; r.halo = halo; r.live_valid = false; r.xprev = nullptr;
  r.bytes = total; r.fresh = true; r.refs_valid = false;
  if (prof) fprintf(stderr, "m355 upload%s: validate %.3f ms, wait/alloc %.3f, copy %.3f (%.1f MB), intra schedule %.3f, tables + dependencies %.3f, work list + jobs %.3f\n",
                    in_place ? " (in place)" : "", ms(t_start, t_valid), ms(t_valid, t_wait), ms(t_wait, t_copy), total / 1e6, ms(t_copy, t_sched), ms(t_sched, t_deps), ms(t_deps, now()));
  {
    size_t run_b = 0, run_e = 0;
    for (int i = 0; i <= ns; i++) {
      const bool used = i < ns && seg[i].bytes && i != L.i_ibin;
      const size_t b = used ? seg[i].ofs : 0, e = used ? seg[i].ofs + seg[i].bytes : 0;
      if (used && run_e > run_b && b - run_e <= 4096) { run_e = e; continue; }
      if (run_e > run_b) HIPCHK(hipMemcpyAsync(r.dev + run_b, r.host + run_b, run_e - run_b, hipMemcpyHostToDevice, lane(c).stream));
      run_b = b; run_e = e;
    }
  }
  {
    const int rcm = ev_mark(c, lane(c).stream, &r.up);
    if (rcm) return rcm;
  }

  r.hdr = *pic;
  DevPic& d = r.dp;
  memset(&d, 0, sizeof(d));
  d.pp = dev_pic_params(pp);
  d.sw = (pp.chroma_format_idc == 1 || pp.chroma_format_idc == 2) ? 2 : 1;
  d.sh = pp.chroma_format_idc == 1 ? 2 : 1;
  d.ctbW = ctbW; d.ctbH = ctbH; d.nCtb = nCtb;
  d.w4 = (pp.width + 3) / 4; d.h4 = (pp.height + 3) / 4;
  d.wcb = (pp.width + (1 << pp.log2_min_cb_size) - 1) >> pp.log2_min_cb_size;
  d.hcb = (pp.height + (1 << pp.log2_min_cb_size) - 1) >> pp.log2_min_cb_size;
  d.slices = (const m355_slice*)(r.dev + seg[i_sl].ofs);
  d.ctbs = (const m355_ctb*)(r.dev + seg[i_ct].ofs);
  d.cus = (const m355_cu*)(r.dev + seg[i_cu].ofs);
  d.tus = (const m355_tu*)(r.dev + seg[i_tu].ofs);
  d.pbs = (const m355_pb*)(r.dev + seg[i_pb].ofs);
  d.wts = (const m355_wt*)(r.dev + seg[i_wt].ofs);
  for (int b = 0; b < 4; b++) d.rb_bin[b] = (const m355_rb*)(r.dev + seg[L.i_rb[b]].ofs);
  d.ibs = (const m355_ib*)(r.dev + seg[i_ib].ofs);
  d.ib_aux = (const uint32_t*)(r.dev + seg[i_il].ofs);
  d.intra_dense = intra_dense;
  d.coeffs = (const uint32_t*)(r.dev + seg[i_co].ofs);
  d.pcm = (const uint16_t*)(r.dev + seg[i_pc].ofs);
  d.scaling = pic->scaling_factors ? (const uint8_t*)(r.dev + seg[i_sc].ofs) : nullptr;
  d.n_cus = pic->n_cus; d.n_tus = pic->n_tus; d.n_pbs = pic->n_pbs; d.n_ibs = pic->n_ibs;
  for (int s = 0; s < 4; s++) d.rb_count[s] = pic->rb_count[s];
  d.ctb_ts = (const uint32_t*)(r.dev + seg[i_ts].ofs);
  d.ts2rs = (const uint32_t*)(r.dev + seg[i_rs].ofs);
  d.tile_id = (const uint16_t*)(r.dev + seg[i_ti].ofs);
  d.intra_work = (const DevIntraWork*)(r.dev + seg[i_iw].ofs);
  d.n_intra_work = nw; d.n_intra_ticket = n_ticket;
  d.ctb_dep = (const uint8_t*)(r.dev + seg[i_dp].ofs);
  d.ctb_owner = sharded ? (const uint8_t*)(r.dev + seg[i_ow].ofs) : nullptr;
  d.halo_cu_base = pic->n_cus; d.halo_pb_base = pic->n_pbs;
  d.n_pb_records = pic->n_pbs + halo.n_units;
  d.device_validate = r.device_validate ? 1 : 0;
  d.n_wts = pic->n_wts; d.n_coeffs = pic->n_coeffs; d.n_pcm = pic->n_pcm; d.res_len = pic->res_len;
  r.used = true;
  return M355_OK;
}

}
```

Before: 25.82 million CTB64/s.

## Split independent intra CTBs into per-wave light items per color plane

Independent CTBs with no dependencies and no 32x32+ intra blocks are no longer given a whole workgroup each. They become per-plane light items, each handled by a single wave through a new light kernel path. The host scheduler now sorts heavy free CTBs ahead of light ones and builds a uint4 light work list. The shared prediction code is moved into header helpers so both paths can use it. This aims to raise parallelism and cut workgroup overhead for sparse intra, at the cost of extra host scheduling work and a larger upload segment.

```diff
diff --git a/libde265_amd/csrc/k_common.h b/libde265_amd/csrc/k_common.h
--- a/libde265_amd/csrc/k_common.h
+++ b/libde265_amd/csrc/k_common.h
@@ -115,6 +115,8 @@
   uint32_t epoch;
   const DevIntraWork* intra_work;
   int n_intra_work, n_intra_ticket;
+  int n_intra_heavy, n_intra_light;
+  const uint4* intra_light;
   int intra_grid;
   int intra_keeper;
   int test_halo_late;
diff --git a/libde265_amd/csrc/k_intra.hip b/libde265_amd/csrc/k_intra.hip
--- a/libde265_amd/csrc/k_intra.hip
+++ b/libde265_amd/csrc/k_intra.hip
@@ -4,6 +4,8 @@
 #include "k_meta_tu.h"
 
 #include "k_intra_plan.h"
+#include "k_intra_block.h"
+#include "k_intra_light.h"
 typedef unsigned long long m355_granule;
 
 __device__ __forceinline__ m355_granule* d_edge_col(const DevPic& p, int c, int col, int y) { return p.edge + p.edge_col_ofs[c] + (size_t)col * (size_t)(p.ph[c] >> 1) + (size_t)(y >> 1); }
@@ -71,6 +73,13 @@
   __shared__ uint16_t s_kp_h1[(DENSE && NW == M355_INTRA_KEEPER_NW) ? 5 * 64 : 1];
 
   const int wv = __builtin_amdgcn_readfirstlane((int)(threadIdx.x >> 6)), lane = threadIdx.x & 63;
+
+  if constexpr (!DENSE && !BATCH && !W16) {
+    if ((int)blockIdx.x >= p0.n_intra_heavy) {
+      k_intra_light_item<PIX, CF>(p0, ((int)blockIdx.x - p0.n_intra_heavy) * NW + wv, s_raw[wv], s_f[wv]);
+      return;
+    }
+  }
 
   for (;;) {
   int item = (int)blockIdx.x, pk = 0;
@@ -492,7 +501,7 @@
       const int lx = (int)(e0 & 127u), ly = (int)((e0 >> 7) & 127u);
 
       auto small_block = [&](auto l2_) {
-        constexpr int LOG2 = decltype(l2_)::value, NT = 1 << LOG2, Z = 2 * NT, NENT = 4 * NT + 1;
+        constexpr int LOG2 = decltype(l2_)::value, NT = 1 << LOG2;
         const int x = lane & (NT - 1), y = lane >> LOG2;
         const bool inb = lane < NT * NT;
         uint32_t bv = bv0;
@@ -505,47 +514,7 @@
             bv = d_poll_halo(d_edge_row(p, cs, ctbY - 1, 0), d_edge_col(p, cs, ctbX - 1, 0), p.timeout, halo, (int)code0 - HALO_BASE, bv, pending, x0c, y0c, epoch);
         }
         PROF_T(1);
-        {
-          const uint32_t nb = (uint32_t)__builtin_amdgcn_update_dpp(0, (int)bv, 0x138, 0xF, 0xF, false) + (uint32_t)__builtin_amdgcn_update_dpp(0, (int)bv, 0x130, 0xF, 0xF, false);
-          const uint32_t fbv = (nb + 2u * bv + 2u) >> 2;
-          if ((e0 & M355_IBX_FILT) && lane > 0 && lane < NENT - 1) bv = fbv;
-        }
-#define BRL(i) ((int)__builtin_amdgcn_readlane((int)bv, (i) + Z))
-#define BRP(i) ((int)__builtin_amdgcn_ds_bpermute(((i) + Z) << 2, (int)bv))
-        int v;
-        if (__builtin_expect(cls >= 3, 1)) {
-          const int a_ = vert ? y : x, b_ = vert ? x : y;
-          const int tt = __mul24(a_ + 1, angle), iIdx = tt >> 5, iFact = tt & 31;
-          const int x1 = b_ + iIdx + 1, x2 = x1 + 1;
-          const int p1 = (__mul24(x1, inv) + 128) >> 8, p2 = (__mul24(x2, inv) + 128) >> 8;
-          int i1 = x1 >= 0 ? x1 : -p1, i2 = x2 >= 0 ? x2 : -p2;
-          if (!vert) { i1 = -i1; i2 = -i2; }
-          const int r1 = BRP(i1), r2 = BRP(i2);
-          v = (32 * r1 + __mul24(iFact, r2 - r1) + 16) >> 5;
-        } else if (cls == 0) {
-          const int l = BRP(-1 - y), t = BRP(1 + x), tr = BRL(1 + NT), bl = BRL(-1 - NT);
-          v = (__mul24(NT - 1 - x, l) + __mul24(x + 1, tr) + __mul24(NT - 1 - y, t) + __mul24(y + 1, bl) + NT) >> (LOG2 + 1);
-        } else if (cls == 1) {
-          int s_ = (lane >= Z - NT && lane <= Z + NT && lane != Z) ? (int)bv : 0;
-          s_ += __builtin_amdgcn_update_dpp(0, s_, 0xB1, 0xF, 0xF, false);
-          s_ += __builtin_amdgcn_update_dpp(0, s_, 0x4E, 0xF, 0xF, false);
-          s_ += __builtin_amdgcn_update_dpp(0, s_, 0x141, 0xF, 0xF, false);
-          s_ += __builtin_amdgcn_update_dpp(0, s_, 0x140, 0xF, 0xF, false);
-          int sum = __builtin_amdgcn_readlane(s_, 0) + __builtin_amdgcn_readlane(s_, 16);
-          const int dc = (sum + NT) >> (LOG2 + 1);
-          v = dc;
-          if (bfilt) {
-            const int eb = BRP(y == 0 ? x + 1 : -y - 1), e2c = BRL(-1) + BRL(1);
-            if (x == 0 || y == 0) v = (eb + 3 * dc + 2) >> 2;
-            if (lane == 0) v = (e2c + 2 * dc + 2) >> 2;
-          }
-        } else {
-          const int l = BRP(-1 - y), t = BRP(1 + x), corner = BRL(0), first = vert ? BRL(1) : BRL(-1);
-          v = vert ? t : l;
-          if (bfilt && (vert ? x == 0 : y == 0)) v = d_clip3(0, pix_max, first + (((vert ? l : t) - corner) >> 1));
-        }
-#undef BRL
-#undef BRP
+        int v = d_intra_small_predict<LOG2>(bv, e0, cls, angle, inv, vert, bfilt, pix_max);
         v = d_clip3(0, pix_max, v + rs);
         if (inb) body[d_baddr] = (uint16_t)v;
         if (__builtin_expect((e0 & (M355_IBX_PUB_COL | M355_IBX_PUB_ROW)) != 0, 0)) {
@@ -570,7 +539,7 @@
       const int it_lo = shared ? (nPass * g) / G : 0, it_hi = shared ? (nPass * (g + 1)) / G : nPass;
       if (!(e0 & M355_IBX_PCM)) {
         if (it_lo < it_hi) {
-        const int nEnt = 4 * nT + 1, Z = 2 * nT;
+        const int nEnt = 4 * nT + 1;
         const uint16_t* pl = s_plan + ((e3 & 0xFFFFu) - plan_lo);
         uint32_t cd[3] = {0, 0, 0}, val[3] = {0, 0, 0};
 #pragma unroll
@@ -603,88 +572,32 @@
         PROF_T(1);
         uint16_t* P = raw;
         if (e0 & M355_IBX_FILT) {
-          const bool bi = (e0 & M355_IBX_STRONG) && d_abs((int)raw[Z] + raw[Z + 64] - 2 * raw[Z + 32]) < thr_strong && d_abs((int)raw[Z] + raw[Z - 64] - 2 * raw[Z - 32]) < thr_strong;
-#pragma unroll
-          for (int q = 0; q < 3; q++) {
-            if (64 * q >= nEnt) continue;
-            const int e = lane + 64 * q;
-            if (e < nEnt) {
-              const int i = e - Z;
-              int v;
-              if (i == -Z || i == Z) v = raw[e];
-              else if (bi) {
-                if (i == 0) v = raw[Z];
-                else if (i < 0) v = raw[Z] + (((-i) * ((int)raw[Z - 64] - raw[Z]) + 32) >> 6);
-                else v = raw[Z] + ((i * ((int)raw[Z + 64] - raw[Z]) + 32) >> 6);
-              } else v = (raw[e + 1] + 2 * raw[e] + raw[e - 1] + 2) >> 2;
-              pf[e] = (uint16_t)v;
-            }
-          }
+          d_intra_big_filter(raw, pf, e0, nT, thr_strong);
           wave_sync();
           P = pf;
         }
-#define BRD(i) ((int)P[(i) + Z])
-        int dcVal = 0;
-        if (mode == 1) {
-          int s_ = 0;
-          if (lane < nT) s_ = BRD(lane + 1) + BRD(-lane - 1);
-          s_ += __builtin_amdgcn_update_dpp(0, s_, 0xB1, 0xF, 0xF, false);
-          s_ += __builtin_amdgcn_update_dpp(0, s_, 0x4E, 0xF, 0xF, false);
-          s_ += __builtin_amdgcn_update_dpp(0, s_, 0x141, 0xF, 0xF, false);
-          s_ += __builtin_amdgcn_update_dpp(0, s_, 0x140, 0xF, 0xF, false);
-          dcVal = (__builtin_amdgcn_readlane(s_, 0) + __builtin_amdgcn_readlane(s_, 16) + nT) >> (log2 + 1);
-        }
+        const int dcVal = mode == 1 ? d_intra_big_dc(P, nT, log2) : 0;
         {
           const int xb = lane & (nT - 1), yb = lane >> log2, ystep = 64 >> log2, nIt = (nT * nT) >> 6;
           const int res_on = has_res ? -1 : 0;
           auto big_loop = [&](auto cls_) {
             constexpr int CLS = decltype(cls_)::value;
             const int x = xb;
-            const int t_x = (CLS == 0 || CLS == 2) ? BRD(1 + x) : 0;
-            const int u_tr = CLS == 0 ? BRD(1 + nT) : 0, u_bl = CLS == 0 ? BRD(-1 - nT) : 0;
-            const int u_c = CLS == 2 ? BRD(0) : 0, u_f = CLS == 2 ? (vert ? BRD(1) : BRD(-1)) : 0;
-            const int u_e2 = CLS == 1 ? BRD(-1) + BRD(1) : 0;
+            const IntraBigFixed fx = d_intra_big_fixed<CLS>(P, nT, x, vert);
             (void)nIt;
             for (int it0 = it_lo; it0 < it_hi; it0 += 4) {
               int ta[4], tb[4], fa[4], rs[4];
 #pragma unroll
               for (int u = 0; u < 4; u++) {
                 const int y = yb + min(it0 + u, it_hi - 1) * ystep;
-                fa[u] = 0; tb[u] = 0;
-                if (CLS == 0 || CLS == 2) ta[u] = BRD(-1 - y);
-                else if (CLS == 1) ta[u] = BRD(y == 0 ? x + 1 : -y - 1);
-                else {
-                  const int a_ = vert ? y : x, b_ = vert ? x : y;
-                  const int tt = __mul24(a_ + 1, angle), iIdx = tt >> 5;
-                  fa[u] = tt & 31;
-                  const int x1 = b_ + iIdx + 1, x2 = x1 + 1;
-                  int i1, i2;
-                  if (CLS == 3) { i1 = vert ? x1 : -x1; i2 = vert ? x2 : -x2; }
-                  else {
-                    const int p1 = (__mul24(x1, inv) + 128) >> 8, p2 = (__mul24(x2, inv) + 128) >> 8;
-                    i1 = x1 >= 0 ? x1 : -p1; i2 = x2 >= 0 ? x2 : -p2;
-                    if (!vert) { i1 = -i1; i2 = -i2; }
-                  }
-                  ta[u] = BRD(i1); tb[u] = BRD(fa[u] ? i2 : i1);
-                }
+                d_intra_big_taps<CLS>(P, nT, x, y, vert, angle, inv, ta[u], tb[u], fa[u]);
                 rs[u] = (int)(int16_t)body[d_bofs + y * BODY_PITCH + x] & res_on;
                 if (res32) rs[u] = has_res ? res32buf[e1 + y * nT + x] : 0;
               }
 #pragma unroll
               for (int u = 0; u < 4; u++) {
                 const int y = yb + min(it0 + u, it_hi - 1) * ystep;
-                int v;
-                if (CLS == 0) v = (__mul24(nT - 1 - x, ta[u]) + __mul24(x + 1, u_tr) + __mul24(nT - 1 - y, t_x) + __mul24(y + 1, u_bl) + nT) >> (log2 + 1);
-                else if (CLS == 1) {
-                  v = dcVal;
-                  if (bfilt) {
-                    if (x == 0 || y == 0) v = (ta[u] + 3 * dcVal + 2) >> 2;
-                    if (x == 0 && y == 0) v = (u_e2 + 2 * dcVal + 2) >> 2;
-                  }
-                } else if (CLS == 2) {
-                  v = vert ? t_x : ta[u];
-                  if (bfilt && (vert ? x == 0 : y == 0)) v = d_clip3(0, pix_max, u_f + (((vert ? ta[u] : t_x) - u_c) >> 1));
-                } else v = (32 * ta[u] + __mul24(fa[u], tb[u] - ta[u]) + 16) >> 5;
+                int v = d_intra_big_value<CLS>(fx, nT, log2, x, y, vert, bfilt, dcVal, pix_max, ta[u], tb[u], fa[u]);
                 v = d_clip3(0, pix_max, v + rs[u]);
                 body[d_bofs + y * BODY_PITCH + x] = (uint16_t)v;
               }
@@ -696,7 +609,6 @@
           else if (cls == 3) big_loop(std::integral_constant<int, 3>());
           else big_loop(std::integral_constant<int, 4>());
         }
-#undef BRD
         }
       } else {
         for (int o = lane; o < nT * nT; o += 64) {
@@ -761,7 +673,10 @@
   const dim3 dense_grid(p.intra_grid > 0 && p.intra_grid < p.n_intra_work ? p.intra_grid : p.n_intra_work);
   if (p.intra_dense && p.intra_keeper) hipLaunchKernelGGL(HIP_KERNEL_NAME(k_intra<PIX, CF, M355_INTRA_KEEPER_NW, true, false, W16>), dense_grid, dim3(64 * M355_INTRA_KEEPER_NW), 0, st, p, p.n_intra_work, (const DevPic*)nullptr, 1, (uint32_t*)nullptr);
   else if (p.intra_dense) hipLaunchKernelGGL(HIP_KERNEL_NAME(k_intra<PIX, CF, M355_INTRA_DENSE_NW, true, false, W16>), dense_grid, dim3(64 * M355_INTRA_DENSE_NW), 0, st, p, p.n_intra_work, (const DevPic*)nullptr, 1, (uint32_t*)nullptr);
-  else hipLaunchKernelGGL(HIP_KERNEL_NAME(k_intra<PIX, CF, M355_INTRA_SPARSE_NW, false, false, W16>), dim3(p.n_intra_work), dim3(64 * M355_INTRA_SPARSE_NW), 0, st, p, p.n_intra_work, (const DevPic*)nullptr, 1, (uint32_t*)nullptr);
+  else {
+    const int n_wg = p.n_intra_heavy + (W16 ? 0 : (p.n_intra_light + M355_INTRA_SPARSE_NW - 1) / M355_INTRA_SPARSE_NW);
+    hipLaunchKernelGGL(HIP_KERNEL_NAME(k_intra<PIX, CF, M355_INTRA_SPARSE_NW, false, false, W16>), dim3(n_wg), dim3(64 * M355_INTRA_SPARSE_NW), 0, st, p, p.n_intra_heavy, (const DevPic*)nullptr, 1, (uint32_t*)nullptr);
+  }
 }
 
 void m355_launch_intra(const DevPic& p, bool hbd, hipStream_t st, bool ticket_zero)
diff --git a/libde265_amd/csrc/k_intra_block.h b/libde265_amd/csrc/k_intra_block.h
--- /dev/null
+++ b/libde265_amd/csrc/k_intra_block.h
@@ -0,0 +1,143 @@
+#ifndef M355_K_INTRA_BLOCK_H
+#define M355_K_INTRA_BLOCK_H
+#include "k_common.h"
+
+template <int LOG2>
+__device__ __forceinline__ int d_intra_small_predict(uint32_t bv, const uint32_t e0, const int cls, const int angle, const int inv, const bool vert, const bool bfilt, const int pix_max)
+{
+  constexpr int NT = 1 << LOG2, Z = 2 * NT, NENT = 4 * NT + 1;
+  const int lane = threadIdx.x & 63;
+  const int x = lane & (NT - 1), y = lane >> LOG2;
+  {
+    const uint32_t nb = (uint32_t)__builtin_amdgcn_update_dpp(0, (int)bv, 0x138, 0xF, 0xF, false) + (uint32_t)__builtin_amdgcn_update_dpp(0, (int)bv, 0x130, 0xF, 0xF, false);
+    const uint32_t fbv = (nb + 2u * bv + 2u) >> 2;
+    if ((e0 & M355_IBX_FILT) && lane > 0 && lane < NENT - 1) bv = fbv;
+  }
+#define BRL(i) ((int)__builtin_amdgcn_readlane((int)bv, (i) + Z))
+#define BRP(i) ((int)__builtin_amdgcn_ds_bpermute(((i) + Z) << 2, (int)bv))
+  int v;
+  if (__builtin_expect(cls >= 3, 1)) {
+    const int a_ = vert ? y : x, b_ = vert ? x : y;
+    const int tt = __mul24(a_ + 1, angle), iIdx = tt >> 5, iFact = tt & 31;
+    const int x1 = b_ + iIdx + 1, x2 = x1 + 1;
+    const int p1 = (__mul24(x1, inv) + 128) >> 8, p2 = (__mul24(x2, inv) + 128) >> 8;
+    int i1 = x1 >= 0 ? x1 : -p1, i2 = x2 >= 0 ? x2 : -p2;
+    if (!vert) { i1 = -i1; i2 = -i2; }
+    const int r1 = BRP(i1), r2 = BRP(i2);
+    v = (32 * r1 + __mul24(iFact, r2 - r1) + 16) >> 5;
+  } else if (cls == 0) {
+    const int l = BRP(-1 - y), t = BRP(1 + x), tr = BRL(1 + NT), bl = BRL(-1 - NT);
+    v = (__mul24(NT - 1 - x, l) + __mul24(x + 1, tr) + __mul24(NT - 1 - y, t) + __mul24(y + 1, bl) + NT) >> (LOG2 + 1);
+  } else if (cls == 1) {
+    int s_ = (lane >= Z - NT && lane <= Z + NT && lane != Z) ? (int)bv : 0;
+    s_ += __builtin_amdgcn_update_dpp(0, s_, 0xB1, 0xF, 0xF, false);
+    s_ += __builtin_amdgcn_update_dpp(0, s_, 0x4E, 0xF, 0xF, false);
+    s_ += __builtin_amdgcn_update_dpp(0, s_, 0x141, 0xF, 0xF, false);
+    s_ += __builtin_amdgcn_update_dpp(0, s_, 0x140, 0xF, 0xF, false);
+    int sum = __builtin_amdgcn_readlane(s_, 0) + __builtin_amdgcn_readlane(s_, 16);
+    const int dc = (sum + NT) >> (LOG2 + 1);
+    v = dc;
+    if (bfilt) {
+      const int eb = BRP(y == 0 ? x + 1 : -y - 1), e2c = BRL(-1) + BRL(1);
+      if (x == 0 || y == 0) v = (eb + 3 * dc + 2) >> 2;
+      if (lane == 0) v = (e2c + 2 * dc + 2) >> 2;
+    }
+  } else {
+    const int l = BRP(-1 - y), t = BRP(1 + x), corner = BRL(0), first = vert ? BRL(1) : BRL(-1);
+    v = vert ? t : l;
+    if (bfilt && (vert ? x == 0 : y == 0)) v = d_clip3(0, pix_max, first + (((vert ? l : t) - corner) >> 1));
+  }
+#undef BRL
+#undef BRP
+  return v;
+}
+
+__device__ __forceinline__ void d_intra_big_filter(const uint16_t* raw, uint16_t* pf, const uint32_t e0, const int nT, const int thr_strong)
+{
+  const int lane = threadIdx.x & 63;
+  const int nEnt = 4 * nT + 1, Z = 2 * nT;
+  const bool bi = (e0 & M355_IBX_STRONG) && d_abs((int)raw[Z] + raw[Z + 64] - 2 * raw[Z + 32]) < thr_strong && d_abs((int)raw[Z] + raw[Z - 64] - 2 * raw[Z - 32]) < thr_strong;
+#pragma unroll
+  for (int q = 0; q < 3; q++) {
+    if (64 * q >= nEnt) continue;
+    const int e = lane + 64 * q;
+    if (e < nEnt) {
+      const int i = e - Z;
+      int v;
+      if (i == -Z || i == Z) v = raw[e];
+      else if (bi) {
+        if (i == 0) v = raw[Z];
+        else if (i < 0) v = raw[Z] + (((-i) * ((int)raw[Z - 64] - raw[Z]) + 32) >> 6);
+        else v = raw[Z] + ((i * ((int)raw[Z + 64] - raw[Z]) + 32) >> 6);
+      } else v = (raw[e + 1] + 2 * raw[e] + raw[e - 1] + 2) >> 2;
+      pf[e] = (uint16_t)v;
+    }
+  }
+}
+
+#define M355_BRD(i) ((int)P[(i) + Z])
+__device__ __forceinline__ int d_intra_big_dc(const uint16_t* P, const int nT, const int log2)
+{
+  const int lane = threadIdx.x & 63, Z = 2 * nT;
+  int s_ = 0;
+  if (lane < nT) s_ = M355_BRD(lane + 1) + M355_BRD(-lane - 1);
+  s_ += __builtin_amdgcn_update_dpp(0, s_, 0xB1, 0xF, 0xF, false);
+  s_ += __builtin_amdgcn_update_dpp(0, s_, 0x4E, 0xF, 0xF, false);
+  s_ += __builtin_amdgcn_update_dpp(0, s_, 0x141, 0xF, 0xF, false);
+  s_ += __builtin_amdgcn_update_dpp(0, s_, 0x140, 0xF, 0xF, false);
+  return (__builtin_amdgcn_readlane(s_, 0) + __builtin_amdgcn_readlane(s_, 16) + nT) >> (log2 + 1);
+}
+struct IntraBigFixed { int t_x, u_tr, u_bl, u_c, u_f, u_e2; };
+template <int CLS>
+__device__ __forceinline__ IntraBigFixed d_intra_big_fixed(const uint16_t* P, const int nT, const int x, const bool vert)
+{
+  const int Z = 2 * nT;
+  IntraBigFixed f;
+  f.t_x = (CLS == 0 || CLS == 2) ? M355_BRD(1 + x) : 0;
+  f.u_tr = CLS == 0 ? M355_BRD(1 + nT) : 0; f.u_bl = CLS == 0 ? M355_BRD(-1 - nT) : 0;
+  f.u_c = CLS == 2 ? M355_BRD(0) : 0; f.u_f = CLS == 2 ? (vert ? M355_BRD(1) : M355_BRD(-1)) : 0;
+  f.u_e2 = CLS == 1 ? M355_BRD(-1) + M355_BRD(1) : 0;
+  return f;
+}
+template <int CLS>
+__device__ __forceinline__ void d_intra_big_taps(const uint16_t* P, const int nT, const int x, const int y, const bool vert, const int angle, const int inv, int& ta, int& tb, int& fa)
+{
+  const int Z = 2 * nT;
+  fa = 0; tb = 0;
+  if (CLS == 0 || CLS == 2) ta = M355_BRD(-1 - y);
+  else if (CLS == 1) ta = M355_BRD(y == 0 ? x + 1 : -y - 1);
+  else {
+    const int a_ = vert ? y : x, b_ = vert ? x : y;
+    const int tt = __mul24(a_ + 1, angle), iIdx = tt >> 5;
+    fa = tt & 31;
+    const int x1 = b_ + iIdx + 1, x2 = x1 + 1;
+    int i1, i2;
+    if (CLS == 3) { i1 = vert ? x1 : -x1; i2 = vert ? x2 : -x2; }
+    else {
+      const int p1 = (__mul24(x1, inv) + 128) >> 8, p2 = (__mul24(x2, inv) + 128) >> 8;
+      i1 = x1 >= 0 ? x1 : -p1; i2 = x2 >= 0 ? x2 : -p2;
+      if (!vert) { i1 = -i1; i2 = -i2; }
+    }
+    ta = M355_BRD(i1); tb = M355_BRD(fa ? i2 : i1);
+  }
+}
+#undef M355_BRD
+template <int CLS>
+__device__ __forceinline__ int d_intra_big_value(const IntraBigFixed& f, const int nT, const int log2, const int x, const int y, const bool vert, const bool bfilt, const int dcVal, const int pix_max, const int ta, const int tb, const int fa)
+{
+  int v;
+  if (CLS == 0) v = (__mul24(nT - 1 - x, ta) + __mul24(x + 1, f.u_tr) + __mul24(nT - 1 - y, f.t_x) + __mul24(y + 1, f.u_bl) + nT) >> (log2 + 1);
+  else if (CLS == 1) {
+    v = dcVal;
+    if (bfilt) {
+      if (x == 0 || y == 0) v = (ta + 3 * dcVal + 2) >> 2;
+      if (x == 0 && y == 0) v = (f.u_e2 + 2 * dcVal + 2) >> 2;
+    }
+  } else if (CLS == 2) {
+    v = vert ? f.t_x : ta;
+    if (bfilt && (vert ? x == 0 : y == 0)) v = d_clip3(0, pix_max, f.u_f + (((vert ? ta : f.t_x) - f.u_c) >> 1));
+  } else v = (32 * ta + __mul24(fa, tb - ta) + 16) >> 5;
+  return v;
+}
+
+#endif
diff --git a/libde265_amd/csrc/k_intra_light.h b/libde265_amd/csrc/k_intra_light.h
--- /dev/null
+++ b/libde265_amd/csrc/k_intra_light.h
@@ -0,0 +1,135 @@
+#ifndef M355_K_INTRA_LIGHT_H
+#define M355_K_INTRA_LIGHT_H
+#include "k_common.h"
+#include "k_intra_plan.h"
+#include "k_intra_block.h"
+
+template <class PIX, int CF>
+__device__ __forceinline__ uint32_t d_light_gather(const PIX* plane, const int stride, const int pw, const int ph, const int x0c, const int y0c, const int cs, const uint32_t code, const uint32_t cval)
+{
+  constexpr int PITCH_L = BODY_PITCH_OF(MAXCTB), PITCH_C = BODY_PITCH_OF(IntraGeo<CF>::CW_C);
+  const int HALO_BASE = cs == 0 ? IntraGeo<CF>::BODY_L : IntraGeo<CF>::BODY_C;
+  int sx, sy;
+  bool konst = false;
+  if ((int)code < HALO_BASE) {
+    sy = cs == 0 ? (int)(code / (uint32_t)PITCH_L) : (int)(code / (uint32_t)PITCH_C);
+    sx = (int)code - sy * (cs == 0 ? PITCH_L : PITCH_C) - BODY_X0;
+  } else if ((int)code < HALO_BASE + HALO_TOP_N) { sy = -1; sx = (int)code - HALO_BASE - 1; }
+  else if ((int)code < HALO_BASE + HALO_N) { sx = -1; sy = (int)code - HALO_BASE - HALO_TOP_N; }
+  else { konst = true; sx = sy = 0; }
+  const int x = min(max(x0c + sx, 0), pw - 1), y = min(max(y0c + sy, 0), ph - 1);
+  const uint32_t v = (uint32_t)__hip_atomic_load(plane + (size_t)y * stride + x, __ATOMIC_RELAXED, __HIP_MEMORY_SCOPE_AGENT);
+  return konst ? cval : v;
+}
+
+template <class PIX, int CF>
+__device__ __forceinline__ void k_intra_light_item(const DevPic& p, const int slot, uint16_t* raw, uint16_t* pf)
+{
+  const int lane = threadIdx.x & 63;
+  if (slot >= p.n_intra_light) return;
+  const uint4 it = p.intra_light[slot];
+  const int ctb = __builtin_amdgcn_readfirstlane((int)(it.x & 0x3FFFFFFFu)), c = __builtin_amdgcn_readfirstlane((int)(it.x >> 30));
+  const uint32_t ib_first = (uint32_t)__builtin_amdgcn_readfirstlane((int)it.y), ib_n = (uint32_t)__builtin_amdgcn_readfirstlane((int)it.z);
+  const uint32_t plan_base = (uint32_t)__builtin_amdgcn_readfirstlane((int)it.w);
+  const int ctbX = ctb % p.ctbW, ctbY = ctb / p.ctbW;
+  const int l2c = p.pp.log2_ctb_size;
+  const int csw = c ? (p.sw == 2) : 0, csh = c ? (p.sh == 2) : 0;
+  const int x0c = (ctbX << l2c) >> csw, y0c = (ctbY << l2c) >> csh;
+  const int bd = c ? p.pp.bit_depth_chroma : p.pp.bit_depth_luma;
+  PIX* plane = (PIX*)p.plane[c];
+  const int stride = p.stride[c], pw = p.pw[c], ph = p.ph[c];
+  const int thr_strong = 1 << (p.pp.bit_depth_luma - 5);
+  const int pix_max = (1 << bd) - 1;
+  const uint32_t cval = 1u << (bd - 1);
+
+  for (uint32_t kbase = 0; kbase < ib_n; kbase += 64) {
+    const int nvalid = (int)min(64u, ib_n - kbase);
+    uint4 ex = make_uint4(0, 0, 0, 0);
+    if (lane < nvalid) ex = ((const uint4*)p.ib_aux)[ib_first + kbase + lane];
+    unsigned long long mine = __ballot((int)(lane < nvalid && ((ex.x >> 17) & 3u) == (uint32_t)c));
+    while (mine) {
+      const int src = __ffsll(mine) - 1;
+      mine &= mine - 1;
+      const uint32_t e0 = (uint32_t)__builtin_amdgcn_readlane((int)ex.x, src), e1 = (uint32_t)__builtin_amdgcn_readlane((int)ex.y, src);
+      const uint32_t e2 = (uint32_t)__builtin_amdgcn_readlane((int)ex.z, src), e3 = (uint32_t)__builtin_amdgcn_readlane((int)ex.w, src);
+      const int log2 = (int)((e0 >> 14) & 7u), nT = 1 << log2;
+      const int lx = (int)(e0 & 127u), ly = (int)((e0 >> 7) & 127u);
+      const int cls = (int)((e2 >> 8) & 7u), angle = (int)(int8_t)(e2 & 0xFFu), inv = (int)(int16_t)(e2 >> 16);
+      const int mode = (int)((e0 >> 19) & 63u);
+      const bool vert = mode >= 18;
+      const bool has_res = (e0 & M355_IBX_HAS_RES) != 0, bfilt = (e0 & M355_IBX_BFILT) != 0;
+      const int bx = x0c + lx, by = y0c + ly;
+      PIX* const dst = plane + (size_t)by * stride + bx;
+      const uint16_t* pl = p.iplan + plan_base + (e3 & 0xFFFFu);
+      auto put = [&](int x, int y, int v) { if (bx + x < pw && by + y < ph) dst[(size_t)y * stride + x] = (PIX)v; };
+
+      if (e0 & M355_IBX_PCM) {
+        for (int o = lane; o < nT * nT; o += 64) put(o & (nT - 1), o >> log2, (int)p.pcm[e1 + o]);
+      } else if (log2 <= 3) {
+        const uint32_t code = pl[min(lane, 4 << log2)];
+        const uint32_t bv = d_light_gather<PIX, CF>(plane, stride, pw, ph, x0c, y0c, c, code, cval);
+        const bool inb = lane < nT * nT;
+        const int rs = (has_res && inb) ? (int)p.resbuf[e1 + lane] : 0;
+        int v = log2 == 2 ? d_intra_small_predict<2>(bv, e0, cls, angle, inv, vert, bfilt, pix_max) : d_intra_small_predict<3>(bv, e0, cls, angle, inv, vert, bfilt, pix_max);
+        v = d_clip3(0, pix_max, v + rs);
+        if (inb) put(lane & (nT - 1), lane >> log2, v);
+      } else {
+        const int nEnt = 4 * nT + 1;
+        uint32_t cd[3] = {0, 0, 0}, val[3] = {0, 0, 0};
+#pragma unroll
+        for (int q = 0; q < 3; q++) {
+          if (64 * q >= nEnt) continue;
+          cd[q] = (uint32_t)pl[min(lane + 64 * q, nEnt - 1)];
+        }
+#pragma unroll
+        for (int q = 0; q < 3; q++) {
+          if (64 * q >= nEnt) continue;
+          val[q] = d_light_gather<PIX, CF>(plane, stride, pw, ph, x0c, y0c, c, cd[q], cval);
+        }
+#pragma unroll
+        for (int q = 0; q < 3; q++) {
+          if (64 * q >= nEnt) continue;
+          if (lane + 64 * q < nEnt) raw[lane + 64 * q] = (uint16_t)val[q];
+        }
+        wave_sync();
+        const uint16_t* P = raw;
+        if (e0 & M355_IBX_FILT) {
+          d_intra_big_filter(raw, pf, e0, nT, thr_strong);
+          wave_sync();
+          P = pf;
+        }
+        const int dcVal = mode == 1 ? d_intra_big_dc(P, nT, log2) : 0;
+        const int x = lane & (nT - 1), yb = lane >> log2, ystep = 64 >> log2, nPass = (nT * nT) >> 6;
+        const int16_t* res = p.resbuf + e1;
+        auto big_loop = [&](auto cls_) {
+          constexpr int CLS = decltype(cls_)::value;
+          const IntraBigFixed fx = d_intra_big_fixed<CLS>(P, nT, x, vert);
+          for (int it0 = 0; it0 < nPass; it0 += 4) {
+            int ta[4], tb[4], fa[4], rs[4];
+#pragma unroll
+            for (int u = 0; u < 4; u++) {
+              const int y = yb + (it0 + u) * ystep;
+              d_intra_big_taps<CLS>(P, nT, x, y, vert, angle, inv, ta[u], tb[u], fa[u]);
+              rs[u] = has_res ? (int)res[y * nT + x] : 0;
+            }
+#pragma unroll
+            for (int u = 0; u < 4; u++) {
+              const int y = yb + (it0 + u) * ystep;
+              int v = d_intra_big_value<CLS>(fx, nT, log2, x, y, vert, bfilt, dcVal, pix_max, ta[u], tb[u], fa[u]);
+              put(x, y, d_clip3(0, pix_max, v + rs[u]));
+            }
+          }
+        };
+        if (cls == 0) big_loop(std::integral_constant<int, 0>());
+        else if (cls == 1) big_loop(std::integral_constant<int, 1>());
+        else if (cls == 2) big_loop(std::integral_constant<int, 2>());
+        else if (cls == 3) big_loop(std::integral_constant<int, 3>());
+        else big_loop(std::integral_constant<int, 4>());
+        wave_sync();
+      }
+      if (mine || kbase + 64 < ib_n) d_drain_vmem();
+    }
+  }
+}
+
+#endif
diff --git a/libde265_amd/csrc/runtime_decode.hip b/libde265_amd/csrc/runtime_decode.hip
--- a/libde265_amd/csrc/runtime_decode.hip
+++ b/libde265_amd/csrc/runtime_decode.hip
@@ -130,6 +130,7 @@
   }
   d.epoch = ++c->epoch;
   if (d.epoch == 0) d.epoch = ++c->epoch;
+  c->dbg_intra[0] = r.n_intra_work; c->dbg_intra[1] = r.n_intra_ticket; c->dbg_intra[2] = r.n_intra_heavy; c->dbg_intra[3] = r.n_intra_light;
   d_out = d; want_sao_out = want_sao;
   return M355_OK;
 }
@@ -357,6 +358,7 @@
 }
 
 unsigned long long m355_last_serial(m355_ctx* c) { return c->serial; }
+M355_API void m355_debug_intra_counts(m355_ctx* c, int* out) { for (int i = 0; i < 4; i++) out[i] = c->dbg_intra[i]; }
 
 int m355_decode_status(m355_ctx* c, unsigned long long serial)
 {
diff --git a/libde265_amd/csrc/runtime_internal.h b/libde265_amd/csrc/runtime_internal.h
--- a/libde265_amd/csrc/runtime_internal.h
+++ b/libde265_amd/csrc/runtime_internal.h
@@ -41,6 +41,7 @@
 constexpr int chain_split_min_depth = 3;
 constexpr int chain_residual_tiles_min_depth = 3;
 constexpr int intra_class_first_lane = 3;
+constexpr bool intra_light_32x32 = false;
 }
 
 struct EvRef { unsigned long long ticket = 0; hipStream_t stream = nullptr; };
@@ -103,6 +104,7 @@
   DevRef* refs_host = nullptr;
   bool refs_valid = false;
   int n_intra_work = 0;
+  int n_intra_ticket = 0, n_intra_heavy = 0, n_intra_light = 0;
   uint32_t n_iplan = 0;
   bool sharded = false;
   int shard_rank = 0, shard_n = 1;
@@ -168,6 +170,7 @@
   unsigned long long serial = 0;
   unsigned long long lost_first = 0; int lost_count = 0;
   int stages = M355_STAGE_ALL;
+  int dbg_intra[4] = {0, 0, 0, 0};
   int shard_rank = 0, shard_n = 0;
   m355_comm comm = {nullptr, nullptr, nullptr};
   void* rccl = nullptr;
@@ -216,7 +219,7 @@
   Seg seg[32];
   int ns;
   size_t total;
-  int i_sl, i_ct, i_cu, i_tu, i_pb, i_wt, i_rb[4], i_ibin, i_ib, i_il, i_co, i_pc, i_sc, i_ts, i_rs, i_ti, i_iw, i_dp, i_ow;
+  int i_sl, i_ct, i_cu, i_tu, i_pb, i_wt, i_rb[4], i_ibin, i_ib, i_il, i_co, i_pc, i_sc, i_ts, i_rs, i_ti, i_iw, i_dp, i_ow, i_lt;
 };
 struct Id128 { char b[128]; };
 struct Rccl {
diff --git a/libde265_amd/csrc/runtime_upload.hip b/libde265_amd/csrc/runtime_upload.hip
--- a/libde265_amd/csrc/runtime_upload.hip
+++ b/libde265_amd/csrc/runtime_upload.hip
@@ -563,6 +563,7 @@
   L.i_iw = add(sizeof(DevIntraWork) * (size_t)nCtb);
   L.i_dp = add((size_t)nCtb);
   L.i_ow = add(sharded ? (size_t)nCtb : 0);
+  L.i_lt = add(16 * 3 * (size_t)nCtb);
 }
 
 int upload(m355_ctx* c, Resident& r, const m355_picture* pic) {
@@ -599,7 +600,7 @@
   const int ns = L.ns;
   const size_t total = L.total;
   const int i_sl = L.i_sl, i_ct = L.i_ct, i_cu = L.i_cu, i_tu = L.i_tu, i_pb = L.i_pb, i_wt = L.i_wt, i_ib = L.i_ib, i_il = L.i_il, i_co = L.i_co, i_pc = L.i_pc,
-            i_sc = L.i_sc, i_ts = L.i_ts, i_rs = L.i_rs, i_ti = L.i_ti, i_iw = L.i_iw, i_dp = L.i_dp, i_ow = L.i_ow;
+            i_sc = L.i_sc, i_ts = L.i_ts, i_rs = L.i_rs, i_ti = L.i_ti, i_iw = L.i_iw, i_dp = L.i_dp, i_ow = L.i_ow, i_lt = L.i_lt;
   {
     size_t rb_o = 0;
     const void* srcs[32]; size_t used[32];
@@ -685,7 +686,7 @@
   intra_dependencies(ctbW, ctbH, tile_id, ctb_touch, ctb_need, (uint8_t*)(r.host + seg[i_dp].ofs));
   for (int i = 0; i < nCtb; i++) ((uint8_t*)(r.host + seg[i_dp].ofs))[i] |= (uint8_t)(log2_waves[i] << 5);
   const auto t_deps = now();
-  int nw = 0, n_free = 0, n_ticket = 0;
+  int nw = 0, n_free = 0, n_ticket = 0, n_heavy = 0, n_light = 0;
   uint32_t n_iplan = 0;
   {
     const uint8_t* dep = (const uint8_t*)(r.host + seg[i_dp].ofs);
@@ -721,16 +722,34 @@
         for (int n = 0; n < 4; n++)
           if ((dep[rs] >> n) & 1) { uint32_t& pr = rem[(size_t)(cy + dy[n]) * ctbW + (cx + dx[n])]; pr = std::max(pr, mine); }
       }
-      bucket.assign((size_t)REM_CAP + 2 + (size_t)max_cnt + 2, 0);
-      size_t n_chain = 0;
+      static const int light32_env = getenv("M355_INTRA_LIGHT_32") ? atoi(getenv("M355_INTRA_LIGHT_32")) : -1;
+      const bool light_on = !sharded && !m355_res32(pp);
+      const bool light_32 = light32_env >= 0 ? light32_env != 0 : sched::intra_light_32x32;
+      for (size_t i = 0; i < n_cand; i++) {
+        const uint32_t rs = cand[2 * i];
+        bool heavy = !light_on;
+        if (light_on && !light_32 && !(dep[rs] & 31)) {
+          const m355_ctb& cb = pic->ctbs[rs];
+          for (uint32_t k = 0; k < cb.ib_count && !heavy; k++) heavy = pic->ibs[cb.ib_start + k].log2_size >= 5 && !(pic->ibs[cb.ib_start + k].flags & M355_IBF_PCM);
+        }
+        if (heavy) cand[2 * i + 1] |= 0x40000000u;
+      }
+      bucket.assign((size_t)REM_CAP + 2 + 2 * ((size_t)max_cnt + 2), 0);
+      size_t n_chain = 0, n_wg_free = 0;
       auto slot_of = [&](size_t i) -> size_t {
         const uint32_t rs = cand[2 * i];
-        return (dep[rs] & 31) ? (size_t)(REM_CAP - rem[rs]) : (size_t)REM_CAP + 1 + (size_t)(max_cnt - (cand[2 * i + 1] & 0x7FFFFFFFu));
+        if (dep[rs] & 31) return (size_t)(REM_CAP - rem[rs]);
+        const size_t by_count = (size_t)(max_cnt - (cand[2 * i + 1] & 0x3FFFFFFFu));
+        return (size_t)REM_CAP + 1 + ((cand[2 * i + 1] & 0x40000000u) ? 0 : (size_t)max_cnt + 1) + by_count;
       };
-      for (size_t i = 0; i < n_cand; i++) { bucket[slot_of(i) + 1]++; if (dep[cand[2 * i]] & 31) n_chain++; }
+      for (size_t i = 0; i < n_cand; i++) {
+        bucket[slot_of(i) + 1]++;
+        if (dep[cand[2 * i]] & 31) n_chain++; else if (cand[2 * i + 1] & 0x40000000u) n_wg_free++;
+      }
       for (size_t i = 1; i < bucket.size(); i++) bucket[i] += bucket[i - 1];
       for (size_t i = 0; i < n_cand; i++) order[bucket[slot_of(i)]++] = cand[2 * i];
       n_ticket = (int)n_chain;
+      n_heavy = (int)(n_chain + n_wg_free);
     } else {
     n_free = (int)(n_cand - n_dep);
     n_ticket = (int)n_cand;
@@ -755,6 +774,25 @@
     std::vector<uint32_t>& pbase = r.sched_u32b;
     pbase.resize((size_t)nw + 1);
     for (int k = 0; k < nw; k++) { pbase[(size_t)k] = n_iplan; n_iplan += (plan_count[order[(size_t)k]] + 7u) & ~7u; }
+    if (intra_dense) n_heavy = nw;
+    {
+      uint4* const lt = (uint4*)(r.host + seg[i_lt].ofs);
+      const m355_ib* const sorted_ibs = (const m355_ib*)(r.host + seg[i_ib].ofs);
+      for (int k = n_heavy; k < nw; k++) {
+        const m355_ctb& cb = pic->ctbs[order[(size_t)k]];
+        uint32_t first[3] = {~0u, ~0u, ~0u}, last[3] = {0, 0, 0};
+        for (uint32_t j = 0; j < cb.ib_count; j++) {
+          const int q = sorted_ibs[cb.ib_start + j].cidx;
+          if (q > 2) continue;
+          if (first[q] == ~0u) first[q] = j;
+          last[q] = j;
+        }
+        for (int q = 0; q < 3; q++)
+          if (first[q] != ~0u) lt[n_light++] = make_uint4(order[(size_t)k] | ((uint32_t)q << 30), cb.ib_start + first[q], last[q] - first[q] + 1u, pbase[(size_t)k]);
+      }
+      static const bool level_stats = getenv("M355_INTRA_LEVEL_STATS") != nullptr;
+      if (level_stats) fprintf(stderr, "intra work list: n_intra_work %d, n_intra_ticket %d, workgroup items %d, light items %d (of %d CTBs)\n", nw, n_ticket, n_heavy, n_light, nw - n_heavy);
+    }
     parallel_ranges((size_t)nw, 512, [&](size_t kb, size_t ke) {
       for (size_t k = kb; k < ke; k++) {
         const uint32_t rs = order[k];
@@ -777,7 +815,8 @@
     });
   }
   seg[i_iw].bytes = sizeof(DevIntraWork) * (size_t)(nw ? nw : 1);
-  r.n_intra_work = nw; r.n_iplan = n_iplan;
+  seg[i_lt].bytes = sizeof(uint4) * (size_t)n_light;
+  r.n_intra_work = nw; r.n_iplan = n_iplan; r.n_intra_ticket = n_ticket; r.n_intra_heavy = n_heavy; r.n_intra_light = n_light;
   if (sharded) {
     uint8_t* ow = (uint8_t*)(r.host + seg[i_ow].ofs);
     const int n_tiles = pp.num_tile_cols * pp.num_tile_rows;
@@ -837,6 +876,8 @@
   d.tile_id = (const uint16_t*)(r.dev + seg[i_ti].ofs);
   d.intra_work = (const DevIntraWork*)(r.dev + seg[i_iw].ofs);
   d.n_intra_work = nw; d.n_intra_ticket = n_ticket;
+  d.n_intra_heavy = n_heavy; d.n_intra_light = n_light;
+  d.intra_light = (const uint4*)(r.dev + seg[i_lt].ofs);
   d.ctb_dep = (const uint8_t*)(r.dev + seg[i_dp].ofs);
   d.ctb_owner = sharded ? (const uint8_t*)(r.dev + seg[i_ow].ofs) : nullptr;
   d.halo_cu_base = pic->n_cus; d.halo_pb_base = pic->n_pbs;
```

New measurement: 26.61 million CTB64/s (median of 6 runs). 1.03x the previous value.
